# apple/ml-gmpi

Hardware: AMD Instinct MI355X
Metric: Mpix*planes/s (higher is better)
Workload: dtype f32; 1 GPU; FFHQ1024-shaped: 1024x1024, 96 planes, batch 4 views, bf16 storage; views_per_gpu=4, views_total=4, H=1024, W=1024, planes=96, variant=auto, strict_order=False, outputs=rgb+depth, parallelism=views sharded x1, poses=truncated-gaussian draw (seed 3) on every rank

## Files before the change

### include/gmpi_render.h

```cpp
#ifndef GMPI_RENDER_H
#define GMPI_RENDER_H

#include <stdint.h>

#ifdef __cplusplus
extern "C" {
#endif

#define GMPI_ABI_VERSION 2

enum { GMPI_DTYPE_F32 = 0, GMPI_DTYPE_BF16 = 1, GMPI_DTYPE_F16 = 2, GMPI_DTYPE_U8 = 3 };

enum {
    GMPI_FLAG_ALIGN_CORNERS = 1 << 0,
    GMPI_FLAG_OUT_PM1 = 1 << 1,
    GMPI_FLAG_CHECK_LAST_PLANE = 1 << 2,
    GMPI_FLAG_CHECK_RANGE = 1 << 3,
    GMPI_FLAG_STRICT_ORDER = 1 << 4,
    GMPI_FLAG_HINT_FRONTAL = 1 << 5,
    GMPI_FLAG_HINT_TILTED = 1 << 6,
    GMPI_FLAG_GRAD_OVERWRITE = 1 << 7,
    GMPI_FLAG_HINT_OBLIQUE = 1 << 8,
    GMPI_FLAG_ALL = (1 << 9) - 1
};
// ... 9 lines not shown
enum {
    GMPI_VARIANT_AUTO = 0,
    GMPI_VARIANT_GATHER = 1,
    GMPI_VARIANT_LDS = 2,
    GMPI_VARIANT_WAVE = 3,
    GMPI_VARIANT_DMA = 4,
    GMPI_VARIANT_BAND = 5
};

enum {
    GMPI_OK = 0,
    GMPI_E_NULL = -1,
    GMPI_E_SHAPE = -2,
    GMPI_E_DTYPE = -3,
    GMPI_E_STRIDE = -4,
    GMPI_E_ABI = -5,
    GMPI_E_VARIANT = -6,
    GMPI_E_FLAGS = -7,
    GMPI_E_WORKSPACE = -8,
    GMPI_E_LAUNCH = -100
};

typedef struct GmpiRenderParams {
    uint32_t struct_size;
    uint32_t flags;
    int32_t variant;
    int32_t rgba_dtype;

    int32_t N, M, D;
    int32_t Ht, Wt;
    int32_t H, W;
    int32_t views_per_mpi;

    const void *rgba;
    int64_t rgba_stride[5];
    const int32_t *view_to_mpi;
    const float *dhw;
    const float *ray_dir;
    const float *eye_pos;
    const float *z_dir;

    float *rgb_out;
    float *depth_out;
    float *transmittance_out;
    uint32_t *status;

    void *workspace;
    uint64_t workspace_bytes;
} GmpiRenderParams;

uint64_t gmpi_render_workspace_bytes(const GmpiRenderParams *params);

int gmpi_mpi_render_launch(const GmpiRenderParams *params, void *stream);

int gmpi_mpi_render_layers_launch(const GmpiRenderParams *params, void *stream);

int gmpi_render_layers_supports(const GmpiRenderParams *params);

int gmpi_mpi_render_layers_backward_launch(const GmpiRenderParams *params, const float *grad_rgb, const float *grad_depth,
                                           const float *grad_transmittance , float *grad_layers,
                                           const int64_t *grad_layers_stride , void *stream);

int gmpi_render_layers_backward_supports(const GmpiRenderParams *params, const int64_t *grad_layers_stride);

int gmpi_mpi_render_backward_launch(const GmpiRenderParams *params, const float *grad_rgb, const float *grad_depth,
                                    float *grad_rgba, const int64_t *grad_rgba_stride, void *stream);
int gmpi_mpi_render_backward_ex_launch(const GmpiRenderParams *params, const float *grad_rgb, const float *grad_depth,
                                       const float *grad_transmittance, float *grad_rgba, const int64_t *grad_rgba_stride,
                                       void *stream);
uint64_t gmpi_render_backward_workspace_bytes(const GmpiRenderParams *params);

typedef struct GmpiCarry {
    uint32_t struct_size;
    uint32_t reserved;
    const float *state_in;
    float *state_out;
} GmpiCarry;
int gmpi_mpi_render_chunk_launch(const GmpiRenderParams *params, const GmpiCarry *carry, void *stream);

int gmpi_mpi_render_chunk_backward_launch(const GmpiRenderParams *params, const float *grad_rgb, const float *grad_depth,
                                          const float *grad_transmittance, const float *T_in, const float *S_in, float *S_out,
                                          float *grad_rgba, const int64_t *grad_rgba_stride, void *stream);

int gmpi_mpi_render_geometry_backward_launch(const GmpiRenderParams *params, const float *grad_rgb, const float *grad_depth,
                                             float *grad_ray_dir, float *grad_eye_pos, float *grad_z_dir, float *grad_dhw,
                                             void *stream);
int gmpi_mpi_render_geometry_backward_ex_launch(const GmpiRenderParams *params, const float *grad_rgb, const float *grad_depth,
                                                const float *grad_transmittance, float *grad_ray_dir, float *grad_eye_pos,
                                                float *grad_z_dir, float *grad_dhw, void *stream);
uint64_t gmpi_render_geometry_backward_workspace_bytes(const GmpiRenderParams *params, int want_dhw);

typedef struct GmpiSharedColor {
    uint32_t struct_size;
    const void *rgb;
    int64_t rgb_stride[3];
    const void *background;
    int64_t background_stride[3];
} GmpiSharedColor;

int gmpi_mpi_render_shared_launch(const GmpiRenderParams *params, const GmpiSharedColor *shared, void *stream);

int gmpi_render_shared_supports(const GmpiRenderParams *params, const GmpiSharedColor *shared);

int gmpi_mpi_render_shared_backward_launch(const GmpiRenderParams *params, const GmpiSharedColor *shared, const float *grad_rgb_out,
                                           const float *grad_depth, const float *grad_transmittance, float *grad_shared_rgb,
                                           const int64_t *grad_shared_rgb_stride, float *grad_alpha, const int64_t *grad_alpha_stride,
// ... 141 lines not shown
```

### ml-gmpi_amd/_lib.py

```python
import ctypes
import os
import subprocess

_PKG = os.path.dirname(os.path.abspath(__file__))
_SO = os.path.join(_PKG, "libgmpi_render.so")
_LIB = None

ABI_VERSION = 2
DTYPE_F32, DTYPE_BF16, DTYPE_F16 = 0, 1, 2
DTYPE_U8 = 3
FLAG_ALIGN_CORNERS, FLAG_OUT_PM1, FLAG_CHECK_LAST_PLANE, FLAG_CHECK_RANGE, FLAG_STRICT_ORDER, FLAG_HINT_FRONTAL, FLAG_HINT_TILTED = 1, 2, 4, 8, 16, 32, 64
FLAG_HINT_OBLIQUE = 256
FLAG_GRAD_OVERWRITE = 128
STATUS_OUT_OF_LAST_PLANE, STATUS_RGBA_RANGE, STATUS_CAMERA_BEHIND_PLANE, STATUS_BAD_VIEW_INDEX = 1, 2, 4, 8
STATUS_WORDS = 4
VARIANT_AUTO, VARIANT_GATHER, VARIANT_LDS, VARIANT_WAVE, VARIANT_DMA, VARIANT_BAND = 0, 1, 2, 3, 4, 5
VARIANTS = {"auto": VARIANT_AUTO, "gather": VARIANT_GATHER, "lds": VARIANT_LDS, "wave": VARIANT_WAVE, "band": VARIANT_BAND}

EXPORTS = (
    "gmpi_mpi_render_launch",
    "gmpi_render_workspace_bytes",
    "gmpi_render_backward_workspace_bytes",
    "gmpi_mpi_render_backward_launch",
    "gmpi_render_geometry_backward_workspace_bytes",
    "gmpi_mpi_render_geometry_backward_launch",
    "gmpi_mpi_render_backward_ex_launch",
    "gmpi_mpi_render_geometry_backward_ex_launch",
    "gmpi_mpi_render_chunk_launch",
    "gmpi_mpi_render_chunk_backward_launch",
    "gmpi_mpi_render_layers_launch",
    "gmpi_render_layers_supports",
    "gmpi_mpi_render_layers_backward_launch",
    "gmpi_render_layers_backward_supports",
    "gmpi_mpi_render_shared_launch",
    "gmpi_mpi_render_shared_backward_launch",
    "gmpi_render_shared_supports",
    "gmpi_mpi_render_shaded_launch",
    "gmpi_render_shaded_supports",
    "gmpi_mpi_render_shaded_backward_launch",
    "gmpi_mpi_render_depth_launch",
    "gmpi_mpi_render_depth_window_launch",
    "gmpi_render_depth_window_supports",
    "gmpi_mpi_render_depth_backward_launch",
    "gmpi_mpi_render_depth_backward_tile_launch",
    "gmpi_render_layout_backward_gather_workspace_bytes",
    "gmpi_render_layout_backward_gather_runs",
    "gmpi_render_layout_backward_gather_set_runs",
    "gmpi_mpi_render_shared_backward_gather_launch",
    "gmpi_mpi_render_depth_backward_gather_launch",
    "gmpi_mpi_render_shared_geometry_backward_launch",
    "gmpi_mpi_render_depth_geometry_backward_launch",
    "gmpi_mpi_render_depth_geometry_backward_pz_launch",
    "gmpi_render_depth_geometry_backward_workspace_bytes",
    "gmpi_last_plane_uv_minmax_launch",
    "gmpi_rgba_range_check_launch",
    "gmpi_frames_to_uint8_launch",
    "gmpi_generate_rays_launch",
    "gmpi_alpha_depth_launch",
    "gmpi_light_blur_launch",
    "gmpi_light_shading_launch",
    "gmpi_light_apply_launch",
    "gmpi_light_apply_backward_launch",
    "gmpi_light_shading_backward_launch",
    "gmpi_light_blur_backward_launch",
    "gmpi_light_shade_images_launch",
    "gmpi_light_shade_images_backward_launch",
    "gmpi_alpha_depth_backward_launch",
    "gmpi_alpha_depth_backward_ex_launch",
    "gmpi_ramp_depth_launch",
    "gmpi_ramp_depth_backward_launch",
    "gmpi_selftest_division_launch",
    "gmpi_stream_probe_launch",
    "gmpi_query",
    "gmpi_version_string",
)

_ERRORS = {
    -1: "GMPI_E_NULL (required pointer is NULL)",
    -2: "GMPI_E_SHAPE (non-positive or inconsistent extent, or more than 65535 views for the gather kernel / the backward)",
    -3: "GMPI_E_DTYPE (unknown rgba dtype, or uint8 storage handed to an entry other than the forward render)",
    -4: "GMPI_E_STRIDE (innermost rgba stride must be 1 -- or 4 with channel stride 1 for interleaved uint8 texels in the forward render, or for float layers at gmpi_mpi_render_layers_launch --, strides non-negative)",
    -5: "GMPI_E_ABI (GmpiRenderParams size mismatch between binding and library)",
    -6: "GMPI_E_VARIANT (requested kernel variant cannot run this shape)",
    -7: "GMPI_E_FLAGS (undefined bit in GmpiRenderParams.flags)",
    -8: "GMPI_E_WORKSPACE (workspace missing, too small or not 256-byte aligned)",
}


class GmpiError(RuntimeError):
    pass


class GmpiRenderParams(ctypes.Structure):
    _fields_ = [
        ("struct_size", ctypes.c_uint32), ("flags", ctypes.c_uint32),
        ("variant", ctypes.c_int32), ("rgba_dtype", ctypes.c_int32),
        ("N", ctypes.c_int32), ("M", ctypes.c_int32), ("D", ctypes.c_int32),
        ("Ht", ctypes.c_int32), ("Wt", ctypes.c_int32), ("H", ctypes.c_int32), ("W", ctypes.c_int32),
        ("views_per_mpi", ctypes.c_int32),
        ("rgba", ctypes.c_void_p), ("rgba_stride", ctypes.c_int64 * 5),
        ("view_to_mpi", ctypes.c_void_p), ("dhw", ctypes.c_void_p), ("ray_dir", ctypes.c_void_p),
        ("eye_pos", ctypes.c_void_p), ("z_dir", ctypes.c_void_p),
        ("rgb_out", ctypes.c_void_p), ("depth_out", ctypes.c_void_p), ("transmittance_out", ctypes.c_void_p),
        ("status", ctypes.c_void_p),
        ("workspace", ctypes.c_void_p), ("workspace_bytes", ctypes.c_uint64),
    ]


class GmpiCarry(ctypes.Structure):
    _fields_ = [
        ("struct_size", ctypes.c_uint32), ("reserved", ctypes.c_uint32),
        ("state_in", ctypes.c_void_p), ("state_out", ctypes.c_void_p),
    ]


class GmpiSharedColor(ctypes.Structure):
    _fields_ = [
        ("struct_size", ctypes.c_uint32),
        ("rgb", ctypes.c_void_p), ("rgb_stride", ctypes.c_int64 * 3),
        ("background", ctypes.c_void_p), ("background_stride", ctypes.c_int64 * 3),
    ]


class GmpiShading(ctypes.Structure):
    _fields_ = [
        ("struct_size", ctypes.c_uint32),
        ("shading", ctypes.c_void_p), ("shading_stride", ctypes.c_int64 * 2),
    ]


class GmpiDepthAlpha(ctypes.Structure):
    _fields_ = [
        ("struct_size", ctypes.c_uint32),
        ("plane_z", ctypes.c_void_p), ("plane_z_stride", ctypes.c_int64),
        ("z_lo", ctypes.c_float), ("z_hi", ctypes.c_float), ("z_den", ctypes.c_float),
    ]


def source_hash() -> str:
    import glob
    import hashlib
    h = hashlib.sha256()
    files = sorted(glob.glob(os.path.join(_PKG, "csrc", "*.hip")) + glob.glob(os.path.join(_PKG, "csrc", "*.hpp")))
    files.append(os.path.join(os.path.dirname(_PKG), "include", "gmpi_render.h"))
    for f in files:
        with open(f, "rb") as fh:
            h.update(os.path.basename(f).encode() + b"\0" + fh.read())
    return h.hexdigest()[:12]


def library_path() -> str:
    return _SO


_STAMP = os.path.join(_PKG, "csrc", ".built_from")


def build_extension(force: bool = False, verbose: bool = False) -> str:
    want = source_hash() + " " + _makefile_hash()
    have = open(_STAMP).read().strip() if os.path.isfile(_STAMP) else None
    force = force or os.environ.get("GMPI_BUILD_FORCE", "") not in ("", "0") or have != want or not os.path.isfile(_SO)
    cmd = ["make", "-C", os.path.join(_PKG, "csrc"), "-j4"] + (["-B"] if force else [])
    res = subprocess.run(cmd, capture_output=True, text=True)
    if verbose or res.returncode != 0:
        print(res.stdout)
        print(res.stderr)
    if res.returncode != 0 or not os.path.isfile(_SO):
        raise GmpiError("building libgmpi_render.so failed:\n" + res.stderr[-4000:])
    with open(_STAMP, "w") as f:
        f.write(want + "\n")
    return _SO


def _makefile_hash() -> str:
    import hashlib
    with open(os.path.join(_PKG, "csrc", "Makefile"), "rb") as f:
        return hashlib.sha256(f.read()).hexdigest()[:8]


def build_report() -> str:
    import glob
    import time
    rows = [f"sources {source_hash()} (csrc/*.hip, *.hpp, include/gmpi_render.h); stamp {open(_STAMP).read().strip() if os.path.isfile(_STAMP) else None}"]
    for f in sorted(glob.glob(os.path.join(_PKG, "csrc", "*.o"))) + [_SO]:
        if os.path.isfile(f):
            rows.append(f"  {os.path.relpath(f, os.path.dirname(_PKG)):44s} {os.path.getsize(f):9d} B  {time.strftime('%Y-%m-%d %H:%M:%S', time.localtime(os.path.getmtime(f)))}")
    return "\n".join(rows)


def load_library():
    global _LIB
    if _LIB is not None:
        return _LIB
    if not os.path.isfile(_SO):
        raise GmpiError(
            f"HIP extension not built: {_SO} is missing. This package has no CPU/PyTorch fallback. "
            "Build it with `python -c \"import __graft_entry__ as g; g.build()\"` or `make -C ml-gmpi_amd/csrc`.")
    import torch
    try:
        lib = ctypes.CDLL(_SO)
    except OSError as e:
        raise GmpiError(f"could not load {_SO}: {e}") from e
    missing = [s for s in EXPORTS if not hasattr(lib, s)]
    if missing:
        raise GmpiError(f"{_SO} does not export {missing}; rebuild it")
    vp = ctypes.c_void_p
    lib.gmpi_mpi_render_launch.restype = ctypes.c_int
    lib.gmpi_mpi_render_launch.argtypes = [ctypes.POINTER(GmpiRenderParams), vp]
    lib.gmpi_render_workspace_bytes.restype = ctypes.c_uint64
    lib.gmpi_render_workspace_bytes.argtypes = [ctypes.POINTER(GmpiRenderParams)]
    lib.gmpi_render_backward_workspace_bytes.restype = ctypes.c_uint64
    lib.gmpi_render_backward_workspace_bytes.argtypes = [ctypes.POINTER(GmpiRenderParams)]
    lib.gmpi_mpi_render_backward_launch.restype = ctypes.c_int
    lib.gmpi_mpi_render_backward_launch.argtypes = [ctypes.POINTER(GmpiRenderParams), vp, vp, vp,
                                                    ctypes.POINTER(ctypes.c_int64), vp]
    lib.gmpi_render_geometry_backward_workspace_bytes.restype = ctypes.c_uint64
    lib.gmpi_render_geometry_backward_workspace_bytes.argtypes = [ctypes.POINTER(GmpiRenderParams), ctypes.c_int]
    lib.gmpi_mpi_render_geometry_backward_launch.restype = ctypes.c_int
    lib.gmpi_mpi_render_geometry_backward_launch.argtypes = [ctypes.POINTER(GmpiRenderParams), vp, vp, vp, vp, vp, vp, vp]
    lib.gmpi_mpi_render_backward_ex_launch.restype = ctypes.c_int
    lib.gmpi_mpi_render_backward_ex_launch.argtypes = [ctypes.POINTER(GmpiRenderParams), vp, vp, vp, vp,
                                                       ctypes.POINTER(ctypes.c_int64), vp]
    lib.gmpi_mpi_render_geometry_backward_ex_launch.restype = ctypes.c_int
    lib.gmpi_mpi_render_geometry_backward_ex_launch.argtypes = [ctypes.POINTER(GmpiRenderParams), vp, vp, vp, vp, vp, vp, vp, vp]
    lib.gmpi_mpi_render_chunk_launch.restype = ctypes.c_int
    lib.gmpi_mpi_render_chunk_launch.argtypes = [ctypes.POINTER(GmpiRenderParams), ctypes.POINTER(GmpiCarry), vp]
    lib.gmpi_mpi_render_chunk_backward_launch.restype = ctypes.c_int
    lib.gmpi_mpi_render_chunk_backward_launch.argtypes = [ctypes.POINTER(GmpiRenderParams), vp, vp, vp, vp, vp, vp, vp,
                                                          ctypes.POINTER(ctypes.c_int64), vp]
    lib.gmpi_mpi_render_layers_launch.restype = ctypes.c_int
    lib.gmpi_mpi_render_layers_launch.argtypes = [ctypes.POINTER(GmpiRenderParams), vp]
    lib.gmpi_render_layers_supports.restype = ctypes.c_int
    lib.gmpi_render_layers_supports.argtypes = [ctypes.POINTER(GmpiRenderParams)]
    lib.gmpi_mpi_render_layers_backward_launch.restype = ctypes.c_int
    lib.gmpi_mpi_render_layers_backward_launch.argtypes = [ctypes.POINTER(GmpiRenderParams), vp, vp, vp, vp, ctypes.POINTER(ctypes.c_int64), vp]
    lib.gmpi_render_layers_backward_supports.restype = ctypes.c_int
    lib.gmpi_render_layers_backward_supports.argtypes = [ctypes.POINTER(GmpiRenderParams), ctypes.POINTER(ctypes.c_int64)]
    lib.gmpi_mpi_render_shared_launch.restype = ctypes.c_int
    lib.gmpi_mpi_render_shared_launch.argtypes = [ctypes.POINTER(GmpiRenderParams), ctypes.POINTER(GmpiSharedColor), vp]
    i64p = ctypes.POINTER(ctypes.c_int64)
    lib.gmpi_render_shared_supports.restype = ctypes.c_int
    lib.gmpi_render_shared_supports.argtypes = [ctypes.POINTER(GmpiRenderParams), ctypes.POINTER(GmpiSharedColor)]
    lib.gmpi_mpi_render_shared_backward_launch.restype = ctypes.c_int
    lib.gmpi_mpi_render_shared_backward_launch.argtypes = [ctypes.POINTER(GmpiRenderParams), ctypes.POINTER(GmpiSharedColor), vp, vp, vp,
                                                           vp, i64p, vp, i64p, vp, i64p, vp]
    lib.gmpi_mpi_render_shaded_launch.restype = ctypes.c_int
    lib.gmpi_mpi_render_shaded_launch.argtypes = [ctypes.POINTER(GmpiRenderParams), ctypes.POINTER(GmpiShading), vp]
    lib.gmpi_render_shaded_supports.restype = ctypes.c_int
    lib.gmpi_render_shaded_supports.argtypes = [ctypes.POINTER(GmpiRenderParams), ctypes.POINTER(GmpiShading)]
    lib.gmpi_mpi_render_shaded_backward_launch.restype = ctypes.c_int
    lib.gmpi_mpi_render_shaded_backward_launch.argtypes = [ctypes.POINTER(GmpiRenderParams), ctypes.POINTER(GmpiShading), vp, vp, vp, vp, i64p, vp, i64p, vp]
    lib.gmpi_mpi_render_depth_launch.restype = ctypes.c_int
    lib.gmpi_mpi_render_depth_launch.argtypes = [ctypes.POINTER(GmpiRenderParams), ctypes.POINTER(GmpiSharedColor), ctypes.POINTER(GmpiDepthAlpha), vp]
    lib.gmpi_mpi_render_depth_window_launch.restype = ctypes.c_int
    lib.gmpi_mpi_render_depth_window_launch.argtypes = list(lib.gmpi_mpi_render_depth_launch.argtypes)
    lib.gmpi_render_depth_window_supports.restype = ctypes.c_int
    lib.gmpi_render_depth_window_supports.argtypes = [ctypes.POINTER(GmpiRenderParams), ctypes.POINTER(GmpiSharedColor), ctypes.POINTER(GmpiDepthAlpha)]
    lib.gmpi_mpi_render_depth_backward_launch.restype = ctypes.c_int
    lib.gmpi_mpi_render_depth_backward_launch.argtypes = [ctypes.POINTER(GmpiRenderParams), ctypes.POINTER(GmpiSharedColor), ctypes.POINTER(GmpiDepthAlpha),
                                                          vp, vp, vp, vp, i64p, vp, i64p, vp, i64p, vp]
    lib.gmpi_mpi_render_depth_backward_tile_launch.restype = ctypes.c_int
# ... 91 lines not shown
```

### ml-gmpi_amd/csrc/gmpi_abi.hip

```cpp
#include "gmpi_device.hpp"
#include "gmpi_shared.hpp"

#include "../../include/gmpi_render.h"

#include <atomic>
#include <cstdlib>

namespace gmpi {

hipError_t launch_gather(const KParams& p, int dtype, hipStream_t stream);
hipError_t launch_lds(const KParams& p, int dtype, int tune, hipStream_t stream);
hipError_t launch_gather_chunk(const KParams& p, const CarryK& carry, int dtype, hipStream_t stream);
hipError_t launch_lds_chunk(const KParams& p, const CarryK& carry, int dtype, hipStream_t stream);
hipError_t launch_u8_chunk(const KParams& p, const CarryK& carry, hipStream_t stream);
hipError_t launch_backward_chunk(const KParams& p, int dtype, const float* g_rgb, const float* g_depth, const float* g_T, const float* T_in, const float* S_in,
                                 float* S_out, float* g_rgba, const int64_t* gstride, bool tiles, hipStream_t stream);
hipError_t launch_backward(const KParams& p, int dtype, const float* g_rgb, const float* g_depth, const float* g_T, float* g_rgba,
                           const int64_t* gstride, bool tiles, hipStream_t stream);
bool lds_variant_supports(const KParams& p, int dtype);
int lds_variant_query(int what);
hipError_t launch_wave(const KParams& p, int dtype, int tune, hipStream_t stream);
bool wave_variant_supports(const KParams& p, int dtype);
hipError_t launch_band(const KParams& p, int dtype, int tune, hipStream_t stream);
bool band_variant_supports(const KParams& p, int dtype);
// ... 178 lines not shown
                                                          float* __restrict__ depth, float* __restrict__ tout) {
    const int b = blockIdx.z;
    const int x = blockIdx.x * blockDim.x + threadIdx.x, y = blockIdx.y;
    if (x >= W) return;
    const T* a = alpha + b * sb + y * sr + x;
    float Tr = 1.0f, Z = 0.0f;
    alpha_depth_composite(D, ds, [&](int k) { return to_f32(a[k * sd]); }, Tr, Z);
    const int64_t o = (static_cast<int64_t>(b) * H + y) * W + x;
    depth[o] = Z;
    if (tout) tout[o] = Tr;
}

__device__ __forceinline__ uint32_t mix32(uint32_t x) {
    x ^= x >> 16, x *= 0x7feb352du, x ^= x >> 15, x *= 0x846ca68bu, x ^= x >> 16;
    return x;
}
__device__ __forceinline__ float unit_float(uint32_t h) { return __uint_as_float(0x3f800000u | (h >> 9)) - 1.0f; }
__global__ __launch_bounds__(256) void selftest_division_kernel(uint64_t pairs, uint32_t seed, unsigned long long* mism) {
    const uint64_t stride = static_cast<uint64_t>(gridDim.x) * blockDim.x;
    unsigned int bad[4] = {0, 0, 0, 0};
    for (uint64_t i = static_cast<uint64_t>(blockIdx.x) * blockDim.x + threadIdx.x; i < pairs; i += stride) {
        const uint32_t lo = static_cast<uint32_t>(i), hi = static_cast<uint32_t>(i >> 32);
        const uint32_t a = mix32(lo ^ seed), b = mix32(a + mix32(seed + 0x5bd1e995u) * 0x9e3779b9u + hi * 0x85ebca6bu + 0x85ebca6bu), c = mix32(b ^ 0xc2b2ae35u);
        const int cls = static_cast<int>(c & 3u);
        float n, d;
        if (cls == 0) {
            n = (unit_float(a) - 0.5f) * 4.0f;
            d = 0.35f + 0.65f * unit_float(b);
            if (c & 4u) d = -d;
        } else if (cls == 1) {
            n = (unit_float(a) - 0.5f) * 2.0f;
            d = 0.02f + 2.0f * unit_float(b);
        } else if (cls == 2) {
            n = __uint_as_float((a & 0x807fffffu) | ((107u + (a >> 23) % 41u) << 23));
            d = __uint_as_float((b & 0x807fffffu) | ((107u + (b >> 23) % 41u) << 23));
        } else {
            n = __uint_as_float((a & 0x807fffffu) | ((107u + (a >> 23) % 41u) << 23));
            d = __uint_as_float(0x007fffffu | ((107u + (b >> 23) % 41u) << 23) | (b & 0x80000000u));
        }
        const float r = 1.0f / d;
        const float q = div_by_recip(n, d, r);
        const float q_ref = n / d;
        if (__float_as_uint(q) != __float_as_uint(q_ref) && !(q == 0.0f && q_ref == 0.0f)) bad[cls]++;
    }
#pragma unroll
    for (int k = 0; k < 4; ++k) {
        unsigned int v = bad[k];
#pragma unroll
        for (int o = 32; o > 0; o >>= 1) v += __shfl_xor(v, o);
        if ((threadIdx.x & 63) == 0 && v) atomicAdd(mism + k, static_cast<unsigned long long>(v));
    }
}

static int to_kparams(const GmpiRenderParams* q, KParams& p, bool need_outputs, bool need_volume = false, bool takes_u8 = false) {
    if (q == nullptr) return GMPI_E_NULL;
    if (q->struct_size != sizeof(GmpiRenderParams)) return GMPI_E_ABI;
    bool interleaved = false;
    if (q->flags & ~static_cast<uint32_t>(GMPI_FLAG_ALL)) return GMPI_E_FLAGS;
    if (q->N < 0 || q->M <= 0 || q->D <= 0 || q->Ht <= 0 || q->Wt <= 0 || q->H <= 0 || q->W <= 0) return GMPI_E_SHAPE;
    if (q->view_to_mpi == nullptr) {
        if (q->views_per_mpi < 1) return GMPI_E_SHAPE;
        if (q->N > static_cast<int64_t>(q->M) * q->views_per_mpi) return GMPI_E_SHAPE;
    }
    if (q->dhw == nullptr || q->ray_dir == nullptr || q->eye_pos == nullptr) return GMPI_E_NULL;
    if (need_outputs && (q->rgb_out == nullptr || q->depth_out == nullptr)) return GMPI_E_NULL;
    if (need_outputs || need_volume) {
        if (q->rgba == nullptr || q->z_dir == nullptr) return GMPI_E_NULL;
        if (q->rgba_dtype < GMPI_DTYPE_F32 || q->rgba_dtype > (takes_u8 ? GMPI_DTYPE_U8 : GMPI_DTYPE_F16)) return GMPI_E_DTYPE;
        interleaved = takes_u8 && q->rgba_dtype == GMPI_DTYPE_U8 && q->rgba_stride[4] == 4 && q->rgba_stride[2] == 1;
        if (q->rgba_stride[4] != 1 && !interleaved) return GMPI_E_STRIDE;
        for (int i = 0; i < 4; ++i)
            if (q->rgba_stride[i] < 0) return GMPI_E_STRIDE;
        if (q->rgba_stride[3] < (interleaved ? 4 : 1) * static_cast<int64_t>(q->Wt) || q->rgba_stride[2] == 0 || q->rgba_stride[1] == 0) return GMPI_E_STRIDE;
    }
    p.rgba = q->rgba;
    p.view_to_mpi = q->view_to_mpi;
    p.dhw = q->dhw;
    p.ray_dir = q->ray_dir;
    p.eye_pos = q->eye_pos;
    p.z_dir = q->z_dir;
    p.rgb_out = q->rgb_out;
    p.depth_out = q->depth_out;
    p.T_out = q->transmittance_out;
    p.status = q->status;
    p.s_mpi = q->rgba_stride[0];
    p.s_plane = q->rgba_stride[1];
    p.s_chan = interleaved ? 0 : q->rgba_stride[2];
    p.s_row = q->rgba_stride[3];
    p.N = q->N, p.M = q->M, p.D = q->D, p.Ht = q->Ht, p.Wt = q->Wt, p.H = q->H, p.W = q->W;
    p.views_per_mpi = q->view_to_mpi ? 1 : q->views_per_mpi;
    p.flags = q->flags;
    p.ws = q->workspace;
    p.ws_bytes = q->workspace != nullptr ? q->workspace_bytes : 0;
    p.gate = nullptr, p.gate_gen = 0, p.gate_sense = 0;
    p.band_cols = 1, p.band_rot = 0, p.band_split = 1, p.band_tail = 0;
    return GMPI_OK;
}

constexpr int64_t kAutoBandMin = 256;
constexpr int64_t kAutoBandMinF32 = 1024;
constexpr int64_t kAutoBandMinUnmeasured = 512;
constexpr int64_t kAutoBandMinShared = 1024, kAutoBandMinSharedF32 = 2048;

static int64_t band_count(const KParams& p, int dtype) {
    const int bw = band_pixels_wide(dtype);
    return static_cast<int64_t>(p.N) * ((p.W + bw - 1) / bw) * ((p.H + 7) / 8);
}
static bool auto_takes_band(const KParams& p, int dtype) {
    if (dtype != GMPI_DTYPE_BF16 && dtype != GMPI_DTYPE_F32 && dtype != GMPI_DTYPE_F16) return false;
    if (p.view_to_mpi == nullptr && p.views_per_mpi > 1) {
        if ((p.flags & (GMPI_FLAG_HINT_OBLIQUE | GMPI_FLAG_HINT_TILTED)) != 0) return false;
#ifdef GMPI_TUNE
        static const int env_shared = [] { const char* e = getenv("GMPI_TUNE_SHARED"); return e ? atoi(e) : 1; }();
        if (env_shared == 0) return false;
#endif
    }
    const int bw = band_pixels_wide(dtype);
    const int64_t cols = (p.W + bw - 1) / bw, rows = (p.H + 7) / 8;
    if (static_cast<int64_t>(p.W) * 4 < cols * bw * 3 || static_cast<int64_t>(p.H) * 4 < rows * 8 * 3) return false;
    int64_t need = dtype == GMPI_DTYPE_F32 ? kAutoBandMinF32 : kAutoBandMin;
    if (p.view_to_mpi == nullptr && p.views_per_mpi > 1) need = dtype == GMPI_DTYPE_F32 ? kAutoBandMinSharedF32 : kAutoBandMinShared;
    if (dtype != GMPI_DTYPE_F32 && (p.flags & (GMPI_FLAG_STRICT_ORDER | GMPI_FLAG_HINT_TILTED | GMPI_FLAG_HINT_OBLIQUE)) != 0) need = kAutoBandMinUnmeasured;
    return band_count(p, dtype) >= need;
}

static int hip_rc(hipError_t e) { return e == hipSuccess ? GMPI_OK : GMPI_E_LAUNCH - static_cast<int>(e); }

static int layers_strides_ok(const GmpiRenderParams* q) {
    if (q->rgba_stride[2] != 1 || q->rgba_stride[4] != 4) return GMPI_E_STRIDE;
    if (q->rgba_stride[0] < 0 || q->rgba_stride[1] < 0 || q->rgba_stride[3] < 4 * static_cast<int64_t>(q->Wt)) return GMPI_E_STRIDE;
    return GMPI_OK;
}
static int to_kparams_layers(const GmpiRenderParams* q, KParams& p, bool backward = false) {
    GmpiRenderParams planar = *q;
    planar.rgba_stride[0] = planar.rgba_stride[1] = planar.rgba_stride[2] = 1, planar.rgba_stride[3] = q->Wt, planar.rgba_stride[4] = 1;
    const int rc = to_kparams(&planar, p, !backward, backward);
    if (rc != GMPI_OK) return rc;
    const int64_t esize = q->rgba_dtype == GMPI_DTYPE_F32 ? 4 : 2;
    p.s_mpi = q->rgba_stride[0] * esize, p.s_plane = q->rgba_stride[1] * esize, p.s_row = q->rgba_stride[3] * esize, p.s_chan = 0;
    return GMPI_OK;
}
static int layers_backward_args(const GmpiRenderParams* q, const int64_t* gst, KParams& p) {
    if (q == nullptr) return GMPI_E_NULL;
    if (q->struct_size != sizeof(GmpiRenderParams)) return GMPI_E_ABI;
    const int rs = layers_strides_ok(q);
    if (rs != GMPI_OK) return rs;
    if (q->rgba_dtype == GMPI_DTYPE_U8) return GMPI_E_DTYPE;
    const int rc = to_kparams_layers(q, p, true);
    if (rc != GMPI_OK) return rc;
    if (gst == nullptr) return GMPI_E_NULL;
    if (gst[2] != 1 || gst[4] != 4 || gst[3] < 4 * static_cast<int64_t>(q->Wt)) return GMPI_E_STRIDE;
    if (gst[1] <= 0 || (gst[0] <= 0 && !(gst[0] == 0 && q->M == 1))) return GMPI_E_STRIDE;
    return GMPI_OK;
}

}

using namespace gmpi;

extern "C" {

int gmpi_mpi_render_launch(const GmpiRenderParams* params, void* stream) {
    if (params != nullptr && params->struct_size == sizeof(GmpiRenderParams) && params->N == 0) return GMPI_OK;
    KParams p;
    const int rc = to_kparams(params, p, true, false, true);
    if (rc != GMPI_OK) return rc;
    if (p.N == 0) return GMPI_OK;
    hipStream_t st = static_cast<hipStream_t>(stream);
    int variant = params->variant;
    if (params->rgba_dtype == GMPI_DTYPE_U8) {
        const bool staged = u8_variant_supports(p);
        if (variant == GMPI_VARIANT_AUTO) variant = staged ? GMPI_VARIANT_LDS : GMPI_VARIANT_GATHER;
        if (variant == GMPI_VARIANT_GATHER) {
            if (p.N > 65535) return GMPI_E_SHAPE;
            return hip_rc(launch_gather(p, GMPI_DTYPE_U8, st));
        }
        if (variant == GMPI_VARIANT_LDS && staged) return hip_rc(launch_u8(p, st));
        return GMPI_E_VARIANT;
    }
    if (variant == GMPI_VARIANT_AUTO) {
        const int64_t pixels = static_cast<int64_t>(p.N) * p.H * p.W;
        const int64_t strips = static_cast<int64_t>(p.N) * ((p.W + 31) / 32) * ((p.H + 7) / 8);
        const bool strict = (p.flags & GMPI_FLAG_STRICT_ORDER) != 0;
        const bool lds_ok = lds_variant_supports(p, params->rgba_dtype), wave_ok = wave_variant_supports(p, params->rgba_dtype);
        const bool frontal = (p.flags & GMPI_FLAG_HINT_FRONTAL) != 0;
        const bool tilted = (p.flags & GMPI_FLAG_HINT_TILTED) != 0;
        const bool shared = p.view_to_mpi == nullptr && p.views_per_mpi > 1;
        const bool small = strict ? (pixels <= (int64_t(1) << 19) && pixels > (int64_t(1) << 18))
                         : params->rgba_dtype == GMPI_DTYPE_F32 ? (strips <= 512 || (strips > 1536 && strips <= 2048 && !tilted))
                                                                : (strips <= 512 || (strips <= 2048 && frontal && !shared));
        variant = (wave_ok && (small || !lds_ok)) ? GMPI_VARIANT_WAVE : lds_ok ? GMPI_VARIANT_LDS : GMPI_VARIANT_GATHER;
        const bool band_path = lds_ok && auto_takes_band(p, params->rgba_dtype) && band_variant_supports(p, params->rgba_dtype);
        if (band_path) variant = GMPI_VARIANT_LDS;
        if (band_path) {
            static std::atomic<uint32_t> gate_counter{0x6d2b79f5u};
            uint32_t gen = gate_counter.fetch_add(1u, std::memory_order_relaxed);
            KParams pb = p;
            pb.gate = band_gate_words(p, params->rgba_dtype), pb.gate_gen = gen, pb.gate_sense = 0u;
            const hipError_t e = launch_band(pb, params->rgba_dtype, 0, st);
            if (e != hipSuccess) return hip_rc(e);
            pb.gate_sense = 1u;
            return hip_rc(launch_lds(pb, params->rgba_dtype, 0, st));
        }
    }
    if (variant == GMPI_VARIANT_GATHER) {
        if (p.N > 65535) return GMPI_E_SHAPE;
        return hip_rc(launch_gather(p, params->rgba_dtype, st));
    }
    int tune = 0;
#ifdef GMPI_TUNE
    static const int env_tune = [] { const char* e = getenv("GMPI_TUNE_WAVE"); return e ? atoi(e) : 0; }();
    tune = env_tune;
#endif
    if (variant == GMPI_VARIANT_WAVE) {
        if (!wave_variant_supports(p, params->rgba_dtype)) return GMPI_E_VARIANT;
        return hip_rc(launch_wave(p, params->rgba_dtype, tune, st));
    }
    if (variant == GMPI_VARIANT_LDS) {
        if (!lds_variant_supports(p, params->rgba_dtype)) return GMPI_E_VARIANT;
        return hip_rc(launch_lds(p, params->rgba_dtype, tune, st));
    }
    if (variant == GMPI_VARIANT_BAND) {
        if (!band_variant_supports(p, params->rgba_dtype)) return GMPI_E_VARIANT;
        return hip_rc(launch_band(p, params->rgba_dtype, tune, st));
    }
    return GMPI_E_VARIANT;
}

int gmpi_render_layers_supports(const GmpiRenderParams* params) {
    if (params == nullptr) return GMPI_E_NULL;
    if (params->struct_size != sizeof(GmpiRenderParams)) return GMPI_E_ABI;
    const int rs = layers_strides_ok(params);
    if (rs != GMPI_OK) return rs;
    KParams p;
    if (params->rgba_dtype == GMPI_DTYPE_U8) {
        const int rc = to_kparams(params, p, true, false, true);
        return rc != GMPI_OK ? rc : (u8_variant_supports(p) ? 1 : 0);
    }
    const int rc = to_kparams_layers(params, p);
    return rc != GMPI_OK ? rc : (layers_variant_supports(p, params->rgba_dtype) ? 1 : 0);
}

int gmpi_mpi_render_layers_launch(const GmpiRenderParams* params, void* stream) {
    if (params == nullptr) return GMPI_E_NULL;
    if (params->struct_size != sizeof(GmpiRenderParams)) return GMPI_E_ABI;
    if (params->N == 0) return GMPI_OK;
    const int rs = layers_strides_ok(params);
    if (rs != GMPI_OK) return rs;
    if (params->rgba_dtype == GMPI_DTYPE_U8) return gmpi_mpi_render_launch(params, stream);
    KParams p;
    const int rc = to_kparams_layers(params, p);
    if (rc != GMPI_OK) return rc;
    int variant = params->variant;
    if (variant != GMPI_VARIANT_AUTO && variant != GMPI_VARIANT_GATHER && variant != GMPI_VARIANT_LDS) return GMPI_E_VARIANT;
    const bool staged = layers_variant_supports(p, params->rgba_dtype);
    if (variant == GMPI_VARIANT_AUTO) variant = staged ? GMPI_VARIANT_LDS : GMPI_VARIANT_GATHER;
    hipStream_t st = static_cast<hipStream_t>(stream);
    if (variant == GMPI_VARIANT_GATHER) {
        if (p.N > 65535) return GMPI_E_SHAPE;
        return hip_rc(launch_gather_layers(p, params->rgba_dtype, st));
    }
    if (!staged) return GMPI_E_VARIANT;
    return hip_rc(launch_layers(p, params->rgba_dtype, st));
}

int gmpi_render_layers_backward_supports(const GmpiRenderParams* params, const int64_t* grad_layers_stride) {
    KParams p;
    const int rc = layers_backward_args(params, grad_layers_stride, p);
    return rc != GMPI_OK ? rc : (backward_layers_tile_supports(p, params->rgba_dtype, grad_layers_stride) ? 1 : 0);
}

int gmpi_mpi_render_layers_backward_launch(const GmpiRenderParams* params, const float* grad_rgb, const float* grad_depth, const float* grad_transmittance,
                                           float* grad_layers, const int64_t* grad_layers_stride, void* stream) {
    if (params != nullptr && params->struct_size == sizeof(GmpiRenderParams) && params->N == 0) return GMPI_OK;
    KParams p;
    const int rc = layers_backward_args(params, grad_layers_stride, p);
    if (rc != GMPI_OK) return rc;
    if (grad_rgb == nullptr || grad_layers == nullptr) return GMPI_E_NULL;
    return hip_rc(launch_backward_layers(p, params->rgba_dtype, grad_rgb, grad_depth, grad_transmittance, grad_layers, grad_layers_stride,
                                         params->variant != GMPI_VARIANT_GATHER, static_cast<hipStream_t>(stream)));
}

uint64_t gmpi_render_workspace_bytes(const GmpiRenderParams* params) {
    KParams p;
    if (to_kparams(params, p, true, false, true) != GMPI_OK || p.N == 0) return 0;
    if (params->rgba_dtype == GMPI_DTYPE_U8) return 0;
    if (params->variant == GMPI_VARIANT_BAND) return band_workspace_bytes(p, params->rgba_dtype);
    if (params->variant == GMPI_VARIANT_AUTO && auto_takes_band(p, params->rgba_dtype)) return band_workspace_bytes(p, params->rgba_dtype);
    return 0;
}

uint64_t gmpi_render_backward_workspace_bytes(const GmpiRenderParams* params) {
    KParams p;
    if (to_kparams(params, p, false, true) != GMPI_OK || p.N == 0) return 0;
    if (params->variant == GMPI_VARIANT_GATHER) return 0;
    return backward_gather_workspace_bytes(p, params->rgba_dtype);
}

int gmpi_mpi_render_backward_launch(const GmpiRenderParams* params, const float* grad_rgb, const float* grad_depth,
                                    float* grad_rgba, const int64_t* grad_rgba_stride, void* stream) {
    return gmpi_mpi_render_backward_ex_launch(params, grad_rgb, grad_depth, nullptr, grad_rgba, grad_rgba_stride, stream);
}

int gmpi_mpi_render_backward_ex_launch(const GmpiRenderParams* params, const float* grad_rgb, const float* grad_depth,
                                       const float* grad_transmittance, float* grad_rgba, const int64_t* grad_rgba_stride, void* stream) {
    if (params != nullptr && params->struct_size == sizeof(GmpiRenderParams) && params->N == 0) return GMPI_OK;
    KParams p;
    const int rc = to_kparams(params, p, false, true);
    if (rc != GMPI_OK) return rc;
    if (grad_rgb == nullptr || grad_rgba == nullptr || grad_rgba_stride == nullptr) return GMPI_E_NULL;
    if (p.N > 65535) return GMPI_E_SHAPE;
    if (grad_rgba_stride[4] != 1) return GMPI_E_STRIDE;
    for (int i = 0; i < 4; ++i)
        if (grad_rgba_stride[i] <= 0 && !(i == 0 && params->M == 1)) return GMPI_E_STRIDE;
    return hip_rc(launch_backward(p, params->rgba_dtype, grad_rgb, grad_depth, grad_transmittance, grad_rgba, grad_rgba_stride,
                                  params->variant != GMPI_VARIANT_GATHER, static_cast<hipStream_t>(stream)));
}

int gmpi_mpi_render_chunk_launch(const GmpiRenderParams* params, const GmpiCarry* carry, void* stream) {
    if (params != nullptr && params->struct_size == sizeof(GmpiRenderParams) && params->N == 0) return GMPI_OK;
    KParams p;
    const int rc = to_kparams(params, p, false, true, true);
    if (rc != GMPI_OK) return rc;
    if (carry == nullptr) return GMPI_E_NULL;
    if (carry->struct_size != sizeof(GmpiCarry)) return GMPI_E_ABI;
    int variant = params->variant;
    if (variant == GMPI_VARIANT_WAVE || variant == GMPI_VARIANT_BAND) return GMPI_E_VARIANT;
    if (variant != GMPI_VARIANT_AUTO && variant != GMPI_VARIANT_GATHER && variant != GMPI_VARIANT_LDS) return GMPI_E_VARIANT;
    if (carry->state_out == nullptr && p.rgb_out == nullptr && p.depth_out == nullptr && p.T_out == nullptr) return GMPI_E_NULL;
    const CarryK ck{carry->state_in, carry->state_out};
    p.ws = nullptr, p.ws_bytes = 0;
    hipStream_t st = static_cast<hipStream_t>(stream);
    const bool u8 = params->rgba_dtype == GMPI_DTYPE_U8;
    const bool staged = u8 ? u8_variant_supports(p) : lds_variant_supports(p, params->rgba_dtype);
    if (variant == GMPI_VARIANT_AUTO) variant = staged ? GMPI_VARIANT_LDS : GMPI_VARIANT_GATHER;
    if (variant == GMPI_VARIANT_GATHER) {
        if (p.N > 65535) return GMPI_E_SHAPE;
        return hip_rc(launch_gather_chunk(p, ck, params->rgba_dtype, st));
// ... 493 lines not shown
    hipStream_t st = static_cast<hipStream_t>(stream);
    dispatch_dtype(alpha_dtype, [&](auto t) {
        using T = typename decltype(t)::type;
        hipLaunchKernelGGL(alpha_depth_kernel<T>, grid, block, 0, st, static_cast<const T*>(alpha), stride_b, stride_d, stride_row, plane_ds, D, H, W, depth_out,
                           transmittance_out);
    });
    return hip_rc(hipGetLastError());
}

int gmpi_selftest_division_launch(uint64_t pairs, uint32_t seed, uint64_t* mismatches, void* stream) {
    if (mismatches == nullptr) return GMPI_E_NULL;
    if (pairs == 0) return GMPI_OK;
    const uint64_t want = (pairs + 255) / 256;
    const unsigned blocks = static_cast<unsigned>(want < 256u * 64u ? want : 256u * 64u);
    hipLaunchKernelGGL(selftest_division_kernel, dim3(blocks), dim3(256), 0, static_cast<hipStream_t>(stream), pairs, seed,
                       reinterpret_cast<unsigned long long*>(mismatches));
    return hip_rc(hipGetLastError());
}

int gmpi_stream_probe_launch(const void* buf, uint64_t bytes, uint32_t* sink, void* stream) {
    if (buf == nullptr) return GMPI_E_NULL;
    if (reinterpret_cast<uintptr_t>(buf) % 4 != 0) return GMPI_E_STRIDE;
    if (bytes < 4) return GMPI_OK;
    hipLaunchKernelGGL(stream_probe_kernel, dim3(256 * 2), dim3(256), 0, static_cast<hipStream_t>(stream), static_cast<const uint32_t*>(buf),
                       static_cast<int64_t>(bytes / 4), sink);
    return hip_rc(hipGetLastError());
}

int gmpi_query(int32_t what) {
    switch (what) {
        case 0: return GMPI_ABI_VERSION;
        case 1: return static_cast<int>(sizeof(GmpiRenderParams));
        case 2: return 950;
        case 3: case 4: case 5: return lds_variant_query(what);
        case 6: return 1;
        case 7: return 0;
        case 8: return 1;
        case 9: return static_cast<int>(kAutoBandMin);
        case 10: return static_cast<int>(kAutoBandMinF32);
        case 11: return 1;
        case 12: case 13: case 14: return shared_forward_query(what);
        case 16: case 17: case 18: case 20: return u8_variant_query(what);
        case 22: return 1;
        case 23: return depth_tile_planes();
        case 25: return 1;
        case 26: case 27: case 28: return depth_window_query(what);
        case 30: return 1;
        case 32: return 1;
        case 34: return 1;
        case 38: return 1;
        case 40: return 1;
        case 42: return 1;
        case 44: return 1;
        case 46: return 1;
        case 36: return 1;
        default: return -1;
    }
}

const char* gmpi_version_string(void) { return "ml-gmpi_amd 0.3 (gfx950, ABI 2)"; }

}
```

### ml-gmpi_amd/csrc/gmpi_device.hpp

```cpp
#pragma once
#include <hip/hip_runtime.h>
#include <stdint.h>

#include <type_traits>

#include "../../include/gmpi_render.h"

#pragma clang fp contract(off)

namespace gmpi {

constexpr float kNarrowScale = 0.95f;

struct KParams {
    const void* rgba;
    const int32_t* view_to_mpi;
    const float* dhw;
    const float* ray_dir;
    const float* eye_pos;
    const float* z_dir;
    float* rgb_out;
    float* depth_out;
    float* T_out;
    uint32_t* status;
    int64_t s_mpi, s_plane, s_chan, s_row;
    int32_t N, M, D, Ht, Wt, H, W, views_per_mpi;
    uint32_t flags;
    void* ws;
    uint64_t ws_bytes;
    uint32_t* gate;
    uint32_t gate_gen, gate_sense;
    int32_t band_cols;
    int32_t band_rot, band_split;
    int32_t band_tail;
};
struct CarryK {
    const float* state_in;
    float* state_out;
};
struct NoCarry {};

__device__ __forceinline__ int xcd_item_per_group(int block, int group_items, int n_items, int rot = 0, int split = 1) {
    const int per_xcd = (group_items + 7) / 8, n_groups = (n_items + group_items - 1) / group_items;
    const int jb = block / 8, grp = jb / per_xcd, rr = jb - grp * per_xcd;
    const int piece = split > 1 ? rr * split / per_xcd : 0;
    const int in_group = ((block + grp * rot + piece * (8 / max(split, 1))) % 8) * per_xcd + rr;
    const int item = grp * group_items + in_group;
    return (grp >= n_groups || in_group >= group_items || item >= n_items) ? n_items : item;
}
inline __host__ unsigned xcd_grid_per_group(int group_items, int n_items) {
    return static_cast<unsigned>(((group_items + 7) / 8) * 8 * ((n_items + group_items - 1) / group_items));
}

__device__ __forceinline__ bool view_gated_out(const KParams& p, int n) {
    return p.gate != nullptr && ((p.gate[n] == p.gate_gen) != (p.gate_sense != 0u));
}

__device__ __forceinline__ int view_mpi(const KParams& p, int n, uint32_t& bad) {
    int m = p.view_to_mpi ? p.view_to_mpi[n] : n / p.views_per_mpi;
    if (m < 0 || m >= p.M) {
        bad |= GMPI_STATUS_BAD_VIEW_INDEX;
        m = min(max(m, 0), p.M - 1);
    }
    return m;
}

__device__ __forceinline__ void item_to_view(const KParams& p, int item, int per_view, int& n, int& rem) {
    if (p.view_to_mpi == nullptr && p.views_per_mpi > 1) {
        const int group = item / (per_view * p.views_per_mpi);
        const int first = group * p.views_per_mpi, size = min(p.views_per_mpi, p.N - first);
        const int r = item - first * per_view;
        rem = r / size;
        n = first + (r - rem * size);
    } else {
        n = item / per_view;
        rem = item - n * per_view;
    }
}

struct bf16_t { uint16_t bits; };
struct f16_t { _Float16 v; };

__device__ __forceinline__ float to_f32(float v) { return v; }
__device__ __forceinline__ float to_f32(bf16_t v) { return __uint_as_float(static_cast<uint32_t>(v.bits) << 16); }
__device__ __forceinline__ float to_f32(f16_t v) { return static_cast<float>(v.v); }
struct u8_t { uint8_t code; };
constexpr float kInv255 = 1.0f / 255.0f;
__device__ __forceinline__ float unorm8_to_f32(float c) {
// ... 244 lines not shown
            const float t_se = to_f32(ch[ob + xb]);
            if (check_range && !(in_unit(t_nw) && in_unit(t_ne) && in_unit(t_sw) && in_unit(t_se))) bad |= GMPI_STATUS_RGBA_RANGE;
            smp[c] = bilerp<STRICT>(t_nw, t_ne, t_sw, t_se, f);
        }
    }
}

struct NoShade {};
struct ShadeK {
    const float* s;
    int64_t s_mpi, s_row;
};
__device__ __forceinline__ float shade_texel(float t, float s) { return fminf(fmaxf(t * s, 0.0f), 1.0f); }

template <typename TexT, bool STRICT>
__device__ __forceinline__ void shaded_gather_sample(const TexT* __restrict__ pl, int64_t s_chan, int64_t s_row, const float* __restrict__ sh, int64_t sh_row,
                                                     int Ht, int Wt, float ix, float iy, bool check_range, uint32_t& bad, float (&smp)[4]) {
    Footprint f = footprint(ix, iy, Ht, Wt);
    const bool x0in = f.x0 >= 0 && f.x0 <= Wt - 1, x1in = f.x0 >= -1 && f.x0 <= Wt - 2;
    const bool y0in = f.y0 >= 0 && f.y0 <= Ht - 1, y1in = f.y0 >= -1 && f.y0 <= Ht - 2;
    if (!(x0in && y0in)) f.nw = 0.0f;
    if (!(x1in && y0in)) f.ne = 0.0f;
    if (!(x0in && y1in)) f.sw = 0.0f;
    if (!(x1in && y1in)) f.se = 0.0f;
    const int xa = min(max(f.x0, 0), Wt - 1), xb = min(max(f.x0 + 1, 0), Wt - 1);
    const int ya = min(max(f.y0, 0), Ht - 1), yb = min(max(f.y0 + 1, 0), Ht - 1);
    const int64_t oa = static_cast<int64_t>(ya) * s_row, ob = static_cast<int64_t>(yb) * s_row;
    const int64_t ha = static_cast<int64_t>(ya) * sh_row, hb = static_cast<int64_t>(yb) * sh_row;
    const float s_nw = sh[ha + xa], s_ne = sh[ha + xb], s_sw = sh[hb + xa], s_se = sh[hb + xb];
#pragma unroll
    for (int c = 0; c < 4; ++c) {
        const TexT* __restrict__ ch = pl + c * s_chan;
        float t_nw = to_f32(ch[oa + xa]);
        float t_ne = to_f32(ch[oa + xb]);
        float t_sw = to_f32(ch[ob + xa]);
        float t_se = to_f32(ch[ob + xb]);
        if (c < 3) {
            t_nw = shade_texel(t_nw, s_nw), t_ne = shade_texel(t_ne, s_ne), t_sw = shade_texel(t_sw, s_sw), t_se = shade_texel(t_se, s_se);
        } else if (check_range && !(in_unit(t_nw) && in_unit(t_ne) && in_unit(t_sw) && in_unit(t_se))) {
            bad |= GMPI_STATUS_RGBA_RANGE;
        }
        smp[c] = bilerp<STRICT>(t_nw, t_ne, t_sw, t_se, f);
    }
}

struct View {
    int m;
    const float* __restrict__ dhw;
    float ex, ey, ez;
    float zx, zy, zz;
    float cx, cy;
    int64_t HW;
    const float* __restrict__ rays;
};
template <bool AC>
__device__ __forceinline__ View view_setup(const KParams& p, int n, uint32_t& bad) {
    View vw;
    vw.m = view_mpi(p, n, bad);
    vw.dhw = p.dhw + static_cast<int64_t>(vw.m) * p.D * 3;
    vw.ex = p.eye_pos[3 * n + 0], vw.ey = p.eye_pos[3 * n + 1], vw.ez = p.eye_pos[3 * n + 2];
    vw.zx = p.z_dir[3 * n + 0], vw.zy = p.z_dir[3 * n + 1], vw.zz = p.z_dir[3 * n + 2];
    vw.cx = AC ? static_cast<float>(p.Wt - 1) * 0.5f : static_cast<float>(p.Wt);
    vw.cy = AC ? static_cast<float>(p.Ht - 1) * 0.5f : static_cast<float>(p.Ht);
    vw.HW = static_cast<int64_t>(p.H) * p.W;
    vw.rays = p.ray_dir + static_cast<int64_t>(n) * 3 * vw.HW;
    return vw;
}

__device__ __forceinline__ void check_camera_behind(const KParams& p, const View& vw, bool once) {
    if (p.status != nullptr && once) {
        const float ez0 = p.eye_pos[2];
        bool behind = false;
        for (int k = 0; k < p.D; ++k) behind |= !(vw.dhw[3 * k] >= ez0);
        if (behind) atomicOr(p.status, GMPI_STATUS_CAMERA_BEHIND_PLANE);
    }
}

__device__ __forceinline__ float ray_dot(const View& vw, float rx, float ry, float rz) {
    float dot = rx * vw.zx;
    dot = dot + ry * vw.zy;
    dot = dot + rz * vw.zz;
    return dot;
}

__device__ __forceinline__ bool outside_pm1(float u, float v) { return !(u >= -1.0f && u <= 1.0f && v >= -1.0f && v <= 1.0f); }

struct LastPlane {
    bool check;
    float d, ph, pw;
};
__device__ __forceinline__ LastPlane last_plane(const KParams& p, const View& vw) {
    LastPlane lp{(p.flags & GMPI_FLAG_CHECK_LAST_PLANE) != 0, 0.0f, 1.0f, 1.0f};
    if (lp.check) lp.d = vw.dhw[3 * (p.D - 1) + 0], lp.ph = vw.dhw[3 * (p.D - 1) + 1], lp.pw = vw.dhw[3 * (p.D - 1) + 2];
    return lp;
}
template <bool AC>
__device__ __forceinline__ bool leaves_last_plane(const View& vw, const LastPlane& lp, float rx, float ry, float rz) {
    if (!lp.check) return false;
    float ix, iy, s, u, v;
    plane_coord<AC>(lp.d - vw.ez, lp.ph, lp.pw, vw.ex, vw.ey, rx, ry, rz, vw.cx, vw.cy, ix, iy, s, u, v);
    return outside_pm1(u, v);
}

template <typename TexT, bool AC, bool STRICT, typename CheckT>
__device__ __forceinline__ void gather_plane(const KParams& p, const View& vw, const TexT* vol, int k, float zdiff, float ph, float pw,
                                             float rx, float ry, float rz, float dot, CheckT check_range, uint32_t& bad, Accum& A) {
    float ix, iy, s, u, v, smp[4];
    plane_coord<AC>(zdiff, ph, pw, vw.ex, vw.ey, rx, ry, rz, vw.cx, vw.cy, ix, iy, s, u, v);
    gather_sample<TexT, STRICT>(tex_offset(vol, static_cast<int64_t>(k) * p.s_plane), p.s_chan, p.s_row, p.Ht, p.Wt, ix, iy, check_range, bad, smp);
    blend<STRICT>(A, smp[0], smp[1], smp[2], smp[3], s, dot);
}

__device__ __forceinline__ Accum load_carry(NoCarry, int, int64_t, int64_t) { return Accum{}; }
__device__ __forceinline__ void store_carry(NoCarry, int, int64_t, int64_t, const Accum&, bool) {}
__device__ __forceinline__ Accum load_carry(const CarryK& c, int n, int64_t HW, int64_t pix) {
    Accum A;
    if (c.state_in != nullptr) {
        const float* s = c.state_in + static_cast<int64_t>(n) * 5 * HW + pix;
        A.r = s[0], A.g = s[HW], A.b = s[2 * HW], A.z = s[3 * HW], A.T = s[4 * HW];
    }
    return A;
}
__device__ __forceinline__ void store_carry(const CarryK& c, int n, int64_t HW, int64_t pix, const Accum& A, bool active) {
    if (c.state_out != nullptr && active) {
// ... 24 lines not shown
    if (active) {
        float* __restrict__ out = p.rgb_out + static_cast<int64_t>(n) * 3 * HW + pix;
        out[0] = r;
        out[HW] = g;
        out[2 * HW] = b;
        p.depth_out[static_cast<int64_t>(n) * HW + pix] = finish_depth<STRICT>(A, dot);
        if (p.T_out) p.T_out[static_cast<int64_t>(n) * HW + pix] = A.T;
    }
}

inline __host__ __device__ int view_group_items(const KParams& p, int per_view) { return per_view * (p.view_to_mpi == nullptr ? p.views_per_mpi : 1); }

__device__ __forceinline__ int fwd_tile_id(const KParams& p, int block, int tiles_x, int tiles_y, int n_tiles, int rot = 0, int split = 1) {
    return xcd_item_per_group(block, view_group_items(p, tiles_x * tiles_y), n_tiles, rot, split);
}
struct FwdTile { int n, rem, txi, tyi; };
__device__ __forceinline__ bool fwd_tile(const KParams& p, int tile_id, int tiles_x, int tiles_y, int n_tiles, FwdTile& t) {
    if (tile_id >= n_tiles) return false;
    item_to_view(p, tile_id, tiles_x * tiles_y, t.n, t.rem);
    t.tyi = t.rem / tiles_x, t.txi = t.rem - t.tyi * tiles_x;
    return true;
}
struct FwdTileGrid { int tiles_x, tiles_y, n_tiles; dim3 grid; };
template <int TW, int TH>
inline FwdTileGrid fwd_tile_grid(const KParams& p) {
    const int tiles_x = (p.W + TW - 1) / TW, tiles_y = (p.H + TH - 1) / TH, n_tiles = tiles_x * tiles_y * p.N;
    return FwdTileGrid{tiles_x, tiles_y, n_tiles, dim3(xcd_grid_per_group(view_group_items(p, tiles_x * tiles_y), n_tiles))};
}

struct TileLane { int px, py; bool active; int64_t pix; };
template <int TW, int TH>
__device__ __forceinline__ TileLane tile_lane(int txi, int tyi, int lane, int W, int H) {
    TileLane l;
    l.px = txi * TW + (lane % TW), l.py = tyi * TH + (lane / TW);
    l.active = l.px < W && l.py < H;
    l.pix = static_cast<int64_t>(min(l.py, H - 1)) * W + min(l.px, W - 1);
    return l;
}
struct TileCorners { int cx0, cx1, cy0, cy1; };
template <int TW, int TH>
__device__ __forceinline__ TileCorners tile_corners(int txi, int tyi, int W, int H) {
    const int cx0 = txi * TW, cy0 = tyi * TH;
    return TileCorners{cx0, min(cx0 + TW - 1, W - 1), cy0, min(cy0 + TH - 1, H - 1)};
}

struct CornerExtent { float mnx, mxx, mny, mxy; bool finite; };
template <bool AC>
__device__ __forceinline__ CornerExtent corner_extent(const View& vw, const float* __restrict__ rdv, int W, float zdiff, float ph, float pw, int cx0, int cx1,
                                                      int cy0, int cy1, float (&cix)[4], float (&ciy)[4]) {
    CornerExtent e{__builtin_inff(), -__builtin_inff(), __builtin_inff(), -__builtin_inff(), true};
#pragma unroll
    for (int c = 0; c < 4; ++c) {
        const int64_t q = static_cast<int64_t>((c & 2) ? cy1 : cy0) * W + ((c & 1) ? cx1 : cx0);
        float s, u, v;
        plane_coord<AC>(zdiff, ph, pw, vw.ex, vw.ey, rdv[q], rdv[vw.HW + q], rdv[2 * vw.HW + q], vw.cx, vw.cy, cix[c], ciy[c], s, u, v);
        e.finite = e.finite && (fabsf(cix[c]) < 1e6f) && (fabsf(ciy[c]) < 1e6f);
        e.mnx = fminf(e.mnx, cix[c]), e.mxx = fmaxf(e.mxx, cix[c]), e.mny = fminf(e.mny, ciy[c]), e.mxy = fmaxf(e.mxy, ciy[c]);
    }
    return e;
}
template <bool AC>
__device__ __forceinline__ CornerExtent corner_extent(const View& vw, const float* __restrict__ rdv, int W, float zdiff, float ph, float pw, int cx0, int cx1,
                                                      int cy0, int cy1) {
    float cix[4], ciy[4];
    return corner_extent<AC>(vw, rdv, W, zdiff, ph, pw, cx0, cx1, cy0, cy1, cix, ciy);
}
constexpr float kBoxSlack = 1.0f / 64;
template <int TPI>
__device__ __forceinline__ int4 item_box(const CornerExtent& e, int max_cols, int max_rows, bool& fits) {
    int4 bb = make_int4(0, 0, 0, 0);
    fits = false;
    if (e.finite) {
        const int bx0 = static_cast<int>(floorf(e.mnx - kBoxSlack)), bx1 = static_cast<int>(floorf(e.mxx + kBoxSlack)) + 1;
        const int by0 = static_cast<int>(floorf(e.mny - kBoxSlack)), by1 = static_cast<int>(floorf(e.mxy + kBoxSlack)) + 1;
        bb.x = bx0 & ~(TPI - 1), bb.y = by0;
        bb.z = (bx1 - bb.x) / TPI + 1, bb.w = by1 - by0 + 1;
        fits = bb.z <= max_cols && bb.w <= max_rows;
    }
    return bb;
}
template <bool AC>
__device__ __forceinline__ int4 tile_box(const KParams& p, const View& vw, const float* __restrict__ rdv, float zdiff, float ph, float pw, int cx0, int cx1,
                                         int cy0, int cy1, int pitch, int rows, float (&cix)[4], float (&ciy)[4]) {
    bool fits;
    int4 bb = item_box<1>(corner_extent<AC>(vw, rdv, p.W, zdiff, ph, pw, cx0, cx1, cy0, cy1, cix, ciy), pitch, rows, fits);
    if (!fits) bb.z = 0;
    return bb;
}
template <bool AC>
__device__ __forceinline__ int4 tile_box(const KParams& p, const View& vw, const float* __restrict__ rdv, float zdiff, float ph, float pw, int cx0, int cx1,
                                         int cy0, int cy1, int pitch, int rows) {
    float cix[4], ciy[4];
    return tile_box<AC>(p, vw, rdv, zdiff, ph, pw, cx0, cx1, cy0, cy1, pitch, rows, cix, ciy);
}

__device__ __forceinline__ int2 origin_words(uint64_t a) { return make_int2(static_cast<int>(a & 0xffffffffu), static_cast<int>((a >> 32) & 0xffffu)); }
__device__ __forceinline__ __amdgpu_buffer_rsrc_t origin_rsrc(int lo, int hi) {
    const uint32_t b_lo = static_cast<uint32_t>(__builtin_amdgcn_readfirstlane(lo)), b_hi = static_cast<uint32_t>(__builtin_amdgcn_readfirstlane(hi));
    return __builtin_amdgcn_make_buffer_rsrc(reinterpret_cast<void*>((static_cast<uint64_t>(b_hi) << 32) | b_lo), 0, static_cast<int>(0x80000000u), 0x00020000);
}

__device__ __forceinline__ int floor_to_int(float x) {
    int r;
    asm("v_cvt_flr_i32_f32 %0, %1" : "=v"(r) : "v"(x));
    return r;
}

__device__ __forceinline__ void report_status(uint32_t* status, uint32_t bad) {
// ... 10 lines not shown
```

### ml-gmpi_amd/csrc/render_band.hip

```cpp
#include "gmpi_device.hpp"
#include "gmpi_band_masks.hpp"

#include <algorithm>
#include <cstdlib>
#include <type_traits>


namespace gmpi {
namespace band {

constexpr int kNT = 1024;
constexpr int SBW = 64, SBH = 8;
constexpr float kBoxEps = 1.0f / 64;
constexpr int kWindowCols16 = 2, kWindowCols32 = 2, kWindowCols32Deep = 2, kDeepPlanes = 128;
constexpr int kViewRotation = 1;
constexpr int kRunPieces = 2;
constexpr int kTicketTail = 16;
constexpr float kCoordLimit = 16384.0f;

typedef uint32_t u32x4 __attribute__((ext_vector_type(4)));
template <int V> using ic = std::integral_constant<int, V>;

template <int D0, int STEP>
__device__ __forceinline__ void dma16x2(uint32_t voff, uint32_t soff1, const u32x4& rsrc, uint32_t lds_dst, uint64_t m0, uint64_t m1);
// ... 82 lines not shown
                 "s_mov_b64 exec, %7\n\ts_add_i32 m0, %3, %16\n\ts_nop 0\n\tbuffer_load_dwordx4 %1, %2, %11 offen lds\n\t"
                 "s_mov_b64 exec, %8\n\ts_add_i32 m0, %3, %17\n\ts_nop 0\n\tbuffer_load_dwordx4 %1, %2, %12 offen lds\n\t"
                 "s_mov_b64 exec, %0"
                 : "=&s"(save) : "v"(voff), "s"(rsrc), "s"(lds_dst), "s"(m0), "s"(m1), "s"(m2), "s"(m3), "s"(m4), "s"(s1), "s"(s2), "s"(s3), "s"(s4),
                   "i"(D0), "i"(D0 + STEP), "i"(D0 + 2 * STEP), "i"(D0 + 3 * STEP), "i"(D0 + 4 * STEP)
                 : "memory", "scc");
}
__device__ __forceinline__ void wg_barrier() { asm volatile("s_waitcnt vmcnt(0) lgkmcnt(0)\n\ts_barrier" ::: "memory"); }
template <int O> __device__ __forceinline__ void tap16(uint32_t& t, uint32_t a) {
    asm volatile("ds_read_u16_d16_hi %0, %1 offset:%2" : "=v"(t) : "v"(a), "i"(O));
}
template <int O> __device__ __forceinline__ void tap32x2(uint32_t& t0, uint32_t& t1, uint32_t a) {
    typedef uint32_t u32x2 __attribute__((ext_vector_type(2)));
    u32x2 v;
    asm volatile("ds_read2_b32 %0, %1 offset0:%2 offset1:%3" : "=v"(v) : "v"(a), "i"(O), "i"(O + 1));
    t0 = v.x, t1 = v.y;
}

__device__ __forceinline__ void band_pos(int brem, int bands_x, int bands_y, int wc, int& bxi, int& byi) {
    const int per_window = wc * bands_y;
    const int g = brem / per_window, r = brem - g * per_window;
    const int cols = min(wc, bands_x - g * wc);
    byi = r / cols;
    bxi = g * wc + (r - byi * cols);
}

constexpr int kPlU4 = 2;
__device__ __forceinline__ uint32_t shape_pack(int nq, int rows, int clo, int ncol, int rlo, int nrow, bool inside) {
    return inside ? static_cast<uint32_t>(nq | rows << 5)
                  : static_cast<uint32_t>(nq | rows << 5 | clo << 9 | ncol << 14 | rlo << 19 | nrow << 23) | 0x80000000u;
}
struct Shape { int nq, rows; uint32_t clo, ncol, rlo, nrow; };
__device__ __forceinline__ Shape shape_unpack(uint32_t w) {
    Shape h;
    h.nq = w & 31, h.rows = (w >> 5) & 15;
    const bool padded = (w >> 31) != 0;
    h.clo = padded ? (w >> 9) & 31 : 0u, h.ncol = padded ? (w >> 14) & 31 : static_cast<uint32_t>(h.nq);
    h.rlo = padded ? (w >> 19) & 15 : 0u, h.nrow = padded ? (w >> 23) & 15 : static_cast<uint32_t>(h.rows);
    return h;
}
template <typename TexT, bool AC>
__global__ __launch_bounds__(1024) void band_table_kernel(const KParams p, const int bands_x, const int bands_y, const int n_bands, const float cx, const float cy,
                                                         uint4* __restrict__ recs, uint4* __restrict__ pl, uint32_t* __restrict__ hdr, uint32_t* __restrict__ tickets) {
    using G = Geo<TexT>;
    constexpr int kES = G::kES, kTPI = G::kTPI, kCols = G::kCols, kMaxRows = G::kMaxRows, kRowBytes = G::kRowBytes, kSubBytes = G::kSubBytes;
    constexpr int NSB = G::NSB;
    static_assert(kCols < 32 && kMaxRows < 16, "shape_pack");
    const int band_id = blockIdx.x;
    int n, brem;
    item_to_view(p, band_id, bands_x * bands_y, n, brem);
    int bxi, byi;
    band_pos(brem, bands_x, bands_y, p.band_cols, bxi, byi);
    uint32_t ignore = 0;
    const int m = view_mpi(p, n, ignore);
    const int Ht = p.Ht, Wt = p.Wt, H = p.H, W = p.W;
    const float ex = p.eye_pos[3 * n + 0], ey = p.eye_pos[3 * n + 1], ez = p.eye_pos[3 * n + 2];
    const int64_t HW = static_cast<int64_t>(H) * W;
    const float* __restrict__ rdv = p.ray_dir + static_cast<int64_t>(n) * 3 * HW;
    const TexT* __restrict__ vol = static_cast<const TexT*>(p.rgba) + static_cast<int64_t>(m) * p.s_mpi;
    const int sx0 = min(bxi * (NSB * SBW), W - 1), sy0 = byi * SBH;
    const int by0p = min(sy0, H - 1), by1p = min(sy0 + SBH - 1, H - 1);
    bool unfit = false;
    for (int i = threadIdx.x; i < p.D * NSB; i += blockDim.x) {
        const int b = i % NSB, k = i / NSB;
        const float* __restrict__ dhw = p.dhw + (static_cast<int64_t>(m) * p.D + k) * 3;
        const float d = dhw[0], ph = dhw[1], pw = dhw[2];
        const float zdiff = d - ez;
        const float hw = pw * 0.5f, hh = ph * 0.5f;
        const int bx0p = min(sx0 + b * SBW, W - 1), bx1p = min(sx0 + b * SBW + SBW - 1, W - 1);
        float mnx = __builtin_inff(), mxx = -__builtin_inff(), mny = mnx, mxy = mxx;
        bool finite = true;
        const float rw_a = __builtin_amdgcn_rcpf(hw), rh_a = __builtin_amdgcn_rcpf(hh);
#pragma unroll
        for (int c = 0; c < 4; ++c) {
            const int64_t q = static_cast<int64_t>((c & 2) ? by1p : by0p) * W + ((c & 1) ? bx1p : bx0p);
            float ix, iy, sc;
            const float crz = rdv[2 * HW + q];
            plane_coord_recip<AC>(zdiff, hw, hh, rw_a, rh_a, ex, ey, rdv[q], rdv[HW + q], crz, __builtin_amdgcn_rcpf(crz), cx, cy, ix, iy, sc);
            finite = finite && (fabsf(ix) < kCoordLimit) && (fabsf(iy) < kCoordLimit);
            mnx = fminf(mnx, ix), mxx = fmaxf(mxx, ix), mny = fminf(mny, iy), mxy = fmaxf(mxy, iy);
        }
        int qx0 = 0, by0 = 0, nq = -1, nrows = 0;
        if (finite) {
            const int bx0 = static_cast<int>(floorf(mnx - kBoxEps)), bx1 = static_cast<int>(floorf(mxx + kBoxEps)) + 1;
            by0 = static_cast<int>(floorf(mny - kBoxEps));
            const int by1 = static_cast<int>(floorf(mxy + kBoxEps)) + 1;
            qx0 = bx0 & ~(kTPI - 1);
            nq = (bx1 - qx0) / kTPI + 1;
            nrows = by1 - by0 + 1;
            if (nq > kCols || nrows > kMaxRows) nq = -1;
        }
        uint32_t shape = 0;
        if (nq > 0) {
            const int clo = min(max(-qx0 / kTPI, 0), nq), chi = min(max((Wt - qx0) / kTPI, 0), nq);
            const int rlo = min(max(-by0, 0), nrows), rhi = min(max(Ht - by0, 0), nrows);
            const bool inside = clo == 0 && chi == nq && rlo == 0 && rhi == nrows;
            shape = shape_pack(nq, nrows, clo, chi - clo, rlo, rhi - rlo, inside);
        } else {
            qx0 = 0, by0 = 0;
            unfit = true;
        }
        const uint64_t origin = reinterpret_cast<uint64_t>(vol + (static_cast<int64_t>(k) * p.s_plane + static_cast<int64_t>(by0) * p.s_row + qx0));
        const int gpart = b * kSubBytes - (by0 * kRowBytes + qx0 * kES);
        recs[(static_cast<int64_t>(band_id) * p.D + k) * NSB + b] =
            make_uint4(static_cast<uint32_t>(origin & 0xffffffffu), static_cast<uint32_t>((origin >> 32) & 0xffffu), shape, static_cast<uint32_t>(gpart));
        if (brem == 0 && b == 0) {
            uint4* r = pl + (static_cast<int64_t>(n) * p.D + k) * kPlU4;
            r[0] = make_uint4(__float_as_uint(zdiff), __float_as_uint(hw), __float_as_uint(hh), __float_as_uint(1.0f / hw));
            r[1] = make_uint4(__float_as_uint(1.0f / hh), 0u, 0u, 0u);
        }
    }
    if (blockIdx.x == 0 && threadIdx.x < 8) tickets[threadIdx.x] = 0u;
    const int any_unfit = __syncthreads_or(unfit ? 1 : 0);
    if (threadIdx.x == 0) {
        hdr[band_id] = static_cast<uint32_t>(any_unfit);
        if (any_unfit && p.gate != nullptr) {
            if (p.view_to_mpi == nullptr && p.views_per_mpi > 1) {
                const int first = n / p.views_per_mpi * p.views_per_mpi, size = min(p.views_per_mpi, p.N - first);
                for (int v = 0; v < size; ++v) p.gate[first + v] = p.gate_gen;
            } else {
                p.gate[n] = p.gate_gen;
            }
        }
    }
}

template <typename TexT, bool AC, bool STRICT, bool CHECK>
__global__ __launch_bounds__(Geo<TexT>::kThreads, Geo<TexT>::kWavesPerSimd) void render_band_kernel(const KParams p, const int bands_x, const int bands_y, const int n_bands, const float cx, const float cy,
                                                         const uint4* __restrict__ recs, const uint4* __restrict__ pl, const uint32_t* __restrict__ hdr, uint32_t* __restrict__ tickets) {
    using G = Geo<TexT>;
    constexpr int kES = G::kES, kTPI = G::kTPI, kCols = G::kCols, kNP = G::kNP;
// ... 7 lines not shown
    __shared__ __attribute__((aligned(16))) unsigned char smem[G::kLdsBytes];
    typedef __attribute__((address_space(3))) unsigned char lds_byte;
    const uint32_t tile_base = static_cast<uint32_t>(reinterpret_cast<uintptr_t>((lds_byte*)smem));

    const int group_items = bands_x * bands_y * (p.view_to_mpi == nullptr ? p.views_per_mpi : 1);
    int band_id;
    {
        const int per_xcd = (group_items + 7) / 8, n_groups = (n_bands + group_items - 1) / group_items, static_blocks = per_xcd * 8 * n_groups;
        const int T = min(p.band_tail, per_xcd);
        const int jb = static_cast<int>(blockIdx.x) / 8, x = static_cast<int>(blockIdx.x) % 8;
        const bool ticketed = T > 0 && (static_cast<int>(blockIdx.x) >= static_blocks || (jb / per_xcd == n_groups - 1 && jb % per_xcd >= per_xcd - T));
        if (!ticketed) {
            band_id = blockIdx.x < static_cast<unsigned>(static_blocks) ? xcd_item_per_group(blockIdx.x, group_items, n_bands, p.band_rot, p.band_split) : n_bands;
        } else {
            int* word = reinterpret_cast<int*>(smem + 2 * kBufBytes);
            if (threadIdx.x == 0) {
                int got = n_bands;
                for (int i = 0; i < 8; ++i) {
                    const int q = (x + i) % 8;
                    const int t = static_cast<int>(atomicAdd(tickets + q, 1u));
                    if (t < T) {
                        got = xcd_item_per_group(q + 8 * ((n_groups - 1) * per_xcd + per_xcd - T + t), group_items, n_bands, p.band_rot, p.band_split);
                        break;
                    }
                }
                *word = got;
            }
            __syncthreads();
            band_id = __builtin_amdgcn_readfirstlane(*word);
            __syncthreads();
        }
    }
#ifdef GMPI_TUNE
    if (p.flags & (1u << 19)) band_id = static_cast<int>(blockIdx.x % 8) * ((n_bands + 7) / 8) + static_cast<int>(blockIdx.x / 8);
#endif
    if (band_id >= n_bands) return;
    int n, brem;
    item_to_view(p, band_id, bands_x * bands_y, n, brem);
    if (view_gated_out(p, n)) return;
    int bxi, byi;
    band_pos(brem, bands_x, bands_y, p.band_cols, bxi, byi);
#ifdef GMPI_TUNE
    const bool stamp = (p.flags & (1u << 22)) != 0 && p.status != nullptr;
    uint64_t stamp_start = 0;
    if (stamp) asm volatile("s_memrealtime %0\n\ts_waitcnt lgkmcnt(0)" : "=s"(stamp_start));
#endif

    const int tid = threadIdx.x;
    auto fresh_tid = [&]() { int t = tid; asm volatile("" : "+v"(t)); return t; };
    const int wave = __builtin_amdgcn_readfirstlane(tid >> 6);
    const int sb = wave / WPS, wj = wave % WPS;
    const int lane = tid & 63;
    uint32_t bad_w = 0;
    View vw = view_setup<AC>(p, n, bad_w);
    vw.cx = cx, vw.cy = cy;
    const int D = p.D, H = p.H, W = p.W;
    const float* __restrict__ dhw = vw.dhw;
    const float ex = vw.ex, ey = vw.ey, ez = vw.ez;
    constexpr bool check_range = CHECK;
    const int64_t HW = vw.HW;
    const float* __restrict__ rdv = vw.rays;
    const TexT* __restrict__ vol = static_cast<const TexT*>(p.rgba) + static_cast<int64_t>(vw.m) * p.s_mpi;
    const int64_t s_chan = p.s_chan, s_row = p.s_row;

    check_camera_behind(p, vw, brem == 0 && tid == 0);

    const int px = bxi * (NSB * SBW) + sb * SBW + lane;
    const int py0 = byi * SBH + wj;
    const int pxc = min(px, W - 1);
    float rx[PPT], ry[PPT], rz[PPT], rcp_rz[PPT];
    Accum A[PPT];
#pragma unroll
    for (int q = 0; q < PPT; ++q) {
        const int64_t pix = static_cast<int64_t>(min(py0 + WPS * q, H - 1)) * W + pxc;
        rx[q] = rdv[pix], ry[q] = rdv[HW + pix], rz[q] = rdv[2 * HW + pix];
        rcp_rz[q] = 1.0f / rz[q];
    }
    auto ray_dot = [&](int q) { return gmpi::ray_dot(vw, rx[q], ry[q], rz[q]); };

    auto loader_pos = [&](int& l_col, int& l_line, int& l_row, bool& l_on) {
        const int t = fresh_tid() & (kSubLanes - 1);
        l_line = t / kCols, l_col = t - l_line * kCols, l_row = l_line >> 2, l_on = t < kPassItems;
    };
    {
        int l_col, l_line, l_row;
        bool l_on;
        loader_pos(l_col, l_line, l_row, l_on);
        reinterpret_cast<uint32_t*>(smem + 2 * kBufBytes)[tid] = static_cast<uint32_t>(l_row * s_row + (l_line & 3) * s_chan + kTPI * l_col) * static_cast<uint32_t>(kES);
    }
    const uint32_t pass_off = static_cast<uint32_t>(kRPP * s_row) * static_cast<uint32_t>(kES), pass_off2 = 2 * pass_off;
    const uint32_t pass_off3 = 3 * pass_off, pass_off4 = 4 * pass_off;
    const uint32_t sub_base = tile_base + static_cast<uint32_t>(sb * kSubBytes);
    const uint32_t wave_dst = sub_base + static_cast<uint32_t>(wj) * 1024u;

#ifdef GMPI_TUNE
    const bool abl_noload = (p.flags & (1u << 16)) != 0, abl_nocomp = (p.flags & (1u << 17)) != 0, abl_noissue = (p.flags & (1u << 18)) != 0;
    const bool abl_nobar = (p.flags & (1u << 20)) != 0, abl_norec = (p.flags & (1u << 21)) != 0;
#else
    constexpr bool abl_noload = false, abl_nocomp = false, abl_noissue = false, abl_nobar = false, abl_norec = false;
#endif

#ifdef GMPI_PROF
    uint32_t prof_acc[8] = {0, 0, 0, 0, 0, 0, 0, 0};
    uint64_t prof_last, prof_start;
    asm volatile("s_memtime %0\n\ts_waitcnt lgkmcnt(0)" : "=s"(prof_start));
    prof_last = prof_start;
#define GMPI_STAMP(i) do { uint64_t now_; asm volatile("s_memtime %0\n\ts_waitcnt lgkmcnt(0)" : "=s"(now_)); prof_acc[i] += static_cast<uint32_t>(now_ - prof_last); prof_last = now_; } while (0)
#else
#define GMPI_STAMP(i) do { } while (0)
#endif

    const uint4* __restrict__ myrec = recs + (static_cast<int64_t>(band_id) * D * NSB + sb);
    const uint4* __restrict__ mypl = pl + static_cast<int64_t>(n) * D * kPlU4;
    constexpr int kRecStep = NSB;

    if (hdr[band_id] != 0) {
#pragma unroll
        for (int q = 0; q < PPT; ++q) {
            const float dot = ray_dot(q);
            for (int t = 0; t < D; ++t) {
                uint32_t gbad = 0;
                gather_plane<TexT, AC, STRICT>(p, vw, vol, t, dhw[3 * t] - ez, dhw[3 * t + 1], dhw[3 * t + 2], rx[q], ry[q], rz[q], dot, std::bool_constant<CHECK>{}, gbad, A[q]);
                if (check_range && __any(gbad != 0)) bad_w |= GMPI_STATUS_RGBA_RANGE;
            }
        }
    } else {
        float dots[PPT];
#pragma unroll
// ... 465 lines not shown
```

### ml-gmpi_amd/csrc/render_gather.hip

```cpp
#include "gmpi_device.hpp"

namespace gmpi {

constexpr int kGatherTileW = 64;
constexpr int kGatherTileH = 4;

template <typename TexT, bool AC, bool STRICT, typename Carry>
__device__ __forceinline__ void render_gather_pixel(const KParams& p, const Carry& carry) {
    const int n = blockIdx.z;
    const int px = blockIdx.x * kGatherTileW + threadIdx.x;
    const int py = blockIdx.y * kGatherTileH + threadIdx.y;
    uint32_t bad = 0;
    const View vw = view_setup<AC>(p, n, bad);
    check_camera_behind(p, vw, blockIdx.x == 0 && blockIdx.y == 0 && threadIdx.x == 0 && threadIdx.y == 0);
    const bool active = px < p.W && py < p.H;
    const int64_t HW = vw.HW;
    const int64_t pix = static_cast<int64_t>(min(py, p.H - 1)) * p.W + min(px, p.W - 1);
    const float rx = vw.rays[pix], ry = vw.rays[HW + pix], rz = vw.rays[2 * HW + pix];
    const float dot = ray_dot(vw, rx, ry, rz);
    const bool check_range = (p.flags & GMPI_FLAG_CHECK_RANGE) != 0;
    const TexT* __restrict__ vol = tex_offset(static_cast<const TexT*>(p.rgba), static_cast<int64_t>(vw.m) * p.s_mpi);

    Accum A = load_carry(carry, n, HW, pix);
#pragma unroll 2
    for (int k = 0; k < p.D; ++k) {
        const float d = vw.dhw[3 * k + 0], ph = vw.dhw[3 * k + 1], pw = vw.dhw[3 * k + 2];
        float ix, iy, s, u, v;
        plane_coord<AC>(d - vw.ez, ph, pw, vw.ex, vw.ey, rx, ry, rz, vw.cx, vw.cy, ix, iy, s, u, v);
        float smp[4];
        gather_sample<TexT, STRICT>(tex_offset(vol, static_cast<int64_t>(k) * p.s_plane), p.s_chan, p.s_row, p.Ht, p.Wt, ix, iy, check_range, bad, smp);
        blend<STRICT>(A, smp[0], smp[1], smp[2], smp[3], s, dot);
    }
    const LastPlane lp = last_plane(p, vw);
    if (leaves_last_plane<AC>(vw, lp, rx, ry, rz)) bad |= GMPI_STATUS_OUT_OF_LAST_PLANE;
    store_pixel<STRICT>(p, n, HW, pix, A, dot, active, carry);
    report_status(p.status, bad);
}

template <typename TexT, bool AC, bool STRICT>
__global__ __launch_bounds__(kGatherTileW* kGatherTileH) void render_gather_kernel(const KParams p) {
    render_gather_pixel<TexT, AC, STRICT>(p, NoCarry{});
}
template <typename TexT, bool AC, bool STRICT>
__global__ __launch_bounds__(kGatherTileW* kGatherTileH) void render_gather_chunk_kernel(const KParams p, const CarryK carry) {
    render_gather_pixel<TexT, AC, STRICT>(p, carry);
}

template <typename TexT>
static hipError_t launch_gather_t(const KParams& p, const CarryK* carry, hipStream_t stream) {
    const dim3 block(kGatherTileW, kGatherTileH);
    const dim3 grid((p.W + kGatherTileW - 1) / kGatherTileW, (p.H + kGatherTileH - 1) / kGatherTileH, p.N);
    dispatch_ac_strict(p.flags, [&](auto AC, auto STRICT) {
        if (carry != nullptr) hipLaunchKernelGGL((render_gather_chunk_kernel<TexT, decltype(AC)::value, decltype(STRICT)::value>), grid, block, 0, stream, p, *carry);
        else hipLaunchKernelGGL((render_gather_kernel<TexT, decltype(AC)::value, decltype(STRICT)::value>), grid, block, 0, stream, p);
    });
    return hipGetLastError();
}

static hipError_t launch_gather_any(const KParams& p, const CarryK* carry, int dtype, hipStream_t stream) {
    if (dtype == GMPI_DTYPE_U8 && u8_interleaved(p)) return launch_gather_t<rgba8_t>(p, carry, stream);
    if (dtype == GMPI_DTYPE_U8) return launch_gather_t<u8_t>(p, carry, stream);
    return dispatch_dtype(dtype, [&](auto t) { return launch_gather_t<typename decltype(t)::type>(p, carry, stream); });
}
hipError_t launch_gather(const KParams& p, int dtype, hipStream_t stream) { return launch_gather_any(p, nullptr, dtype, stream); }
hipError_t launch_gather_chunk(const KParams& p, const CarryK& carry, int dtype, hipStream_t stream) { return launch_gather_any(p, &carry, dtype, stream); }

template <typename TexT>
static hipError_t launch_gather_layers_t(const KParams& p, hipStream_t stream) {
    const dim3 block(kGatherTileW, kGatherTileH);
    const dim3 grid((p.W + kGatherTileW - 1) / kGatherTileW, (p.H + kGatherTileH - 1) / kGatherTileH, p.N);
    dispatch_ac_strict(p.flags, [&](auto AC, auto STRICT) {
// ... 15 lines not shown
```

### ml-gmpi_amd/csrc/render_lds.hip

```cpp
#include "gmpi_device.hpp"

#include <cstdlib>

#include <algorithm>

#include <type_traits>

namespace gmpi {

constexpr int kNT = 512;
constexpr int kChunk = 96;
constexpr int kRecBytes = 48;
constexpr int kMaxStagedItems = 4;

template <int TW> struct TileCfg;
template <> struct TileCfg<32> { static constexpr int kPitch = 56, kMaxLines = 108; };
template <> struct TileCfg<64> { static constexpr int kPitch = 96, kMaxLines = 56; };
template <int TW> constexpr int lds_bytes() { return kChunk * kRecBytes + 2 * TileCfg<TW>::kMaxLines * TileCfg<TW>::kPitch * 4; }
static_assert(lds_bytes<32>() <= 53 * 1024, "3 workgroups per CU");

template <int TPI, int TW, int LPR> struct LoaderCfg {
    static constexpr int kCols = TileCfg<TW>::kPitch / TPI;
    static constexpr int kLinesPerPass = kNT / kCols;
    static constexpr int kNL = (TileCfg<TW>::kMaxLines / 4 * LPR + kLinesPerPass - 1) / kLinesPerPass;
// ... 38 lines not shown
        const h2 a = __builtin_bit_cast(h2, vx), b = __builtin_bit_cast(h2, vy), c = __builtin_bit_cast(h2, vz), d = __builtin_bit_cast(h2, vw);
        o[0] = make_float4(static_cast<float>(a.x), static_cast<float>(a.y), static_cast<float>(b.x), static_cast<float>(b.y));
        o[1] = make_float4(static_cast<float>(c.x), static_cast<float>(c.y), static_cast<float>(d.x), static_cast<float>(d.y));
    }
};

__device__ __forceinline__ bool quad_out_of_unit(const float4& q) {
    const uint32_t a = __float_as_uint(q.x), b = __float_as_uint(q.y), c = __float_as_uint(q.z), d = __float_as_uint(q.w);
    const uint32_t m = max(max(a, b), max(c, d));
    if (__builtin_expect(m <= 0x3f800000u, 1)) return false;
    auto ok = [](uint32_t e) { return e <= 0x3f800000u || e == 0x80000000u; };
    return !(ok(a) && ok(b) && ok(c) && ok(d));
}

template <typename TexT, bool AC, bool STRICT, int TW, int MINW, int PF, int LAYOUT, typename Carry = NoCarry>
__device__ __forceinline__ void render_lds_tile(const KParams& p, const int tiles_x, const int tiles_y, const int n_tiles, const unsigned vblock,
                                                const uint32_t* view_bits = nullptr, const Carry& carry = Carry{}) {
    using Q = Quad<TexT>;
    constexpr int LPR = LAYOUT == 1 ? 1 : 4;
    constexpr int kTexelBytes = 4 * static_cast<int>(sizeof(TexT));
    using LC = LoaderCfg<(LAYOUT == 1 ? 16 / kTexelBytes : Q::kTexels), TW, LPR>;
    constexpr int kPitch = TileCfg<TW>::kPitch, kMaxLines = TileCfg<TW>::kMaxLines, kMaxRows = kMaxLines / 4;
    constexpr int kCapFloats = (LAYOUT == 1 && sizeof(TexT) == 2) ? kMaxLines * kPitch / 2 : kMaxLines * kPitch;
    constexpr int kLdsBytes = kChunk * kRecBytes + 2 * kCapFloats * 4;
    constexpr int TPI = LAYOUT == 1 ? 16 / kTexelBytes : Q::kTexels, kCols = LC::kCols, kRowcPerPass = LC::kLinesPerPass, kNL = LC::kNL;
    constexpr int TH = kNT / TW;

    __shared__ __attribute__((aligned(16))) unsigned char smem[kLdsBytes];
    __shared__ int box_max[2];
    int4* tabL = reinterpret_cast<int4*>(smem);
    float4* tabF = reinterpret_cast<float4*>(smem + kChunk * 16);
    int4* tabG = reinterpret_cast<int4*>(smem + kChunk * 32);
    float* tile0 = reinterpret_cast<float*>(smem + kChunk * kRecBytes);

    const int per_xcd = (n_tiles + 7) / 8;
    int tile_id = (vblock % 8) * per_xcd + vblock / 8;
    if (vblock >= static_cast<unsigned>(per_xcd * 8)) tile_id = n_tiles;
    if (p.gate != nullptr || sizeof(TexT) == 4)
        tile_id = fwd_tile_id(p, vblock, tiles_x, tiles_y, n_tiles, p.band_rot, p.band_split);
#ifdef GMPI_TUNE
    if (p.flags & (1u << 19)) {
        tile_id = (p.gate != nullptr || sizeof(TexT) == 4) ? (vblock % 8) * per_xcd + vblock / 8
                                                           : fwd_tile_id(p, vblock, tiles_x, tiles_y, n_tiles);
        if (vblock >= static_cast<unsigned>(per_xcd * 8) && (p.gate != nullptr || sizeof(TexT) == 4)) tile_id = n_tiles;
    }
#endif
    FwdTile ft;
    if (!fwd_tile(p, tile_id, tiles_x, tiles_y, n_tiles, ft)) return;
    const int n = ft.n;
    if (view_bits != nullptr ? ((view_bits[n >> 5] >> (n & 31)) & 1u) == 0u : view_gated_out(p, n)) return;

    const int tid = threadIdx.x;
    uint32_t bad = 0;
    const View vw = view_setup<AC>(p, n, bad);
    const int D = p.D, Ht = p.Ht, Wt = p.Wt, H = p.H, W = p.W;
    const float* __restrict__ dhw = vw.dhw;
    const float ex = vw.ex, ey = vw.ey, ez = vw.ez, cx = vw.cx, cy = vw.cy;
    const bool check_range = (p.flags & GMPI_FLAG_CHECK_RANGE) != 0;
    const int64_t HW = vw.HW;
    const float* __restrict__ rdv = vw.rays;
    const TexT* __restrict__ vol = static_cast<const TexT*>(p.rgba) + static_cast<int64_t>(vw.m) * p.s_mpi;
    const int64_t s_chan = p.s_chan, s_row = p.s_row, s_plane = p.s_plane;

    check_camera_behind(p, vw, ft.rem == 0 && tid == 0);

    const TileLane tl = tile_lane<TW, TH>(ft.txi, ft.tyi, tid, W, H);
    const int64_t pix = tl.pix;
    const float rx = rdv[pix], ry = rdv[HW + pix], rz = rdv[2 * HW + pix];
    const float dot = ray_dot(vw, rx, ry, rz);
    const float rcp_rz = 1.0f / rz;
    Accum A = load_carry(carry, n, HW, pix);

    const TileCorners tc = tile_corners<TW, TH>(ft.txi, ft.tyi, W, H);
    const int cy0 = tc.cy0, cy1 = tc.cy1;

    int lcol = 0, lrowc = 0, perpass = kRowcPerPass, npass = kNL, dst_base = 0;
    uint32_t g_off[kNL];
    auto set_loader_map = [&](int cols, int max_rows) {
        perpass = __builtin_amdgcn_readfirstlane(kNT / cols);
        npass = __builtin_amdgcn_readfirstlane((LPR * max_rows + perpass - 1) / perpass);
        lrowc = tid / cols;
        lcol = tid - lrowc * cols;
        dst_base = LAYOUT == 1 ? lrowc * (kPitch / TPI) + lcol : lrowc * (kPitch / 4) + lcol * (TPI / 4);
        if (lrowc >= perpass) lcol = 0x3fffffff;
#pragma unroll
        for (int r = 0; r < kNL; ++r) {
            const int rowc = lrowc + r * perpass;
            g_off[r] = static_cast<uint32_t>(LAYOUT == 1 ? rowc * s_row + TPI * lcol : (rowc & 3) * s_chan + (rowc >> 2) * s_row + TPI * lcol) *
                       static_cast<uint32_t>(sizeof(TexT));
        }
    };

    for (int kc = 0; kc < D; kc += kChunk) {
        const int kn = min(kChunk, D - kc);
        int max_nq = kCols, max_rows = kMaxRows;
        auto build_table = [&](int y_lo, int y_hi) -> bool {
            __syncthreads();
            if (tid < 2) box_max[tid] = 0;
            __syncthreads();
            int nq_max = 0, row_max = 0;
            for (int t = tid; t < kn; t += kNT) {
                const int k = kc + t;
                const float d = dhw[3 * k + 0], ph = dhw[3 * k + 1], pw = dhw[3 * k + 2];
                const float zdiff = d - ez;
                bool fits;
                int4 ri = item_box<TPI>(corner_extent<AC>(vw, rdv, W, zdiff, ph, pw, tc.cx0, tc.cx1, y_lo, y_hi), kCols, kMaxRows, fits);
                int cols = 0, lines = 0;
                if (!fits) {
                    ri.z = -1;
                } else {
                    const int clo = min(max(-ri.x / TPI, 0), ri.z), chi = min(max((Wt - ri.x) / TPI, 0), ri.z);
                    const int rlo = min(max(-ri.y, 0), ri.w), rhi = min(max(Ht - ri.y, 0), ri.w);
                    cols = ri.z | clo << 8 | (chi - clo) << 16;
                    lines = LPR * ri.w | LPR * rlo << 8 | LPR * (rhi - rlo) << 16;
                }
                nq_max = max(nq_max, ri.z < 0 ? 1 << 20 : ri.z);
                row_max = max(row_max, ri.w);
                const float hw = pw * 0.5f, hh = ph * 0.5f;
                const int2 origin = origin_words(reinterpret_cast<uint64_t>(vol + (static_cast<int64_t>(k) * s_plane + static_cast<int64_t>(ri.y) * s_row + ri.x)));
                tabL[t] = make_int4(origin.x, origin.y, cols, lines);
                tabF[t] = make_float4(zdiff, hw, hh, 1.0f / hw);
// ... 365 lines not shown
```

### ml-gmpi_amd/csrc/render_u8.hip

```cpp
#include "gmpi_device.hpp"

namespace gmpi {

constexpr int kUW = 32, kUH = 16, kUThreads = kUW * kUH;
constexpr int kUPitch = 64, kURows = 32;
constexpr int kUTPI = 4, kUCols = kUPitch / kUTPI;
constexpr int kUBufWords = kURows * kUPitch;
constexpr int kUChunk = 64;
static_assert(kURows * kUCols == kUThreads, "one loader item per thread");
static_assert(kUPitch % 32 == 0, "row pitch: a multiple of the 32 banks of ds_read2_b32");
static_assert(2 * kUBufWords * 4 + kUChunk * 48 <= 40 * 1024, "4 workgroups per CU");

template <typename TexT, bool AC, bool STRICT, typename Carry = NoCarry>
__device__ __forceinline__ void render_u8_tile(const KParams& p, const int tiles_x, const int tiles_y, const int n_tiles, const Carry& carry = Carry{}) {
    __shared__ int4 box[kUChunk];
    __shared__ int4 org[kUChunk];
    __shared__ float4 geo[kUChunk];
    __shared__ __attribute__((aligned(16))) uint32_t stage[2][kUBufWords];

    const int tid = threadIdx.x;
    FwdTile ft;
    if (!fwd_tile(p, fwd_tile_id(p, blockIdx.x, tiles_x, tiles_y, n_tiles), tiles_x, tiles_y, n_tiles, ft)) return;
    const int n = ft.n;

    uint32_t bad = 0;
    const View vw = view_setup<AC>(p, n, bad);
    check_camera_behind(p, vw, ft.rem == 0 && tid == 0);
    const int D = p.D, Ht = p.Ht, Wt = p.Wt, H = p.H, W = p.W;
    const int64_t HW = vw.HW;
    const float* __restrict__ rdv = vw.rays;
    constexpr bool kPacked = std::is_same_v<TexT, rgba8_t>;
    constexpr int kTexelBytes = kPacked ? 4 : 1;
    const TexT* __restrict__ vol = tex_offset(static_cast<const TexT*>(p.rgba), static_cast<int64_t>(vw.m) * p.s_mpi);

    const TileLane tl = tile_lane<kUW, kUH>(ft.txi, ft.tyi, tid, W, H);
    const int64_t pix = tl.pix;
    const float rx = rdv[pix], ry = rdv[HW + pix], rz = rdv[2 * HW + pix];
    const float dot = ray_dot(vw, rx, ry, rz);
    const float rcp_rz = 1.0f / rz;
    Accum A = load_carry(carry, n, HW, pix);
    const TileCorners tc = tile_corners<kUW, kUH>(ft.txi, ft.tyi, W, H);

    const int lrow = tid / kUCols, lcol = tid - lrow * kUCols;
    const uint32_t l_off = static_cast<uint32_t>(lrow) * static_cast<uint32_t>(p.s_row) + kTexelBytes * kUTPI * lcol;
    const int chan_bytes = __builtin_amdgcn_readfirstlane(static_cast<int>(p.s_chan));

    for (int kc = 0; kc < D; kc += kUChunk) {
        const int kn = min(kUChunk, D - kc);
        __syncthreads();
        for (int t = tid; t < kn; t += kUThreads) {
            const int k = kc + t;
            const float zdiff = vw.dhw[3 * k] - vw.ez, ph = vw.dhw[3 * k + 1], pw = vw.dhw[3 * k + 2];
            bool fits;
            int4 bb = item_box<kUTPI>(corner_extent<AC>(vw, rdv, W, zdiff, ph, pw, tc.cx0, tc.cx1, tc.cy0, tc.cy1), kUCols, kURows, fits);
            if (!fits) bb = make_int4(0, 0, 0, 0);
            box[t] = bb;
            const float hw = pw * 0.5f, hh = ph * 0.5f;
            const int2 o = origin_words(reinterpret_cast<uint64_t>(vol) + static_cast<uint64_t>(static_cast<int64_t>(k) * p.s_plane + bb.y * p.s_row + kTexelBytes * bb.x));
            org[t] = make_int4(o.x, o.y, __float_as_int(1.0f / hh), 0);
            geo[t] = make_float4(zdiff, hw, hh, 1.0f / hw);
        }
        __syncthreads();

        auto issue_loads = [&](int t, uint32_t (&L)[4]) {
            const int4 bb = box[min(t, kn - 1)];
            const int4 oo = org[min(t, kn - 1)];
            const int qx0 = __builtin_amdgcn_readfirstlane(bb.x), by0 = __builtin_amdgcn_readfirstlane(bb.y);
            const int nq = t < kn ? __builtin_amdgcn_readfirstlane(bb.z) : 0, nrows = __builtin_amdgcn_readfirstlane(bb.w);
            const __amdgpu_buffer_rsrc_t rsrc = origin_rsrc(oo.x, oo.y);
            const int gx = qx0 + kUTPI * lcol, gy = by0 + lrow;
            const bool ok = (lcol < nq) & (lrow < nrows) & (gx >= 0) & (gx < Wt) & (gy >= 0) & (gy < Ht);
            const uint32_t off = ok ? l_off : 0x80000000u;
            if constexpr (kPacked) {
                typedef uint32_t u32x4 __attribute__((ext_vector_type(4)));
                const u32x4 q = __builtin_bit_cast(u32x4, __builtin_amdgcn_raw_buffer_load_b128(rsrc, off, 0, 0));
                L[0] = q.x, L[1] = q.y, L[2] = q.z, L[3] = q.w;
            } else {
                L[0] = __builtin_amdgcn_raw_buffer_load_b32(rsrc, off, 0, 0);
                L[1] = __builtin_amdgcn_raw_buffer_load_b32(rsrc, off, chan_bytes, 0);
                L[2] = __builtin_amdgcn_raw_buffer_load_b32(rsrc, off, 2 * chan_bytes, 0);
                L[3] = __builtin_amdgcn_raw_buffer_load_b32(rsrc, off, 3 * chan_bytes, 0);
            }
        };
        auto store_box = [&](int t, uint32_t* buf, const uint32_t (&L)[4]) {
            const int4 bb = box[t];
            const int nq = __builtin_amdgcn_readfirstlane(bb.z), nrows = __builtin_amdgcn_readfirstlane(bb.w);
            typedef uint32_t u32x4 __attribute__((ext_vector_type(4)));
            u32x4 o;
            if constexpr (kPacked) {
                o.x = L[0], o.y = L[1], o.z = L[2], o.w = L[3];
// ... 134 lines not shown
```

### ml-gmpi_amd/csrc/render_wave.hip

```cpp
#include "gmpi_device.hpp"

#include <type_traits>

namespace gmpi {

constexpr int kSW = 32, kSH = 8;
constexpr int kPX = 4;
constexpr int kRing = 32;
constexpr int kGroup = 16;
constexpr int kEntry = 32;
constexpr int wave_lds(int waves_per_simd) { return waves_per_simd >= 4 ? 10240 : waves_per_simd == 3 ? 13312 : 20480; }
constexpr int box_slots(int waves_per_simd, int slot_bytes) { return (wave_lds(waves_per_simd) - kRing * kEntry - 16) / slot_bytes; }
constexpr int kMaxNP = 3;

typedef uint32_t u32x4_t __attribute__((ext_vector_type(4)));
typedef uint32_t u32x2_t __attribute__((ext_vector_type(2)));
typedef float f32x4_t __attribute__((ext_vector_type(4)));
typedef __attribute__((address_space(3))) f32x4_t lds_f32x4;
typedef __attribute__((address_space(3))) u32x4_t lds_u32x4;
typedef __attribute__((address_space(3))) u32x2_t lds_u32x2;
typedef _Float16 f16x2_t __attribute__((ext_vector_type(2)));

template <typename TexT> struct ItemIO;
template <> struct ItemIO<float> {
// ... 53 lines not shown
    }
    static __device__ __forceinline__ bool unsafe_half(const u32x4_t&) { return false; }
    static __device__ __forceinline__ void unpack(const u32x4_t& v, float (&o)[8]) {
        typedef _Float16 h2 __attribute__((ext_vector_type(2)));
        const uint32_t d[4] = {v.x, v.y, v.z, v.w};
#pragma unroll
        for (int i = 0; i < 4; ++i) {
            const h2 h = __builtin_bit_cast(h2, d[i]);
            o[2 * i] = static_cast<float>(h.x), o[2 * i + 1] = static_cast<float>(h.y);
        }
    }
};

__device__ __forceinline__ int wave_max(int v) {
#pragma unroll
    for (int o = 32; o > 0; o >>= 1) v = max(v, __shfl_xor(v, o));
    return __builtin_amdgcn_readfirstlane(v);
}

template <typename TexT, bool AC, bool STRICT, int WPB, int WPS, int SPLIT, bool HALF, int GRPSEL>
__global__ __launch_bounds__(WPB * SPLIT * 64, WPS) void render_wave_kernel(const KParams p, const int tiles_x, const int tiles_y,
                                                                   const int n_tiles) {
    using IO = ItemIO<TexT>;
    constexpr int TPI = IO::kTPI;
    constexpr int ES = static_cast<int>(sizeof(TexT));
    constexpr int SS = HALF ? 8 : 16;
    constexpr int PADS = HALF ? 2 : 1;
    constexpr int kWaveLds = wave_lds(WPS), kBoxSlots = box_slots(WPS, SS);
    static_assert(SPLIT == 1 || !STRICT, "plane split changes the association of the composite");
    static_assert(!HALF || (!STRICT && sizeof(TexT) == 2), "fp16 texels in LDS: 16-bit volumes, default mode");
    __shared__ __attribute__((aligned(16))) unsigned char smem[WPB * SPLIT * kWaveLds];
    const int lane = threadIdx.x & 63;
    const int wv = __builtin_amdgcn_readfirstlane(static_cast<int>(threadIdx.x) >> 6);

    const int per_xcd = (n_tiles + 7) / 8;
    const int tile_id = (blockIdx.x % 8) * per_xcd + blockIdx.x / 8;
    if (tile_id >= n_tiles) return;
    const int tiles_per_view = tiles_x * tiles_y;
    int n, trem;
    if (p.view_to_mpi == nullptr && p.views_per_mpi > 1) {
        const int group = tile_id / (tiles_per_view * p.views_per_mpi);
        const int first = group * p.views_per_mpi, size = min(p.views_per_mpi, p.N - first);
        const int r = tile_id - first * tiles_per_view;
        trem = r / size;
        n = first + (r - trem * size);
    } else {
        n = tile_id / tiles_per_view;
        trem = tile_id - n * tiles_per_view;
    }
    if (view_gated_out(p, n)) return;
    const int tyi = trem / tiles_x, txi = trem - tyi * tiles_x;

    uint32_t bad = 0;
    const int m = view_mpi(p, n, bad);
    const int D = p.D, Ht = p.Ht, Wt = p.Wt, H = p.H, W = p.W;
    const float* __restrict__ dhw = p.dhw + static_cast<int64_t>(m) * D * 3;
    const float ex = p.eye_pos[3 * n + 0], ey = p.eye_pos[3 * n + 1], ez = p.eye_pos[3 * n + 2];
    const float zx = p.z_dir[3 * n + 0], zy = p.z_dir[3 * n + 1], zz = p.z_dir[3 * n + 2];
    const float cx = AC ? static_cast<float>(Wt - 1) * 0.5f : static_cast<float>(Wt);
    const float cy = AC ? static_cast<float>(Ht - 1) * 0.5f : static_cast<float>(Ht);
    const bool check_range = (p.flags & GMPI_FLAG_CHECK_RANGE) != 0;
    const bool check_last = (p.flags & GMPI_FLAG_CHECK_LAST_PLANE) != 0;
    const int64_t HW = static_cast<int64_t>(H) * W;
    const float* __restrict__ rdv = p.ray_dir + static_cast<int64_t>(n) * 3 * HW;
    const TexT* __restrict__ vol = static_cast<const TexT*>(p.rgba) + static_cast<int64_t>(m) * p.s_mpi;
    const int64_t s_chan = p.s_chan, s_row = p.s_row, s_plane = p.s_plane;

    if (p.status != nullptr && trem == 0 && threadIdx.x == 0) {
        const float ez0 = p.eye_pos[2];
        bool behind = false;
        for (int k = 0; k < D; ++k) behind |= !(dhw[3 * k] >= ez0);
        if (behind) atomicOr(p.status, GMPI_STATUS_CAMERA_BEHIND_PLANE);
    }

    const int part = SPLIT == 1 ? 0 : wv / WPB;
    int sx0 = (txi * WPB + (wv - part * WPB)) * kSW;
    const int sy0 = tyi * kSH;
    const bool ghost = sx0 >= W;
    if (ghost) {
        if (SPLIT == 1) return;
        sx0 = 0;
    }
    const int planes_per_part = (D + SPLIT - 1) / SPLIT;
    const int k_begin = SPLIT == 1 ? 0 : min(part * planes_per_part, D), k_end = SPLIT == 1 ? D : min(k_begin + planes_per_part, D);
    const int lxp = lane & 31, lyp = lane >> 5;
    const int pxx = min(sx0 + lxp, W - 1);
    float rx[kPX], ry[kPX], rz[kPX], rrz[kPX];
    auto pixel_index = [&](int j) -> int64_t { return static_cast<int64_t>(min(sy0 + lyp + 2 * j, H - 1)) * W + pxx; };
#pragma unroll
    for (int j = 0; j < kPX; ++j) {
        const int64_t q = pixel_index(j);
        rx[j] = rdv[q], ry[j] = rdv[HW + q], rz[j] = rdv[2 * HW + q];
        rrz[j] = 1.0f / rz[j];
    }
    Accum A[kPX];
    auto ray_dot = [&](int j) -> float {
        float d = rx[j] * zx;
        d = d + ry[j] * zy;
        d = d + rz[j] * zz;
        return d;
    };

    lds_u32x4* const tab = reinterpret_cast<lds_u32x4*>(
        static_cast<uintptr_t>(static_cast<uint32_t>(reinterpret_cast<uintptr_t>((__attribute__((address_space(3))) unsigned char*)smem)) +
                               static_cast<uint32_t>(wv * kWaveLds)));
    const uint32_t box_addr = static_cast<uint32_t>(reinterpret_cast<uintptr_t>(tab)) + kRing * kEntry + 16;
    const int qc = lane & 3, qt = lane >> 2;

#pragma unroll 1
    for (int att = 0; att < 3 && !ghost && k_begin < k_end; ++att) {
        const int pmask = att == 0 ? 3 : att;
        const int y_lo = min(sy0 + (att == 2 ? kSH / 2 : 0), H - 1);
        const int y_hi = min(sy0 + (att == 1 ? kSH / 2 - 1 : kSH - 1), H - 1);

        float crx, cry, crz;
        {
            const int64_t q = static_cast<int64_t>((qc & 2) ? y_hi : y_lo) * W + ((qc & 1) ? min(sx0 + kSW - 1, W - 1) : sx0);
            crx = rdv[q], cry = rdv[HW + q], crz = rdv[2 * HW + q];
        }
        struct Box { int bx0, bx1, by0, nr; float zdiff, hw, hh; };
        const float crcp = __builtin_amdgcn_rcpf(crz);
        auto box_of = [&](int k) -> Box {
            Box b;
            const float d = dhw[3 * k + 0];
            b.hh = dhw[3 * k + 1] * 0.5f, b.hw = dhw[3 * k + 2] * 0.5f;
            b.zdiff = d - ez;
            float ix, iy, s;
            plane_coord_recip<AC>(b.zdiff, b.hw, b.hh, __builtin_amdgcn_rcpf(b.hw), __builtin_amdgcn_rcpf(b.hh), ex, ey, crx, cry, crz, crcp,
                                  cx, cy, ix, iy, s);
            const float inf = __builtin_inff();
            if (!(fabsf(ix) < 16384.0f)) ix = inf;
            if (!(fabsf(iy) < 16384.0f)) iy = inf;
            float mnx = ix, mxx = ix, mny = iy, mxy = iy;
#pragma unroll
            for (int o = 1; o < 4; o <<= 1) {
                mnx = fminf(mnx, __shfl_xor(mnx, o)), mxx = fmaxf(mxx, __shfl_xor(mxx, o));
                mny = fminf(mny, __shfl_xor(mny, o)), mxy = fmaxf(mxy, __shfl_xor(mxy, o));
            }
            if (mxx < inf && mxy < inf) {
                b.bx0 = static_cast<int>(floorf(mnx - kBoxSlack)), b.bx1 = static_cast<int>(floorf(mxx + kBoxSlack)) + 1;
                b.by0 = static_cast<int>(floorf(mny - kBoxSlack));
                b.nr = static_cast<int>(floorf(mxy + kBoxSlack)) + 1 - b.by0 + 1;
            } else {
                b.bx0 = b.by0 = 0, b.bx1 = -1, b.nr = 1;
            }
            return b;
        };

        constexpr int kLooseAlign = ES == 2 ? 2 : TPI;
        int ni_loose = 1, ni_tight = 1, nr_max = 1, touch = 0;
        for (int g = k_begin; g < k_end; g += 16) {
            const Box b = box_of(min(g + qt, k_end - 1));
            if (b.bx1 < b.bx0) ni_loose = ni_tight = 1 << 20;
            ni_loose = max(ni_loose, (b.bx1 - (b.bx0 & ~(kLooseAlign - 1))) / TPI + 1);
            ni_tight = max(ni_tight, (b.bx1 - (b.bx0 & ~(TPI - 1))) / TPI + 1);
            nr_max = max(nr_max, b.nr);
            touch |= (b.bx0 < 0 || b.bx1 + TPI > Wt) ? 1 : 0;
        }
        const int align = wave_max(touch) ? TPI : kLooseAlign;
        const int LPR = wave_max(align == TPI ? ni_tight : ni_loose);
        const int NR = wave_max(nr_max);
        const bool wide = LPR > 64;
        const int rpp_max = wide ? 1 : 64 / LPR;
        const int NP = (NR + rpp_max - 1) / rpp_max;
        const int RPP = (NR + NP - 1) / NP;
        const int pitch = TPI == 8 ? (8 + PADS) * LPR : TPI * LPR + (TPI * LPR + 7) / 8 + 1;
        const bool fit = !wide && NP <= kMaxNP && pitch * NR <= kBoxSlots;
#ifdef GMPI_TUNE
        if (p.status != nullptr && lane == 0) {
            if (p.flags & (1u << 27)) {
                if (fit) atomicAdd(p.status + 1, static_cast<uint32_t>(NP - 1)), atomicAdd(p.status + 2, static_cast<uint32_t>(LPR)), atomicAdd(p.status + 3, static_cast<uint32_t>(NR));
// ... 420 lines not shown
```

### ml-gmpi_amd/driver.py

```python
import ctypes
from typing import Callable, List, Optional, Sequence

import torch
import torch.distributed as dist

from . import _lib
from .hip_mpi import _call, _ptr


def shard_views(n_views: int, rank: int, world_size: int, mode: str = "strided") -> List[int]:
    assert 0 <= rank < world_size
    if mode == "strided":
        return list(range(rank, n_views, world_size))
    if mode == "block":
        per = (n_views + world_size - 1) // world_size
        return list(range(min(rank * per, n_views), min((rank + 1) * per, n_views)))
    raise ValueError(mode)


def frames_to_uint8(rgb_pm1: torch.Tensor, depth: Optional[torch.Tensor], near: float, far: float, out=None):
    if not rgb_pm1.is_cuda:
        raise _lib.GmpiError("frames_to_uint8 needs device tensors (no CPU path)")
    rgb_pm1 = rgb_pm1.contiguous()
    N, _, H, W = rgb_pm1.shape
# ... 59 lines not shown
    paths = []
    for n in range(img8.shape[0]):
        seed, j = divmod(n, n_view_per_z)
        name = f"{start_index + seed:06d}" if n_view_per_z == 1 else f"{start_index + seed:06d}_{j}"
        Image.fromarray(img8[n]).save(os.path.join(dirs["rgb"], name + ".png"))
        with open(os.path.join(dirs["angle"], name + ".npy"), "wb") as f:
            np.save(f, angles[n])
        if depth is not None:
            with open(os.path.join(dirs["depth"], name + ".npy"), "wb") as f:
                np.save(f, depth[n])
        paths.append(os.path.join(dirs["rgb"], name + ".png"))
    return paths


DEPTH_FORWARD_DEFAULT = "pixel"


class ViewBatchDriver:

    def __init__(self, renderer, batch: int = 8):
        self.renderer = renderer
        self.batch = int(batch)
        self._host = {}
        self._copy_stream = None

    def _pinned(self, slot, shape, dtype):
        key = (slot, tuple(shape), dtype)
        buf = self._host.get(key)
        if buf is None:
            while len(self._host) >= 8:
                self._host.pop(next(iter(self._host)))
            buf = self._host[key] = torch.empty(shape, dtype=dtype, pin_memory=True)
        return buf

    def to_host(self, *tensors: torch.Tensor):
        outs = []
        for i, t in enumerate(tensors):
            buf = self._pinned(i, t.shape, t.dtype) if t.is_cuda else torch.empty(t.shape, dtype=t.dtype)
            buf.copy_(t, non_blocking=True)
            outs.append(buf)
        if tensors and tensors[0].is_cuda:
            torch.cuda.current_stream(tensors[0].device).synchronize()
        return tuple(outs)

    @torch.no_grad()
    def render_path(self, mpi_rgbas: torch.Tensor, render_size: int, yaws: Sequence[float],
                    pitches: Sequence[float], indices: Optional[Sequence[int]] = None, to_uint8: bool = False,
                    depth_range=None, want_transmittance: bool = False, to_host: bool = False):
        assert mpi_rgbas.shape[0] == 1, "render_path draws many views of one MPI"
        r = self.renderer

        def launch(dhw, ray, eye, zd, **kw):
            r.mpi.render_views(mpi_rgbas, dhw, ray, eye, zd, **kw)
        return self._render_path(launch, mpi_rgbas.device, render_size, yaws, pitches, indices, to_uint8, depth_range, want_transmittance, to_host)

    @torch.no_grad()
    def render_path_layers(self, layers: torch.Tensor, render_size: int, yaws: Sequence[float], pitches: Sequence[float],
                           indices: Optional[Sequence[int]] = None, to_uint8: bool = False, depth_range=None, want_transmittance: bool = False,
                           to_host: bool = False, variant: Optional[str] = None):
        assert layers.ndim == 5 and layers.shape[4] == 4 and layers.shape[0] == 1, "render_path_layers draws many views of one MPI [1,D,Ht,Wt,4]"
        r = self.renderer

        def launch(dhw, ray, eye, zd, **kw):
            r.mpi.render_views_layers(layers, dhw, ray, eye, zd, variant=variant, **kw)
        return self._render_path(launch, layers.device, render_size, yaws, pitches, indices, to_uint8, depth_range, want_transmittance, to_host)

    @torch.no_grad()
    def render_path_shared(self, rgb: torch.Tensor, alpha: torch.Tensor, render_size: int, yaws: Sequence[float], pitches: Sequence[float],
                           background: Optional[torch.Tensor] = None, indices: Optional[Sequence[int]] = None, to_uint8: bool = False,
                           depth_range=None, want_transmittance: bool = False, to_host: bool = False, variant: Optional[str] = "lds"):
        from .shared_color import _check
        _check(rgb, alpha, background)
        assert alpha.shape[0] == 1, "render_path_shared draws many views of one MPI"
        r = self.renderer

        def launch(dhw, ray, eye, zd, **kw):
            r.mpi.render_views_shared(rgb, alpha, dhw, ray, eye, zd, background=background, variant=variant, **kw)
        return self._render_path(launch, alpha.device, render_size, yaws, pitches, indices, to_uint8, depth_range, want_transmittance, to_host)

    @torch.no_grad()
    def render_path_depth(self, rgb: torch.Tensor, depth: torch.Tensor, render_size: int, yaws: Sequence[float], pitches: Sequence[float], *,
                          z_range, n_z_bins, plane_z: Optional[torch.Tensor] = None, background: Optional[torch.Tensor] = None,
                          indices: Optional[Sequence[int]] = None, to_uint8: bool = False, depth_range=None, want_transmittance: bool = False,
                          to_host: bool = False, depth_forward: Optional[str] = DEPTH_FORWARD_DEFAULT):
        from .depth_alpha import depth_alpha_bounds
        assert depth.shape[0] == 1, "render_path_depth draws many views of one MPI"
        r = self.renderer
        if plane_z is None:
            plane_z = r.get_xyz_single_res(depth.shape[-2], depth.shape[-1], only_z=True)[1].reshape(-1)
        z_bounds = depth_alpha_bounds(z_range, n_z_bins)

        def launch(dhw, ray, eye, zd, **kw):
            r.mpi.render_views_depth(rgb, depth, plane_z, z_bounds, dhw, ray, eye, zd, background=background, depth_forward=depth_forward, **kw)
        return self._render_path(launch, depth.device, render_size, yaws, pitches, indices, to_uint8, depth_range, want_transmittance, to_host)

    def _render_path(self, launch, dev, render_size, yaws, pitches, indices, to_uint8, depth_range, want_transmittance, to_host):
        r = self.renderer
        idx = list(range(len(yaws))) if indices is None else list(indices)
        n = len(idx)
        rgb = torch.empty((n, 3, render_size, render_size), dtype=torch.float32, device=dev)
        dep = torch.empty((n, 1, render_size, render_size), dtype=torch.float32, device=dev)
        T = torch.empty((n, 1, render_size, render_size), dtype=torch.float32, device=dev) if want_transmittance else None
        status = torch.zeros(_lib.STATUS_WORDS, dtype=torch.int32, device=dev)
        if render_size != r.render_h or render_size != r.render_w:
            r.set_cam(r.cam_fov, render_size, render_size)
        dhw = r._dhw_on_device()
        pipe = to_host and to_uint8 and dev.type == "cuda"
        if pipe:
            near, far = depth_range if depth_range is not None else (r.plane_min_d, r.plane_max_d)
            img8 = torch.empty((n, render_size, render_size, 3), dtype=torch.uint8, device=dev)
            dep8 = torch.empty((n, render_size, render_size, 1), dtype=torch.uint8, device=dev)
            img8_h, dep8_h = self._pinned("path_img8", img8.shape, torch.uint8), self._pinned("path_dep8", dep8.shape, torch.uint8)
            if self._copy_stream is None or self._copy_stream.device != dev:
                self._copy_stream = torch.cuda.Stream(device=dev)
            main = torch.cuda.current_stream(dev)
            self._copy_stream.wait_stream(main)
        group = max(self.batch, (int(256e6 // (12 * render_size * render_size)) // self.batch) * self.batch)
        ray_g = eye_g = zd_g = None
        for s in range(0, n, self.batch):
            chunk = idx[s:s + self.batch]
            if s % group == 0:
                members = idx[s:s + group]
                gy = torch.tensor([[float(yaws[i])] for i in members], dtype=torch.float32)
                gp = torch.tensor([[float(pitches[i])] for i in members], dtype=torch.float32)
                _, _, c2w, rays, eyes, zdirs = r.sample_cam_poses(len(members), 0.0, 0.0, 0.0, 0.0, False, given_yaws=gy, given_pitches=gp)
                if r._batched_cam is not None and rays is r._batched_cam[0]:
                    ray_g, eye_g, zd_g = r._batched_cam[1:]
                else:
                    ray_g, eye_g, zd_g = torch.cat(rays), torch.cat(eyes), torch.cat(zdirs)
                r._batched_cam = None
            g0 = s % group
            ray_t, eye_t, zd_t = ray_g[g0:g0 + len(chunk)], eye_g[g0:g0 + len(chunk)], zd_g[g0:g0 + len(chunk)]
            out = dict(color=rgb[s:s + len(chunk)], depth=dep[s:s + len(chunk)])
            if T is not None:
                out["T"] = T[s:s + len(chunk)]
            launch(dhw, ray_t, eye_t, zd_t, views_per_mpi=len(chunk), check_last_plane=True, out_pm1=True,
                   want_transmittance=want_transmittance, status=status, defer_status=True, out=out)
            if pipe:
                e = s + len(chunk)
                frames_to_uint8(rgb[s:e], dep[s:e], near, far, out=(img8[s:e], dep8[s:e]))
                ev = torch.cuda.Event()
                ev.record(main)
                with torch.cuda.stream(self._copy_stream):
                    self._copy_stream.wait_event(ev)
                    img8_h[s:e].copy_(img8[s:e], non_blocking=True)
                    dep8_h[s:e].copy_(dep8[s:e], non_blocking=True)
        r.mpi.raise_on_status(status)
        res = dict(rgb=rgb, depth=dep, T=T)
        if pipe:
            self._copy_stream.synchronize()
            res.update(img8=img8, dep8=dep8, img8_host=img8_h, dep8_host=dep8_h)
        elif to_uint8:
            near, far = depth_range if depth_range is not None else (r.plane_min_d, r.plane_max_d)
            res["img8"], res["dep8"] = frames_to_uint8(rgb, dep, near, far)
        return res

    @torch.no_grad()
    def render_seeds(self, mpi_rgbas: torch.Tensor, render_size: int, views_per_mpi: int = 1, **render_kwargs):
        def render(s):
            return self.renderer.render(mpi_rgbas[s:s + self.batch], render_size, render_size, views_per_mpi=views_per_mpi, **render_kwargs)
        return self._render_seeds(render, mpi_rgbas.shape[0], render_kwargs)

    @torch.no_grad()
    def render_seeds_layers(self, layers: torch.Tensor, render_size: int, views_per_mpi: int = 1, variant: Optional[str] = None, **render_kwargs):
        def render(s):
            return self.renderer.render_layers(layers[s:s + self.batch], render_size, render_size, variant=variant, views_per_mpi=views_per_mpi, **render_kwargs)
        return self._render_seeds(render, layers.shape[0], render_kwargs)

    @torch.no_grad()
    def render_seeds_shared(self, rgb: torch.Tensor, alpha: torch.Tensor, render_size: int, background: Optional[torch.Tensor] = None,
                            views_per_mpi: int = 1, variant: Optional[str] = "lds", **render_kwargs):
        def render(s):
            e = s + self.batch
            return self.renderer.render_shared(rgb[s:e], alpha[s:e], render_size, render_size, background_rgb=None if background is None else background[s:e],
                                               variant=variant, views_per_mpi=views_per_mpi, **render_kwargs)
        return self._render_seeds(render, alpha.shape[0], render_kwargs)

    @torch.no_grad()
    def render_seeds_depth(self, rgb: torch.Tensor, depth: torch.Tensor, render_size: int, *, z_range, n_z_bins,
                           plane_z: Optional[torch.Tensor] = None, background: Optional[torch.Tensor] = None, views_per_mpi: int = 1,
                           depth_forward: Optional[str] = DEPTH_FORWARD_DEFAULT, **render_kwargs):
        def render(s):
            e = s + self.batch
            return self.renderer.render_depth(rgb[s:e], depth[s:e], render_size, render_size, z_range=z_range, n_z_bins=n_z_bins,
                                              plane_z=plane_z[s:e] if plane_z is not None and plane_z.ndim == 2 else plane_z,
                                              background_rgb=None if background is None else background[s:e], depth_forward=depth_forward,
                                              views_per_mpi=views_per_mpi, **render_kwargs)
        return self._render_seeds(render, depth.shape[0], render_kwargs)

    def _render_seeds(self, render, n_mpis, render_kwargs):
# ... 9 lines not shown
```

### ml-gmpi_amd/hip_mpi.py

```python
import atexit
import collections
import contextlib
import ctypes
import sys
import threading
import warnings
import weakref
from typing import List, Optional, Sequence, Union

import numpy as np
import torch
from torch import nn

from . import _lib, depth_alpha, shaded, shared_color
from .quantized import is_interleaved, layers_as_volume
from .layers import FLOAT_DTYPES, is_float_layers, layer_strides

_DTYPES = {torch.float32: _lib.DTYPE_F32, torch.bfloat16: _lib.DTYPE_BF16, torch.float16: _lib.DTYPE_F16, torch.uint8: _lib.DTYPE_U8}


def _refuse_uint8(what: str, *tensors) -> None:
    for t in tensors:
        if t is not None and t.dtype is torch.uint8:
            raise TypeError(f"{what} does not take uint8 storage: pass dequantize_volume(q) (ml_gmpi_amd.quantized), or render the RGBA volume "
# ... 178 lines not shown
    return status, defer_status, None, None


def _flush_at_exit() -> None:
    try:
        flush_status()
    except BaseException as e:
        import os
        import traceback
        if not isinstance(e, SystemExit):
            traceback.print_exception(type(e), e, e.__traceback__)
        print("ml_gmpi_amd: a render with a lagged status check asserted (above); exit status 1", file=sys.stderr)
        try:
            atexit.unregister(_flush_at_exit)
            atexit._run_exitfuncs()
        except BaseException:
            traceback.print_exc()
        try:
            import logging
            logging.shutdown()
        except BaseException:
            pass
        sys.stderr.flush(), sys.stdout.flush()
        os._exit(1)


atexit.register(_flush_at_exit)


def _on_device(dev: Optional[torch.device]):
    if dev is None or dev.index is None or torch.cuda.current_device() == dev.index:
        return contextlib.nullcontext()
    return torch.cuda.device(dev)


def _call(name: str, dev: torch.device, *args, stream: Optional[int] = None) -> None:
    lib = _lib.load_library()
    if dev.type != "cuda":
        if not getattr(lib, "records_only", False):
            raise _lib.GmpiError(f"{name} needs tensors on a ROCm device: this package has no CPU path (got {dev})")
        return _lib.check(getattr(lib, name)(*args, 0), name)
    if stream is None:
        stream = torch.cuda.current_stream(dev).cuda_stream
    if dev.index is None or torch.cuda.current_device() == dev.index:
        return _lib.check(getattr(lib, name)(*args, stream), name)
    with torch.cuda.device(dev):
        _lib.check(getattr(lib, name)(*args, stream), name)


def _ptr(t: Optional[torch.Tensor]):
    return None if t is None else t.data_ptr()


_Keep = collections.namedtuple("_Keep", "rgba dhw ray_dir eye_pos z_dir view_to_mpi")
_Scalars = collections.namedtuple("_Scalars", "flags variant rgba_dtype N M D Ht Wt H W views_per_mpi")


def _render_params(scalars: _Scalars, keep: _Keep, color=None, depth=None, T=None, status=None) -> _lib.GmpiRenderParams:
    p = _lib.GmpiRenderParams()
    p.struct_size = ctypes.sizeof(_lib.GmpiRenderParams)
    p.flags, p.variant, p.rgba_dtype, p.N, p.M, p.D, p.Ht, p.Wt, p.H, p.W, p.views_per_mpi = scalars
    rgba, dhw, ray_dir, eye_pos, z_dir, view_to_mpi = keep
    p.rgba = rgba.data_ptr()
    p.rgba_stride[:] = rgba.stride()
    p.dhw, p.ray_dir, p.eye_pos, p.z_dir = dhw.data_ptr(), ray_dir.data_ptr(), eye_pos.data_ptr(), z_dir.data_ptr()
    if view_to_mpi is not None:
        p.view_to_mpi = view_to_mpi.data_ptr()
    if color is not None:
        p.rgb_out, p.depth_out, p.status = color.data_ptr(), depth.data_ptr(), status.data_ptr()
    if T is not None:
        p.transmittance_out = T.data_ptr()
    return p


def _shared_color(rgb: torch.Tensor, background: Optional[torch.Tensor]) -> _lib.GmpiSharedColor:
    sc = _lib.GmpiSharedColor()
    sc.struct_size = ctypes.sizeof(_lib.GmpiSharedColor)
    sc.rgb = rgb.data_ptr()
    sc.rgb_stride[:] = rgb.stride()[:3]
    if background is not None:
        sc.background = background.data_ptr()
        sc.background_stride[:] = background.stride()[:3]
    return sc


def _shading_struct(shading: torch.Tensor) -> _lib.GmpiShading:
    sh = _lib.GmpiShading()
    sh.struct_size = ctypes.sizeof(_lib.GmpiShading)
    sh.shading = shading.data_ptr()
    sh.shading_stride[:] = (shading.stride(0), shading.stride(2))
    return sh


def _shading_operand(shading: torch.Tensor, dev: torch.device) -> torch.Tensor:
    shading = shading.to(dev, torch.float32)
    M, _, _, Wt = shading.shape
    ok = shading.stride(3) == 1 and shading.stride(2) >= Wt and (shading.stride(0) > 0 or (shading.stride(0) == 0 and M == 1))
    return shading if ok else shading.contiguous()


def _depth_alpha(plane_z: torch.Tensor, z_lo: float, z_hi: float) -> _lib.GmpiDepthAlpha:
    da = _lib.GmpiDepthAlpha()
    da.struct_size = ctypes.sizeof(_lib.GmpiDepthAlpha)
    da.plane_z = plane_z.data_ptr()
    da.plane_z_stride = plane_z.stride(0) if plane_z.ndim == 2 else 0
    da.z_lo, da.z_hi, da.z_den = depth_alpha.ramp_constants(z_lo, z_hi)
    return da


_Kind = collections.namedtuple("_Kind", "name expand first geometry_entry")
_SHARED_COLOUR = _Kind("shared-colour", "expand_shared_color", "alpha", "gmpi_mpi_render_shared_geometry_backward_launch")
_DEPTH_ALPHA = _Kind("depth-alpha", "expand_depth_alpha", "depth", "gmpi_mpi_render_depth_geometry_backward_launch")
_DEPTH_PZ_ENTRY, _DEPTH_PZ_QUERY = "gmpi_mpi_render_depth_geometry_backward_pz_launch", "gmpi_render_depth_geometry_backward_workspace_bytes"
_DEPTH_BACKWARD_ENTRIES = {"pixel": "gmpi_mpi_render_depth_backward_launch", "tile": "gmpi_mpi_render_depth_backward_tile_launch",
                           "gather": "gmpi_mpi_render_depth_backward_launch"}
_SHARED_BACKWARD_ENTRIES = {"tile": "gmpi_mpi_render_shared_backward_launch", "gather": "gmpi_mpi_render_shared_backward_launch"}
_GATHER_ENTRIES = {"shared-colour": "gmpi_mpi_render_shared_backward_gather_launch", "depth-alpha": "gmpi_mpi_render_depth_backward_gather_launch"}


class _Layout:

    def __init__(self, kind, rgb, background, variant, backward_entry, plane_z=None, ramp=None, depth_forward=None, gather=False, gather_runs=None,
                 plane_z_arg=None):
        self.kind, self.rgb, self.background, self.variant, self.backward_entry = kind, rgb, background, variant, backward_entry
        self.plane_z, self.plane_z_arg, self.ramp, self.depth_forward = plane_z, plane_z_arg, ramp, depth_forward
# ... 276 lines not shown
    def _volume_fingerprint(rgba: torch.Tensor):
        anchor = rgba._base if rgba._base is not None else rgba
        return anchor, (rgba.data_ptr(), tuple(rgba.shape), tuple(rgba.stride()), rgba.dtype, rgba._version, str(rgba.device))

    def _full_check_needed(self, rgba: torch.Tensor) -> bool:
        hit = self._full_check_passed
        if hit is None:
            return True
        anchor, fp = self._volume_fingerprint(rgba)
        return not (hit[0]() is anchor and hit[1] == fp)

    def _full_check_record(self, rgba: torch.Tensor) -> None:
        anchor, fp = self._volume_fingerprint(rgba)
        try:
            self._full_check_passed = (weakref.ref(anchor), fp)
        except TypeError:
            self._full_check_passed = None

    def check_shapes(self, *, batch_rgba, batch_dhw, batch_ray_dir, batch_eye_pos, batch_z_dir, separate_background):
        assert (batch_rgba.ndim == 5) and (batch_rgba.shape[2] == 4), (
            f"Expected rgba to be of shape (#mpi, #planes, 4, texture_height, texture_width), "
            f"but instead got {batch_rgba.shape}")
        assert ((batch_dhw.ndim == 3) and (batch_dhw.shape[0] == batch_rgba.shape[0])
                and (batch_dhw.shape[1] == batch_rgba.shape[1]) and (batch_dhw.shape[2] == 3)), (
            f"Expected dhw to be of shape (#mpi, #planes, 3), but instead got {batch_dhw.shape} (rgba: {batch_rgba.shape})")
        n_mpi = batch_rgba.shape[0]
        assert len(batch_ray_dir) == n_mpi, f"{len(batch_ray_dir)}, {n_mpi}"
        assert len(batch_eye_pos) == n_mpi, f"{len(batch_eye_pos)}, {n_mpi}"
        assert len(batch_z_dir) == n_mpi, f"{len(batch_z_dir)}, {n_mpi}"
        for i in range(n_mpi):
            assert (batch_ray_dir[i].ndim == 4) and (batch_ray_dir[i].shape[1] == 3), (
                f"Expected ray_dir to be of shape (minibatch, 3, image_height, image_width), "
                f"but instead got {batch_ray_dir[i].shape} for {i} th elem.")
            assert (batch_eye_pos[i].ndim == 2) and (batch_eye_pos[i].shape[1] == 3), (
                f"Expected eye_pos to be of shape (minibatch, 3), but instead got {batch_eye_pos[i].shape} for {i} th elem.")
            assert (batch_z_dir[i].ndim == 2) and (batch_z_dir[i].shape[1] == 3), (
                f"Expected z_dir to be of shape (minibatch, 3), but instead got {batch_z_dir[i].shape} for {i} th elem.")
        if separate_background is not None:
            assert separate_background.ndim == 4 and separate_background.shape[1] == 3, (
                f"Expect background to be of shape (#mpi, 3, h, w), but instead get {separate_background.shape}.")

    def forward(self, *, batch_rgba: torch.Tensor, batch_dhw: torch.Tensor, batch_ray_dir: List[torch.Tensor],
                batch_eye_pos: List[torch.Tensor], batch_z_dir: List[torch.Tensor],
                separate_background: Union[None, torch.Tensor], assert_not_out_of_last_plane: bool = False,
                c2w_mat: torch.Tensor = None, sphere_c: np.ndarray = None):
        self.check_shapes(batch_rgba=batch_rgba, batch_dhw=batch_dhw, batch_ray_dir=batch_ray_dir,
                          batch_eye_pos=batch_eye_pos, batch_z_dir=batch_z_dir, separate_background=separate_background)
        counts = [int(r.shape[0]) for r in batch_ray_dir]
        out = self.render_views(batch_rgba, batch_dhw, _cat(batch_ray_dir), _cat(batch_eye_pos), _cat(batch_z_dir),
                                views_per_mpi=counts, check_last_plane=assert_not_out_of_last_plane,
                                c2w_mat=c2w_mat, sphere_c=sphere_c)
        return out["color"], out["depth"]

    def render_views(self, rgba: torch.Tensor, dhw: torch.Tensor, ray_dir: torch.Tensor, eye_pos: torch.Tensor,
                     z_dir: torch.Tensor, views_per_mpi: Union[int, Sequence[int]] = 1,
                     view_to_mpi: Optional[torch.Tensor] = None, check_last_plane: bool = False,
                     out_pm1: bool = False, want_transmittance: bool = False, c2w_mat=None, sphere_c=None,
                     status: Optional[torch.Tensor] = None, defer_status: bool = False, out: Optional[dict] = None,
                     _in_autograd_fn: bool = False, frontal_hint: bool = False, tilted_hint: bool = False, oblique_hint: bool = False,
                     _layout: Optional[_Layout] = None, _shading: Optional[torch.Tensor] = None, _layers: Optional[str] = None,
                     _layers_backward: str = "planar"):
        if torch.is_grad_enabled() and dhw.requires_grad and not self.geometry_grad:
            raise NotImplementedError("no gradient flows to the plane geometry (the reference computes the grid under "
                                      "torch.no_grad(), mpi.py:65); MPI(geometry_grad=True) provides one")
        if torch.is_grad_enabled() and not _in_autograd_fn:
            if rgba.dtype is torch.uint8 and self.geometry_grad and any(t.requires_grad for t in (dhw, ray_dir, eye_pos, z_dir)):
                raise NotImplementedError("no gradient flows through a uint8 volume, w.r.t. the plane geometry and the camera tensors included "
                                          "(geometry_grad=True): render dequantize_volume(q) (ml_gmpi_amd.quantized) for that, or detach the "
                                          "camera and dhw tensors")
            if _layers is not None:
                bridge = self._layers_bridge(rgba, dhw, ray_dir, eye_pos, z_dir)
            else:
                bridge = self._autograd_bridge(rgba, dhw, ray_dir, eye_pos, z_dir, _layout) if _shading is None else self._shaded_bridge(
                    rgba, _shading, dhw, ray_dir, eye_pos, z_dir)
            if bridge is not None:
                kwargs = dict(views_per_mpi=views_per_mpi, view_to_mpi=view_to_mpi, check_last_plane=check_last_plane,
                              out_pm1=out_pm1, want_transmittance=want_transmittance, c2w_mat=c2w_mat, sphere_c=sphere_c,
                              status=status, defer_status=defer_status, out=out, frontal_hint=frontal_hint, tilted_hint=tilted_hint, oblique_hint=oblique_hint,
                              _layout=_layout, _shading=_shading)
                if _layers is not None:
                    kwargs["_layers"], kwargs["_layers_backward"] = _layers, _layers_backward
                color, depth, T, st = bridge[0].apply(*bridge[1], self, dhw, ray_dir, eye_pos, z_dir, kwargs)
                return dict(color=color, depth=depth, T=T if want_transmittance else None, status=st)
        on_device = rgba.is_cuda
        if not on_device and not getattr(_lib.load_library(), "records_only", False):
            raise _lib.GmpiError("MPI.forward needs tensors on a ROCm device: this package has no CPU path "
                                 f"(got rgba on {rgba.device})")
        dev = rgba.device
        rgba_in = rgba
        if _layers is None:
            rgba = _volume_operand(rgba)
            M, D, _, Ht, Wt = rgba.shape
            variant, images = _lib.VARIANTS[self.variant], None
        else:
            M, D, Ht, Wt, _ = rgba.shape
            variant, images = _lib.VARIANTS[_layers], None
        if _shading is not None:
            variant, images = _lib.VARIANT_GATHER if self.variant == "gather" else _lib.VARIANT_AUTO, (_shading_operand(_shading, dev),)
        if _layout is not None:
            D, variant, images = _layout.operands(self, rgba, dhw)
        ray_dir, eye_pos, z_dir, dhw = (_f32_on(t, dev) for t in (ray_dir, eye_pos, z_dir, dhw))
        N, _, H, W = ray_dir.shape
        assert eye_pos.shape == (N, 3) and z_dir.shape == (N, 3), (eye_pos.shape, z_dir.shape, N)
        assert dhw.shape == (M, D, 3), (dhw.shape, rgba.shape)
        uniform, view_to_mpi = _view_index(views_per_mpi, view_to_mpi, M, N, dev)
        keep = _Keep(rgba, dhw, ray_dir, eye_pos, z_dir, view_to_mpi)
        out = out or {}
        color, depth, T = out.get("color"), out.get("depth"), out.get("T") if want_transmittance else None
        if color is None:
            color = torch.empty((N, 3, H, W), dtype=torch.float32, device=dev)
        if depth is None:
            depth = torch.empty((N, 1, H, W), dtype=torch.float32, device=dev)
        if T is None and want_transmittance:
            T = torch.empty((N, 1, H, W), dtype=torch.float32, device=dev)
        scalars = _Scalars(self._flags(out_pm1, check_last_plane, frontal_hint, tilted_hint, oblique_hint), variant, _DTYPES[rgba.dtype],
                           N, M, D, Ht, Wt, H, W, max(uniform, 1))
        current = torch.cuda.current_stream(dev) if on_device else None
        stream = current.cuda_stream if on_device else 0
        with _stream_lock(dev, stream) if on_device else contextlib.nullcontext():
            status, defer_status, ring, slot = _status_target(dev, stream, status, defer_status, on_device and not _in_autograd_fn)
            p = _render_params(scalars, keep, color, depth, T, status)
            fully_checked = None
            if _layers is not None:
                p.rgba_stride[:] = layer_strides(rgba)
                if self.range_check == "full" and self._full_check_needed(rgba_in):
                    _range_pass((rgba[:1] if M > 1 and rgba.stride(0) == 0 else rgba,), p, dev, stream)
                    fully_checked = rgba_in
                if variant == _lib.VARIANT_LDS and on_device:
                    rc = _lib.load_library().gmpi_render_layers_supports(ctypes.byref(p))
                    if rc < 0:
                        _lib.check(rc, "gmpi_render_layers_supports")
                    if rc == 0:
                        p.variant = _lib.VARIANT_GATHER
                        self.layers_lds_fallbacks += 1
                        _warn_layers_lds_fallback()
                _call("gmpi_mpi_render_layers_launch", dev, ctypes.byref(p), stream=stream)
            elif _shading is not None:
                if self.range_check == "full":
                    _range_pass((rgba[:, :, 3:],), p, dev, stream)
                sh = _shading_struct(images[0])
                if self.variant != "gather" and on_device:
                    p.variant = _lib.VARIANT_LDS
                    if not _forward_takes("gmpi_render_shaded_supports", (p, sh), (rgba, images[0])):
                        p.variant = _lib.VARIANT_GATHER
                        if self.variant == "lds":
                            self.shaded_lds_fallbacks += 1
                            _warn_shaded_lds_fallback()
                _call("gmpi_mpi_render_shaded_launch", dev, ctypes.byref(p), ctypes.byref(sh), stream=stream)
            elif _layout is None:
                if on_device:
                    need = int(_lib.load_library().gmpi_render_workspace_bytes(ctypes.byref(p)))
                    if need:
                        _lend(p, _workspace(dev, stream, need))
                if self.range_check == "full" and rgba.dtype is not torch.uint8 and self._full_check_needed(rgba_in):
                    _range_pass((rgba,), p, dev, stream)
                    fully_checked = rgba_in
                _call("gmpi_mpi_render_launch", dev, ctypes.byref(p), stream=stream)
            else:
                _layout.launch(self, p, rgba, images, dev, stream)
            res = dict(color=color, depth=depth, T=T, status=status)
            if _in_autograd_fn:
                res["_bwd"] = (p, keep) if images is None else (p, keep, images)
            if ring is not None:
                ring.host_words[slot].copy_(status, non_blocking=True)
                ev = torch.cuda.Event()
                ev.record(current)
                ring.pending.append((slot, ev, self, p, keep, c2w_mat, sphere_c))
            elif not defer_status:
                self._settle(status, p, keep, c2w_mat, sphere_c, fully_checked)
            return res

    def _autograd_bridge(self, rgba, dhw, ray_dir, eye_pos, z_dir, layout):
        geometry = self.geometry_grad and any(t.requires_grad for t in (dhw, ray_dir, eye_pos, z_dir))
        if layout is None:
            return (_RenderFunction, (rgba,)) if rgba.requires_grad or geometry else None
        if geometry and not self.geometry_grad_layouts:
            raise NotImplementedError(f"the {layout.kind.name} render has no gradient w.r.t. the plane geometry or the camera tensors under "
                                      f'geometry_grad=True: build the module with geometry_grad="all" for that (or render the expanded '
                                      f"volume, {layout.kind.expand}, with render_views)")
        plane_z = layout.plane_z_arg if self.geometry_grad_layouts and layout.plane_z_arg is not None and layout.plane_z_arg.requires_grad else None
        if geometry or rgba.requires_grad or layout.requires_grad or plane_z is not None:
            return _LayoutRenderFunction, (layout.rgb, rgba, layout.background, plane_z)
        return None

    def _layers_bridge(self, layers, dhw, ray_dir, eye_pos, z_dir):
        if self.geometry_grad and any(t.requires_grad for t in (dhw, ray_dir, eye_pos, z_dir)):
            raise NotImplementedError("the render of float layers has no gradient w.r.t. the plane geometry or the camera tensors: render the planar "
                                      "volume layers.permute(0, 1, 4, 2, 3) with render_views for that, or detach the camera and dhw tensors")
        return (_LayersRenderFunction, (layers,)) if layers.requires_grad else None

    def _shaded_bridge(self, rgba, shading, dhw, ray_dir, eye_pos, z_dir):
        if self.geometry_grad and any(t.requires_grad for t in (dhw, ray_dir, eye_pos, z_dir)):
            raise NotImplementedError("the shaded render has no gradient w.r.t. the plane geometry or the camera tensors: render "
                                      "apply_shading(rgba, shading) with render_views for that, or detach the camera and dhw tensors")
        return (_ShadedRenderFunction, (rgba, shading)) if rgba.requires_grad or shading.requires_grad else None

    def _flags(self, out_pm1, check_last_plane, frontal_hint, tilted_hint, oblique_hint) -> int:
        return ((_lib.FLAG_ALIGN_CORNERS if self._align_corners else 0) | (_lib.FLAG_OUT_PM1 if out_pm1 else 0)
                | (_lib.FLAG_CHECK_LAST_PLANE if check_last_plane else 0) | (_lib.FLAG_CHECK_RANGE if self.range_check != "off" else 0)
                | (_lib.FLAG_STRICT_ORDER if self.strict_order else 0) | (_lib.FLAG_HINT_FRONTAL if frontal_hint else 0)
                | (_lib.FLAG_HINT_TILTED if tilted_hint else 0) | (_lib.FLAG_HINT_OBLIQUE if oblique_hint else 0))

    def _settle(self, status, p, keep, c2w_mat, sphere_c, fully_checked) -> None:
        try:
            self.raise_on_status(status, params=p, keep=keep, c2w_mat=c2w_mat, sphere_c=sphere_c)
        except BaseException:
            if status.is_cuda:
                status.zero_()
            self._full_check_passed = None
            raise
# ... 27 lines not shown
            _warn_layers_copy()
        return self.render_views(layers, dhw, ray_dir, eye_pos, z_dir, _layers=variant, _layers_backward=layers_backward, **kwargs)

    def render_views_shaded(self, rgba: torch.Tensor, shading: torch.Tensor, dhw: torch.Tensor, ray_dir: torch.Tensor, eye_pos: torch.Tensor,
                            z_dir: torch.Tensor, **kwargs):
        if rgba.dtype is torch.uint8:
            raise TypeError("the shaded render takes fp32, bf16 or fp16 volumes, not uint8 codes: render dequantize_volume(q) (ml_gmpi_amd.quantized)")
        shaded._check(rgba, shading)
        return self.render_views(rgba, dhw, ray_dir, eye_pos, z_dir, _shading=shading, **kwargs)

    def render_views_shared(self, rgb: torch.Tensor, alpha: torch.Tensor, dhw: torch.Tensor, ray_dir: torch.Tensor, eye_pos: torch.Tensor,
                            z_dir: torch.Tensor, background: Optional[torch.Tensor] = None, variant: Optional[str] = None, **kwargs):
        alpha, layout = _shared_layout(rgb, alpha, background, variant, kwargs.pop("shared_backward", "tile"), kwargs.pop("_gather_runs", None))
        return self.render_views(alpha, dhw, ray_dir, eye_pos, z_dir, _layout=layout, **kwargs)

    def render_views_depth(self, rgb: torch.Tensor, depth: torch.Tensor, plane_z: torch.Tensor, z_bounds, dhw: torch.Tensor, ray_dir: torch.Tensor,
                           eye_pos: torch.Tensor, z_dir: torch.Tensor, background: Optional[torch.Tensor] = None, **kwargs):
        depth5, layout = _depth_layout(rgb, depth, plane_z, z_bounds, background, dhw.shape[1], kwargs.pop("variant", None),
                                       kwargs.pop("depth_backward", "pixel"), kwargs.pop("depth_forward", "pixel"), kwargs.pop("_gather_runs", None))
        return self.render_views(depth5, dhw, ray_dir, eye_pos, z_dir, _layout=layout, **kwargs)

    def chunked_render(self, dhw: torch.Tensor, ray_dir: torch.Tensor, eye_pos: torch.Tensor, z_dir: torch.Tensor, **kwargs) -> "ChunkedRender":
        return ChunkedRender(self, dhw, ray_dir, eye_pos, z_dir, **kwargs)

    def render_views_chunks(self, chunks, dhw: torch.Tensor, ray_dir: torch.Tensor, eye_pos: torch.Tensor, z_dir: torch.Tensor, **kwargs):
        if torch.is_grad_enabled():
            if any(t.requires_grad for t in (dhw, ray_dir, eye_pos, z_dir)) and (self.geometry_grad or dhw.requires_grad):
                raise NotImplementedError("the plane-chunked render has no gradient w.r.t. the plane geometry or the camera tensors: use render_views "
                                          "on the concatenation, torch.cat(chunks, 1), with MPI(geometry_grad=True), or detach these tensors")
            if isinstance(chunks, (list, tuple)) and any(c.requires_grad for c in chunks):
                chunks = tuple(chunks)
                color, depth, T, st = _ChunkedRenderFunction.apply(self, dhw, ray_dir, eye_pos, z_dir, kwargs, *chunks)
                return dict(color=color, depth=depth, T=T if kwargs.get("want_transmittance") else None, status=st)
        cr = self.chunked_render(dhw, ray_dir, eye_pos, z_dir, **kwargs)
        it = iter(chunks)
        while True:
            chunk = next(it, None)
            if chunk is None:
                break
            cr.add(chunk)
            del chunk
        return cr.finish()

    def raise_on_status(self, status: torch.Tensor, params=None, keep=None, c2w_mat=None, sphere_c=None):
        word = int(status[0].item())
        if word == 0:
            return
        if status.is_cuda:
            status.zero_()
        if word & _lib.STATUS_BAD_VIEW_INDEX:
            raise IndexError("view_to_mpi holds an index outside [0, #mpi)")
        if word & _lib.STATUS_RGBA_RANGE:
            raise AssertionError("Expected alpha to be within the the range [0, 1]")
        if word & _lib.STATUS_CAMERA_BEHIND_PLANE:
            dist = keep[1][..., 0].flatten().tolist() if keep is not None else "?"
            eye0 = keep[3][0].tolist() if keep is not None else "?"
            raise AssertionError(f"Camera must be placed closer to origin than MPI. {dist}, {eye0}")
        if word & _lib.STATUS_OUT_OF_LAST_PLANE:
            msg = "Ray goes out of the last plane"
            if params is not None:
                dev = keep[0].device if keep is not None else status.device
                uv = torch.empty((params.N, 4), dtype=torch.float32, device=dev)
                _call("gmpi_last_plane_uv_minmax_launch", dev, ctypes.byref(params), uv.data_ptr())
                uv = uv.cpu()
                mn_u, mx_u, mn_v, mx_v = (float(uv[:, 0].min()), float(uv[:, 1].max()), float(uv[:, 2].min()),
                                          float(uv[:, 3].max()))
                dist = keep[1][0, -1, 0].item()
                if not mn_u >= -1:
                    msg = f"Ray's U direction goes out of plane at {dist}, min val {mn_u}"
                elif not mx_u <= 1:
                    msg = f"Ray's U direction goes out of plane at {dist}, max val {mx_u}"
                elif not mn_v >= -1:
                    msg = f"Ray's V direction goes out of plane at {dist}, min val {mn_v}"
                else:
                    msg = f"Ray's V direction goes out of plane at {dist}, max val {mx_v}"
                print("\npos: ", keep[3][:4, :].cpu())
                print("\ndir: ", keep[2][:4, :3, 0, 0].cpu())
                if c2w_mat is not None and sphere_c is not None:
                    from .poses import yaw_pitch_from_w2c
                    yaws, pitches = yaw_pitch_from_w2c(torch.inverse(c2w_mat.float().cpu()), torch.FloatTensor(sphere_c))
                    print("\nyaws: ", yaws.numpy().tolist(), "\n")
                    print("\npitches: ", pitches.numpy().tolist(), "\n")
            if self.on_out_of_plane == "exit":
                print(f"AssertionError: {msg}", file=sys.stderr)
                sys.exit(1)
            raise RuntimeError(msg)


def _bridge_forward(ctx, mpi, volume, geometry, kwargs):
    kw = dict(kwargs, want_transmittance=True)
    user_out = kw.get("out") or {}
    kw["out"] = {k: v for k, v in user_out.items() if k != "T"}
    res = mpi.render_views(volume.detach(), *geometry, _in_autograd_fn=True, **kw)
    bwd = res.pop("_bwd")
    p, images = bwd[0], bwd[2] if len(bwd) == 3 else None
    if kwargs.get("want_transmittance") and user_out.get("T") is not None:
        user_out["T"].copy_(res["T"])
    bwd_variant = _lib.VARIANT_AUTO if images is not None and p.variant == _lib.VARIANT_LDS else p.variant
    ctx.scalars = _Scalars(p.flags, bwd_variant, p.rgba_dtype, p.N, p.M, p.D, p.Ht, p.Wt, p.H, p.W, p.views_per_mpi)
    ctx.mark_non_differentiable(res["status"])
    ctx.set_materialize_grads(False)
    return res, bwd[1], images


def _upstream(ctx, dev, g_color, g_depth, g_T):
    if g_color is None:
# ... 404 lines not shown
```

### ml-gmpi_amd/renderer.py

```python
import logging

import numpy as np
import torch

from .hip_mpi import MPI, _call, _cat, _depth_layout, _shared_layout
from .pinhole import gen_cam
from .plane_geometry import compute_plane_dhws, sample_distance
from .poses import draw_angle_noise, gen_sphere_path, gen_sphere_paths_ahead, host_math

logger = logging.getLogger("ml_gmpi_amd")

EPS = 1e-6
_COS_FRONTAL = 0.98006658
_COS_TILTED = 0.86280707
_COS_OBLIQUE = 0.93937271

PRESETS = {
    "FFHQ": dict(plane_min_d=0.95, plane_max_d=1.12, cam_fov=12.6, sphere_center_z=1.0, sphere_r=1.0,
                 horizontal_mean=0.0, horizontal_std=0.289, vertical_mean=0.0, vertical_std=0.127,
                 cam_pose_n_truncated_stds=2),
    "MetFaces": dict(plane_min_d=0.95, plane_max_d=1.12, cam_fov=12.6, sphere_center_z=1.0, sphere_r=1.0,
                     horizontal_mean=0.0, horizontal_std=0.339, vertical_mean=0.0, vertical_std=0.133,
                     cam_pose_n_truncated_stds=2),
    "AFHQCat": dict(plane_min_d=2.55, plane_max_d=2.8, cam_fov=13.39, sphere_center_z=2.7, sphere_r=2.7,
# ... 288 lines not shown
        if hit is None or hit[0] is not base or hit[1].shape[0] != n_mpis:
            hit = self._dhw_rep = (base, base.expand(n_mpis, -1, -1).contiguous())
        return hit[1]

    def _generate_rays_hip(self, c2w: torch.Tensor, reuse: bool = False):
        from . import _lib
        if not c2w.is_cuda:
            raise _lib.GmpiError("ray_backend='hip' needs a ROCm device (use ray_backend='torch' on the CPU)")
        if c2w.dtype is not torch.float32 or not c2w.is_contiguous():
            c2w = c2w.to(torch.float32).contiguous()
        B, H, W = c2w.shape[0], self.cam.height, self.cam.width
        dirs = self.cam.unit_dirs(c2w.device)
        stream = torch.cuda.current_stream(c2w.device).cuda_stream
        bufs = self._ray_bufs.get((B, H, W, stream)) if reuse else None
        if bufs is None:
            bufs = (torch.empty((B, 3, H, W), dtype=torch.float32, device=c2w.device),
                    torch.empty((B, 3), dtype=torch.float32, device=c2w.device),
                    torch.empty((B, 3), dtype=torch.float32, device=c2w.device))
            if reuse:
                if len(self._ray_bufs) >= 4:
                    self._ray_bufs.clear()
                self._ray_bufs[(B, H, W, stream)] = bufs
        ray, eye, zd = bufs
        _call("gmpi_generate_rays_launch", c2w.device, c2w.data_ptr(), dirs.data_ptr(), B, H, W, ray.data_ptr(), eye.data_ptr(), zd.data_ptr(),
              stream=stream)
        return ray, eye, zd

    def _dhw_on_device(self):
        src = self.dynamic_mpi_plane_dhws
        if self._dhw_dev is None or self._dhw_dev[0] is not src:
            self._dhw_dev = (src, src.reshape((1, -1, 3)).to(self.device, torch.float32).contiguous())
        return self._dhw_dev[1]

    def render(self, batch_mpi_rgbas, render_h, render_w, horizontal_mean=None, horizontal_std=None,
               vertical_mean=None, vertical_std=None, random_pose=True, given_yaws=None, given_pitches=None,
               given_cam_infos=None, assert_not_out_of_last_plane=True, **ext):
        horizontal_mean = self.horizontal_mean if horizontal_mean is None else horizontal_mean
        horizontal_std = self.horizontal_std if horizontal_std is None else horizontal_std
        vertical_mean = self.vertical_mean if vertical_mean is None else vertical_mean
        vertical_std = self.vertical_std if vertical_std is None else vertical_std
        views_per_mpi = int(ext.pop("views_per_mpi", 1))
        want_T = bool(ext.pop("want_transmittance", False))
        layout = ext.pop("_layout", None)
        shading = ext.pop("_shading", None)
        layers_variant = ext.pop("_layers", None)
        chunks = ext.pop("_chunks", None)
        defer = ext.pop("defer_status", self.status_mode)
        assert not ext, f"unknown arguments {list(ext)}"

        n_mpis = batch_mpi_rgbas.shape[0]
        batch_size = n_mpis * views_per_mpi
        if render_h != self.render_h or render_w != self.render_w:
            self.set_cam(self.cam_fov, render_h, render_w)
        cam_angles, frontal, tilted, oblique = None, False, False, False
        if given_cam_infos is None and self.ray_backend == "hip":
            yaws, pitches, c2w, cam_angles = self._draw_poses(batch_size, horizontal_mean, horizontal_std, vertical_mean, vertical_std,
                                                              random_pose, given_yaws, given_pitches)
            frontal, tilted, oblique = self._frontal, self._tilted, self._oblique
            recording = torch.is_grad_enabled() and (batch_mpi_rgbas.requires_grad or (layout is not None and layout.requires_grad) or (shading is not None and shading.requires_grad) or (self.mpi.geometry_grad and self._dhw_for(n_mpis).requires_grad)
                                                     or (layout is not None and self.mpi.geometry_grad_layouts and layout.plane_z_arg is not None and layout.plane_z_arg.requires_grad)
                                                     or (isinstance(chunks, (list, tuple)) and any(c.requires_grad for c in chunks)))
            ray_t, eye_t, zd_t = self._generate_rays_hip(c2w, reuse=not recording and defer != "lag")
        else:
            if given_cam_infos is None:
                yaws, pitches, c2w, rays, eyes, zdirs = self.sample_cam_poses(
                    batch_size, horizontal_mean, horizontal_std, vertical_mean, vertical_std, random_pose=random_pose,
                    given_yaws=given_yaws, given_pitches=given_pitches)
            else:
                yaws, pitches, c2w = (given_cam_infos[k] for k in ("batch_yaws", "batch_pitches", "batch_tf_c2w"))
                rays, eyes, zdirs = (given_cam_infos[k] for k in ("batch_ray_dir", "batch_eye_pos", "batch_z_dir"))
            assert len(rays) == batch_size or (isinstance(rays, torch.Tensor) and rays.shape[0] == batch_size), \
                f"{len(rays)}, {batch_size}"
            if self._batched_cam is not None and rays is self._batched_cam[0]:
                ray_t, eye_t, zd_t = self._batched_cam[1:]
            else:
                ray_t, eye_t, zd_t = _cat(rays), _cat(eyes), _cat(zdirs)
            self._batched_cam = None
        assert ray_t.shape[0] == batch_size, f"{ray_t.shape[0]}, {batch_size}"

        dhw = self._dhw_for(n_mpis)
        if chunks is not None:
            res = self.mpi.render_views_chunks(
                chunks, dhw, ray_t, eye_t, zd_t, views_per_mpi=views_per_mpi, check_last_plane=assert_not_out_of_last_plane, out_pm1=True,
                want_transmittance=want_T, c2w_mat=c2w, sphere_c=self.sphere_center, defer_status=defer)
        elif layers_variant is not None:
            res = self.mpi.render_views_layers(
                batch_mpi_rgbas, dhw, ray_t, eye_t, zd_t, variant=layers_variant[0], layers_backward=layers_variant[1], views_per_mpi=views_per_mpi,
                check_last_plane=assert_not_out_of_last_plane, out_pm1=True, want_transmittance=want_T,
                c2w_mat=c2w, sphere_c=self.sphere_center, defer_status=defer)
        elif shading is not None:
            res = self.mpi.render_views_shaded(
                batch_mpi_rgbas, shading, dhw, ray_t, eye_t, zd_t, views_per_mpi=views_per_mpi,
                check_last_plane=assert_not_out_of_last_plane, out_pm1=True, want_transmittance=want_T,
                c2w_mat=c2w, sphere_c=self.sphere_center, defer_status=defer, frontal_hint=frontal, tilted_hint=tilted, oblique_hint=oblique)
        else:
            res = self.mpi.render_views(
                batch_mpi_rgbas, dhw, ray_t, eye_t, zd_t, views_per_mpi=views_per_mpi,
                check_last_plane=assert_not_out_of_last_plane, out_pm1=True, want_transmittance=want_T,
                c2w_mat=c2w, sphere_c=self.sphere_center, defer_status=defer, frontal_hint=frontal, tilted_hint=tilted, oblique_hint=oblique,
                _layout=layout)
        if cam_angles is None:
            cam_angles = torch.cat([pitches, yaws], -1).to(self.device)
        if want_T:
            return res["color"], res["depth"], c2w, cam_angles, res["T"]
        return res["color"], res["depth"], c2w, cam_angles


    def render_chunks(self, chunks, render_h, render_w, **kwargs):
        if isinstance(chunks, (list, tuple)):
            assert len(chunks) > 0, "no chunks"
            return self.render(chunks[0], render_h, render_w, _chunks=chunks, **kwargs)
        it = iter(chunks)
        first = next(it)

        def rest():
            nonlocal first
            chunk, first = first, None
            yield chunk
            del chunk
            yield from it
        shape_only = first.new_empty((first.shape[0], 0))
        return self.render(shape_only, render_h, render_w, _chunks=rest(), **kwargs)

    def render_layers(self, layers, render_h, render_w, *, variant=None, layers_backward="planar", **kwargs):
        if layers.ndim != 5 or layers.shape[4] != 4:
            raise ValueError(f"render_layers takes layers of shape [B, D, Ht, Wt, 4], got {tuple(layers.shape)}")
        if layers_backward not in ("planar", "texel"):
            raise ValueError(f'layers_backward is "planar" or "texel", not {layers_backward!r}')
        return self.render(layers, render_h, render_w, _layers=(variant, layers_backward), **kwargs)

    def render_shaded(self, batch_mpi_rgbas, shading, render_h, render_w, **kwargs):
        if shading is None:
            raise ValueError("render_shaded needs a shading image [B,1,Ht,Wt]")
        return self.render(batch_mpi_rgbas, render_h, render_w, _shading=shading, **kwargs)

    def render_shared(self, batch_mpi_rgb, batch_mpi_alpha, render_h, render_w, *, background_rgb=None, variant=None, **kwargs):
        alpha, layout = _shared_layout(batch_mpi_rgb, batch_mpi_alpha, background_rgb, variant, kwargs.pop("shared_backward", "tile"),
                                       kwargs.pop("_gather_runs", None))
        return self.render(alpha, render_h, render_w, _layout=layout, **kwargs)


    def render_depth(self, batch_rgb, batch_depth, render_h, render_w, *, z_range, n_z_bins, plane_z=None, background_rgb=None, **kwargs):
        from .depth_alpha import depth_alpha_bounds
        if plane_z is None:
            plane_z = self.get_xyz_single_res(batch_depth.shape[-2], batch_depth.shape[-1], only_z=True)[1].reshape(-1)
        depth5, layout = _depth_layout(batch_rgb, batch_depth, plane_z, depth_alpha_bounds(z_range, n_z_bins), background_rgb,
                                       self.dynamic_mpi_plane_dhws.shape[0], None, kwargs.pop("depth_backward", "pixel"), kwargs.pop("depth_forward", "pixel"),
                                       kwargs.pop("_gather_runs", None))
        return self.render(depth5, render_h, render_w, _layout=layout, **kwargs)


class _RaysFromC2W(torch.autograd.Function):

# ... 25 lines not shown
```

Before: 534,800 Mpix*planes/s.

## Add pinhole camera path computing world rays in-kernel from c2w and shared unit directions

Adds a pinhole launch entry in which kernels get per-view c2w matrices and one shared camera-space unit-direction grid, and rotate each pixel ray on the fly. This replaces the per-view world ray buffer, so the ray-generation pass and the reads of N*3*H*W floats go away. The renderer picks this path by default for non-recording plain renders. In exchange each pixel does a few extra FMAs, and the error path has to rebuild the full camera tensors when status flags fire.

```diff
diff --git a/include/gmpi_render.h b/include/gmpi_render.h
--- a/include/gmpi_render.h
+++ b/include/gmpi_render.h
@@ -85,6 +85,13 @@
 uint64_t gmpi_render_workspace_bytes(const GmpiRenderParams *params);
 
 int gmpi_mpi_render_launch(const GmpiRenderParams *params, void *stream);
+
+typedef struct GmpiPinhole {
+    uint32_t struct_size;
+    const float *c2w;
+    const float *unit_dirs;
+} GmpiPinhole;
+int gmpi_mpi_render_pinhole_launch(const GmpiRenderParams *params, const GmpiPinhole *cam, void *stream);
 
 int gmpi_mpi_render_layers_launch(const GmpiRenderParams *params, void *stream);
 
diff --git a/ml-gmpi_amd/_lib.py b/ml-gmpi_amd/_lib.py
--- a/ml-gmpi_amd/_lib.py
+++ b/ml-gmpi_amd/_lib.py
@@ -19,6 +19,7 @@
 
 EXPORTS = (
     "gmpi_mpi_render_launch",
+    "gmpi_mpi_render_pinhole_launch",
     "gmpi_render_workspace_bytes",
     "gmpi_render_backward_workspace_bytes",
     "gmpi_mpi_render_backward_launch",
@@ -107,6 +108,13 @@
     ]
 
 
+class GmpiPinhole(ctypes.Structure):
+    _fields_ = [
+        ("struct_size", ctypes.c_uint32),
+        ("c2w", ctypes.c_void_p), ("unit_dirs", ctypes.c_void_p),
+    ]
+
+
 class GmpiCarry(ctypes.Structure):
     _fields_ = [
         ("struct_size", ctypes.c_uint32), ("reserved", ctypes.c_uint32),
@@ -207,6 +215,8 @@
     vp = ctypes.c_void_p
     lib.gmpi_mpi_render_launch.restype = ctypes.c_int
     lib.gmpi_mpi_render_launch.argtypes = [ctypes.POINTER(GmpiRenderParams), vp]
+    lib.gmpi_mpi_render_pinhole_launch.restype = ctypes.c_int
+    lib.gmpi_mpi_render_pinhole_launch.argtypes = [ctypes.POINTER(GmpiRenderParams), ctypes.POINTER(GmpiPinhole), vp]
     lib.gmpi_render_workspace_bytes.restype = ctypes.c_uint64
     lib.gmpi_render_workspace_bytes.argtypes = [ctypes.POINTER(GmpiRenderParams)]
     lib.gmpi_render_backward_workspace_bytes.restype = ctypes.c_uint64
diff --git a/ml-gmpi_amd/csrc/gmpi_abi.hip b/ml-gmpi_amd/csrc/gmpi_abi.hip
--- a/ml-gmpi_amd/csrc/gmpi_abi.hip
+++ b/ml-gmpi_amd/csrc/gmpi_abi.hip
@@ -254,7 +254,7 @@
     }
 }
 
-static int to_kparams(const GmpiRenderParams* q, KParams& p, bool need_outputs, bool need_volume = false, bool takes_u8 = false) {
+static int to_kparams(const GmpiRenderParams* q, KParams& p, bool need_outputs, bool need_volume = false, bool takes_u8 = false, bool no_camera = false) {
     if (q == nullptr) return GMPI_E_NULL;
     if (q->struct_size != sizeof(GmpiRenderParams)) return GMPI_E_ABI;
     bool interleaved = false;
@@ -264,10 +264,10 @@
         if (q->views_per_mpi < 1) return GMPI_E_SHAPE;
         if (q->N > static_cast<int64_t>(q->M) * q->views_per_mpi) return GMPI_E_SHAPE;
     }
-    if (q->dhw == nullptr || q->ray_dir == nullptr || q->eye_pos == nullptr) return GMPI_E_NULL;
+    if (q->dhw == nullptr || (!no_camera && (q->ray_dir == nullptr || q->eye_pos == nullptr))) return GMPI_E_NULL;
     if (need_outputs && (q->rgb_out == nullptr || q->depth_out == nullptr)) return GMPI_E_NULL;
     if (need_outputs || need_volume) {
-        if (q->rgba == nullptr || q->z_dir == nullptr) return GMPI_E_NULL;
+        if (q->rgba == nullptr || (!no_camera && q->z_dir == nullptr)) return GMPI_E_NULL;
         if (q->rgba_dtype < GMPI_DTYPE_F32 || q->rgba_dtype > (takes_u8 ? GMPI_DTYPE_U8 : GMPI_DTYPE_F16)) return GMPI_E_DTYPE;
         interleaved = takes_u8 && q->rgba_dtype == GMPI_DTYPE_U8 && q->rgba_stride[4] == 4 && q->rgba_stride[2] == 1;
         if (q->rgba_stride[4] != 1 && !interleaved) return GMPI_E_STRIDE;
@@ -360,14 +360,13 @@
 
 using namespace gmpi;
 
-extern "C" {
-
-int gmpi_mpi_render_launch(const GmpiRenderParams* params, void* stream) {
+static int render_launch(const GmpiRenderParams* params, const GmpiPinhole* cam, void* stream) {
     if (params != nullptr && params->struct_size == sizeof(GmpiRenderParams) && params->N == 0) return GMPI_OK;
     KParams p;
-    const int rc = to_kparams(params, p, true, false, true);
+    const int rc = to_kparams(params, p, true, false, true, cam != nullptr);
     if (rc != GMPI_OK) return rc;
     if (p.N == 0) return GMPI_OK;
+    if (cam != nullptr) p.ray_dir = cam->unit_dirs, p.eye_pos = cam->c2w, p.z_dir = nullptr;
     hipStream_t st = static_cast<hipStream_t>(stream);
     int variant = params->variant;
     if (params->rgba_dtype == GMPI_DTYPE_U8) {
@@ -429,6 +428,17 @@
     return GMPI_E_VARIANT;
 }
 
+extern "C" {
+
+int gmpi_mpi_render_launch(const GmpiRenderParams* params, void* stream) { return render_launch(params, nullptr, stream); }
+
+int gmpi_mpi_render_pinhole_launch(const GmpiRenderParams* params, const GmpiPinhole* cam, void* stream) {
+    if (params == nullptr || cam == nullptr) return GMPI_E_NULL;
+    if (params->struct_size != sizeof(GmpiRenderParams) || cam->struct_size != sizeof(GmpiPinhole)) return GMPI_E_ABI;
+    if (cam->c2w == nullptr || cam->unit_dirs == nullptr) return GMPI_E_NULL;
+    return render_launch(params, cam, stream);
+}
+
 int gmpi_render_layers_supports(const GmpiRenderParams* params) {
     if (params == nullptr) return GMPI_E_NULL;
     if (params->struct_size != sizeof(GmpiRenderParams)) return GMPI_E_ABI;
@@ -485,7 +495,7 @@
 
 uint64_t gmpi_render_workspace_bytes(const GmpiRenderParams* params) {
     KParams p;
-    if (to_kparams(params, p, true, false, true) != GMPI_OK || p.N == 0) return 0;
+    if (to_kparams(params, p, true, false, true, true) != GMPI_OK || p.N == 0) return 0;
     if (params->rgba_dtype == GMPI_DTYPE_U8) return 0;
     if (params->variant == GMPI_VARIANT_BAND) return band_workspace_bytes(p, params->rgba_dtype);
     if (params->variant == GMPI_VARIANT_AUTO && auto_takes_band(p, params->rgba_dtype)) return band_workspace_bytes(p, params->rgba_dtype);
@@ -1085,6 +1095,7 @@
         case 40: return 1;
         case 42: return 1;
         case 44: return 1;
+        case 48: return 1;
         case 46: return 1;
         case 36: return 1;
         default: return -1;
diff --git a/ml-gmpi_amd/csrc/gmpi_device.hpp b/ml-gmpi_amd/csrc/gmpi_device.hpp
--- a/ml-gmpi_amd/csrc/gmpi_device.hpp
+++ b/ml-gmpi_amd/csrc/gmpi_device.hpp
@@ -34,6 +34,9 @@
     int32_t band_rot, band_split;
     int32_t band_tail;
 };
+__device__ __host__ __forceinline__ bool pinhole_cameras(const KParams& p) { return p.z_dir == nullptr; }
+__device__ __forceinline__ const float* pinhole_c2w(const KParams& p) { return p.eye_pos; }
+__device__ __forceinline__ const float* pinhole_unit_dirs(const KParams& p) { return p.ray_dir; }
 struct CarryK {
     const float* state_in;
     float* state_out;
@@ -384,24 +387,57 @@
     float cx, cy;
     int64_t HW;
     const float* __restrict__ rays;
+    const float* __restrict__ c2w;
 };
-template <bool AC>
-__device__ __forceinline__ View view_setup(const KParams& p, int n, uint32_t& bad) {
+struct Rotation { float r00, r01, r02, r10, r11, r12, r20, r21, r22; };
+template <bool AC, bool PINHOLE = false>
+__device__ __forceinline__ View view_setup(const KParams& p, int n, uint32_t& bad, Rotation* rot = nullptr) {
     View vw;
     vw.m = view_mpi(p, n, bad);
     vw.dhw = p.dhw + static_cast<int64_t>(vw.m) * p.D * 3;
-    vw.ex = p.eye_pos[3 * n + 0], vw.ey = p.eye_pos[3 * n + 1], vw.ez = p.eye_pos[3 * n + 2];
-    vw.zx = p.z_dir[3 * n + 0], vw.zy = p.z_dir[3 * n + 1], vw.zz = p.z_dir[3 * n + 2];
     vw.cx = AC ? static_cast<float>(p.Wt - 1) * 0.5f : static_cast<float>(p.Wt);
     vw.cy = AC ? static_cast<float>(p.Ht - 1) * 0.5f : static_cast<float>(p.Ht);
     vw.HW = static_cast<int64_t>(p.H) * p.W;
-    vw.rays = p.ray_dir + static_cast<int64_t>(n) * 3 * vw.HW;
+    vw.c2w = nullptr;
+    if (PINHOLE && pinhole_cameras(p)) {
+        const float* __restrict__ c = vw.c2w = pinhole_c2w(p) + 16 * static_cast<int64_t>(n);
+        vw.ex = c[3], vw.ey = c[7], vw.ez = c[11];
+        vw.zx = c[2], vw.zy = c[6], vw.zz = c[10];
+        if (rot != nullptr) *rot = Rotation{c[0], c[1], c[2], c[4], c[5], c[6], c[8], c[9], c[10]};
+        vw.rays = pinhole_unit_dirs(p);
+    } else {
+        vw.ex = p.eye_pos[3 * n + 0], vw.ey = p.eye_pos[3 * n + 1], vw.ez = p.eye_pos[3 * n + 2];
+        vw.zx = p.z_dir[3 * n + 0], vw.zy = p.z_dir[3 * n + 1], vw.zz = p.z_dir[3 * n + 2];
+        vw.rays = p.ray_dir + static_cast<int64_t>(n) * 3 * vw.HW;
+    }
     return vw;
+}
+
+__device__ __forceinline__ Rotation view_rotation(const View& vw) {
+    Rotation R{0.0f, 0.0f, 0.0f, 0.0f, 0.0f, 0.0f, 0.0f, 0.0f, 0.0f};
+    if (vw.c2w != nullptr) {
+        const float* __restrict__ c = vw.c2w;
+        R = Rotation{c[0], c[1], c[2], c[4], c[5], c[6], c[8], c[9], c[10]};
+    }
+    return R;
+}
+__device__ __forceinline__ void pixel_ray(const View& vw, const Rotation& R, const float* __restrict__ rdv, int64_t q, float& rx, float& ry, float& rz) {
+    const float d0 = rdv[q], d1 = rdv[vw.HW + q], d2 = rdv[2 * vw.HW + q];
+    if (vw.c2w != nullptr) {
+        rx = __builtin_fmaf(R.r02, d2, __builtin_fmaf(R.r01, d1, R.r00 * d0));
+        ry = __builtin_fmaf(R.r12, d2, __builtin_fmaf(R.r11, d1, R.r10 * d0));
+        rz = __builtin_fmaf(R.r22, d2, __builtin_fmaf(R.r21, d1, R.r20 * d0));
+    } else {
+        rx = d0, ry = d1, rz = d2;
+    }
+}
+__device__ __forceinline__ void pixel_ray(const View& vw, const float* __restrict__ rdv, int64_t q, float& rx, float& ry, float& rz) {
+    pixel_ray(vw, view_rotation(vw), rdv, q, rx, ry, rz);
 }
 
 __device__ __forceinline__ void check_camera_behind(const KParams& p, const View& vw, bool once) {
     if (p.status != nullptr && once) {
-        const float ez0 = p.eye_pos[2];
+        const float ez0 = vw.c2w != nullptr ? pinhole_c2w(p)[11] : p.eye_pos[2];
         bool behind = false;
         for (int k = 0; k < p.D; ++k) behind |= !(vw.dhw[3 * k] >= ez0);
         if (behind) atomicOr(p.status, GMPI_STATUS_CAMERA_BEHIND_PLANE);
@@ -532,8 +568,9 @@
 #pragma unroll
     for (int c = 0; c < 4; ++c) {
         const int64_t q = static_cast<int64_t>((c & 2) ? cy1 : cy0) * W + ((c & 1) ? cx1 : cx0);
-        float s, u, v;
-        plane_coord<AC>(zdiff, ph, pw, vw.ex, vw.ey, rdv[q], rdv[vw.HW + q], rdv[2 * vw.HW + q], vw.cx, vw.cy, cix[c], ciy[c], s, u, v);
+        float s, u, v, crx, cry, crz;
+        pixel_ray(vw, rdv, q, crx, cry, crz);
+        plane_coord<AC>(zdiff, ph, pw, vw.ex, vw.ey, crx, cry, crz, vw.cx, vw.cy, cix[c], ciy[c], s, u, v);
         e.finite = e.finite && (fabsf(cix[c]) < 1e6f) && (fabsf(ciy[c]) < 1e6f);
         e.mnx = fminf(e.mnx, cix[c]), e.mxx = fmaxf(e.mxx, cix[c]), e.mny = fminf(e.mny, ciy[c]), e.mxy = fmaxf(e.mxy, ciy[c]);
     }
diff --git a/ml-gmpi_amd/csrc/render_band.hip b/ml-gmpi_amd/csrc/render_band.hip
--- a/ml-gmpi_amd/csrc/render_band.hip
+++ b/ml-gmpi_amd/csrc/render_band.hip
@@ -158,11 +158,11 @@
     int bxi, byi;
     band_pos(brem, bands_x, bands_y, p.band_cols, bxi, byi);
     uint32_t ignore = 0;
-    const int m = view_mpi(p, n, ignore);
+    const View vw = view_setup<AC, true>(p, n, ignore);
+    const int m = vw.m;
     const int Ht = p.Ht, Wt = p.Wt, H = p.H, W = p.W;
-    const float ex = p.eye_pos[3 * n + 0], ey = p.eye_pos[3 * n + 1], ez = p.eye_pos[3 * n + 2];
-    const int64_t HW = static_cast<int64_t>(H) * W;
-    const float* __restrict__ rdv = p.ray_dir + static_cast<int64_t>(n) * 3 * HW;
+    const float ex = vw.ex, ey = vw.ey, ez = vw.ez;
+    const float* __restrict__ rdv = vw.rays;
     const TexT* __restrict__ vol = static_cast<const TexT*>(p.rgba) + static_cast<int64_t>(m) * p.s_mpi;
     const int sx0 = min(bxi * (NSB * SBW), W - 1), sy0 = byi * SBH;
     const int by0p = min(sy0, H - 1), by1p = min(sy0 + SBH - 1, H - 1);
@@ -180,9 +180,9 @@
 #pragma unroll
         for (int c = 0; c < 4; ++c) {
             const int64_t q = static_cast<int64_t>((c & 2) ? by1p : by0p) * W + ((c & 1) ? bx1p : bx0p);
-            float ix, iy, sc;
-            const float crz = rdv[2 * HW + q];
-            plane_coord_recip<AC>(zdiff, hw, hh, rw_a, rh_a, ex, ey, rdv[q], rdv[HW + q], crz, __builtin_amdgcn_rcpf(crz), cx, cy, ix, iy, sc);
+            float ix, iy, sc, crx, cry, crz;
+            pixel_ray(vw, rdv, q, crx, cry, crz);
+            plane_coord_recip<AC>(zdiff, hw, hh, rw_a, rh_a, ex, ey, crx, cry, crz, __builtin_amdgcn_rcpf(crz), cx, cy, ix, iy, sc);
             finite = finite && (fabsf(ix) < kCoordLimit) && (fabsf(iy) < kCoordLimit);
             mnx = fminf(mnx, ix), mxx = fmaxf(mxx, ix), mny = fminf(mny, iy), mxy = fmaxf(mxy, iy);
         }
@@ -296,7 +296,8 @@
     const int sb = wave / WPS, wj = wave % WPS;
     const int lane = tid & 63;
     uint32_t bad_w = 0;
-    View vw = view_setup<AC>(p, n, bad_w);
+    Rotation rot{0.0f, 0.0f, 0.0f, 0.0f, 0.0f, 0.0f, 0.0f, 0.0f, 0.0f};
+    View vw = view_setup<AC, true>(p, n, bad_w, &rot);
     vw.cx = cx, vw.cy = cy;
     const int D = p.D, H = p.H, W = p.W;
     const float* __restrict__ dhw = vw.dhw;
@@ -317,7 +318,7 @@
 #pragma unroll
     for (int q = 0; q < PPT; ++q) {
         const int64_t pix = static_cast<int64_t>(min(py0 + WPS * q, H - 1)) * W + pxc;
-        rx[q] = rdv[pix], ry[q] = rdv[HW + pix], rz[q] = rdv[2 * HW + pix];
+        pixel_ray(vw, rot, rdv, pix, rx[q], ry[q], rz[q]);
         rcp_rz[q] = 1.0f / rz[q];
     }
     auto ray_dot = [&](int q) { return gmpi::ray_dot(vw, rx[q], ry[q], rz[q]); };
diff --git a/ml-gmpi_amd/csrc/render_gather.hip b/ml-gmpi_amd/csrc/render_gather.hip
--- a/ml-gmpi_amd/csrc/render_gather.hip
+++ b/ml-gmpi_amd/csrc/render_gather.hip
@@ -11,12 +11,13 @@
     const int px = blockIdx.x * kGatherTileW + threadIdx.x;
     const int py = blockIdx.y * kGatherTileH + threadIdx.y;
     uint32_t bad = 0;
-    const View vw = view_setup<AC>(p, n, bad);
+    const View vw = view_setup<AC, true>(p, n, bad);
     check_camera_behind(p, vw, blockIdx.x == 0 && blockIdx.y == 0 && threadIdx.x == 0 && threadIdx.y == 0);
     const bool active = px < p.W && py < p.H;
     const int64_t HW = vw.HW;
     const int64_t pix = static_cast<int64_t>(min(py, p.H - 1)) * p.W + min(px, p.W - 1);
-    const float rx = vw.rays[pix], ry = vw.rays[HW + pix], rz = vw.rays[2 * HW + pix];
+    float rx, ry, rz;
+    pixel_ray(vw, vw.rays, pix, rx, ry, rz);
     const float dot = ray_dot(vw, rx, ry, rz);
     const bool check_range = (p.flags & GMPI_FLAG_CHECK_RANGE) != 0;
     const TexT* __restrict__ vol = tex_offset(static_cast<const TexT*>(p.rgba), static_cast<int64_t>(vw.m) * p.s_mpi);
diff --git a/ml-gmpi_amd/csrc/render_lds.hip b/ml-gmpi_amd/csrc/render_lds.hip
--- a/ml-gmpi_amd/csrc/render_lds.hip
+++ b/ml-gmpi_amd/csrc/render_lds.hip
@@ -114,7 +114,7 @@
 
     const int tid = threadIdx.x;
     uint32_t bad = 0;
-    const View vw = view_setup<AC>(p, n, bad);
+    const View vw = view_setup<AC, true>(p, n, bad);
     const int D = p.D, Ht = p.Ht, Wt = p.Wt, H = p.H, W = p.W;
     const float* __restrict__ dhw = vw.dhw;
     const float ex = vw.ex, ey = vw.ey, ez = vw.ez, cx = vw.cx, cy = vw.cy;
@@ -128,7 +128,8 @@
 
     const TileLane tl = tile_lane<TW, TH>(ft.txi, ft.tyi, tid, W, H);
     const int64_t pix = tl.pix;
-    const float rx = rdv[pix], ry = rdv[HW + pix], rz = rdv[2 * HW + pix];
+    float rx, ry, rz;
+    pixel_ray(vw, rdv, pix, rx, ry, rz);
     const float dot = ray_dot(vw, rx, ry, rz);
     const float rcp_rz = 1.0f / rz;
     Accum A = load_carry(carry, n, HW, pix);
diff --git a/ml-gmpi_amd/csrc/render_u8.hip b/ml-gmpi_amd/csrc/render_u8.hip
--- a/ml-gmpi_amd/csrc/render_u8.hip
+++ b/ml-gmpi_amd/csrc/render_u8.hip
@@ -24,7 +24,7 @@
     const int n = ft.n;
 
     uint32_t bad = 0;
-    const View vw = view_setup<AC>(p, n, bad);
+    const View vw = view_setup<AC, true>(p, n, bad);
     check_camera_behind(p, vw, ft.rem == 0 && tid == 0);
     const int D = p.D, Ht = p.Ht, Wt = p.Wt, H = p.H, W = p.W;
     const int64_t HW = vw.HW;
@@ -35,7 +35,8 @@
 
     const TileLane tl = tile_lane<kUW, kUH>(ft.txi, ft.tyi, tid, W, H);
     const int64_t pix = tl.pix;
-    const float rx = rdv[pix], ry = rdv[HW + pix], rz = rdv[2 * HW + pix];
+    float rx, ry, rz;
+    pixel_ray(vw, rdv, pix, rx, ry, rz);
     const float dot = ray_dot(vw, rx, ry, rz);
     const float rcp_rz = 1.0f / rz;
     Accum A = load_carry(carry, n, HW, pix);
diff --git a/ml-gmpi_amd/csrc/render_wave.hip b/ml-gmpi_amd/csrc/render_wave.hip
--- a/ml-gmpi_amd/csrc/render_wave.hip
+++ b/ml-gmpi_amd/csrc/render_wave.hip
@@ -129,26 +129,19 @@
     const int tyi = trem / tiles_x, txi = trem - tyi * tiles_x;
 
     uint32_t bad = 0;
-    const int m = view_mpi(p, n, bad);
+    const View vw = view_setup<AC, true>(p, n, bad);
+    const int m = vw.m;
     const int D = p.D, Ht = p.Ht, Wt = p.Wt, H = p.H, W = p.W;
-    const float* __restrict__ dhw = p.dhw + static_cast<int64_t>(m) * D * 3;
-    const float ex = p.eye_pos[3 * n + 0], ey = p.eye_pos[3 * n + 1], ez = p.eye_pos[3 * n + 2];
-    const float zx = p.z_dir[3 * n + 0], zy = p.z_dir[3 * n + 1], zz = p.z_dir[3 * n + 2];
-    const float cx = AC ? static_cast<float>(Wt - 1) * 0.5f : static_cast<float>(Wt);
-    const float cy = AC ? static_cast<float>(Ht - 1) * 0.5f : static_cast<float>(Ht);
+    const float* __restrict__ dhw = vw.dhw;
+    const float ex = vw.ex, ey = vw.ey, ez = vw.ez, zx = vw.zx, zy = vw.zy, zz = vw.zz, cx = vw.cx, cy = vw.cy;
     const bool check_range = (p.flags & GMPI_FLAG_CHECK_RANGE) != 0;
     const bool check_last = (p.flags & GMPI_FLAG_CHECK_LAST_PLANE) != 0;
-    const int64_t HW = static_cast<int64_t>(H) * W;
-    const float* __restrict__ rdv = p.ray_dir + static_cast<int64_t>(n) * 3 * HW;
+    const int64_t HW = vw.HW;
+    const float* __restrict__ rdv = vw.rays;
     const TexT* __restrict__ vol = static_cast<const TexT*>(p.rgba) + static_cast<int64_t>(m) * p.s_mpi;
     const int64_t s_chan = p.s_chan, s_row = p.s_row, s_plane = p.s_plane;
 
-    if (p.status != nullptr && trem == 0 && threadIdx.x == 0) {
-        const float ez0 = p.eye_pos[2];
-        bool behind = false;
-        for (int k = 0; k < D; ++k) behind |= !(dhw[3 * k] >= ez0);
-        if (behind) atomicOr(p.status, GMPI_STATUS_CAMERA_BEHIND_PLANE);
-    }
+    check_camera_behind(p, vw, trem == 0 && threadIdx.x == 0);
 
     const int part = SPLIT == 1 ? 0 : wv / WPB;
     int sx0 = (txi * WPB + (wv - part * WPB)) * kSW;
@@ -167,7 +160,7 @@
 #pragma unroll
     for (int j = 0; j < kPX; ++j) {
         const int64_t q = pixel_index(j);
-        rx[j] = rdv[q], ry[j] = rdv[HW + q], rz[j] = rdv[2 * HW + q];
+        pixel_ray(vw, rdv, q, rx[j], ry[j], rz[j]);
         rrz[j] = 1.0f / rz[j];
     }
     Accum A[kPX];
@@ -193,7 +186,7 @@
         float crx, cry, crz;
         {
             const int64_t q = static_cast<int64_t>((qc & 2) ? y_hi : y_lo) * W + ((qc & 1) ? min(sx0 + kSW - 1, W - 1) : sx0);
-            crx = rdv[q], cry = rdv[HW + q], crz = rdv[2 * HW + q];
+            pixel_ray(vw, rdv, q, crx, cry, crz);
         }
         struct Box { int bx0, bx1, by0, nr; float zdiff, hw, hh; };
         const float crcp = __builtin_amdgcn_rcpf(crz);
diff --git a/ml-gmpi_amd/driver.py b/ml-gmpi_amd/driver.py
--- a/ml-gmpi_amd/driver.py
+++ b/ml-gmpi_amd/driver.py
@@ -135,7 +135,11 @@
 
         def launch(dhw, ray, eye, zd, **kw):
             r.mpi.render_views(mpi_rgbas, dhw, ray, eye, zd, **kw)
-        return self._render_path(launch, mpi_rgbas.device, render_size, yaws, pitches, indices, to_uint8, depth_range, want_transmittance, to_host)
+
+        def launch_pinhole(dhw, pinhole, **kw):
+            r.mpi.render_views(mpi_rgbas, dhw, pinhole=pinhole, **kw)
+        return self._render_path(launch, mpi_rgbas.device, render_size, yaws, pitches, indices, to_uint8, depth_range, want_transmittance, to_host,
+                                 launch_pinhole if r.ray_backend == "hip" and mpi_rgbas.is_cuda and mpi_rgbas.dtype is not torch.uint8 else None)
 
     @torch.no_grad()
     def render_path_layers(self, layers: torch.Tensor, render_size: int, yaws: Sequence[float], pitches: Sequence[float],
@@ -177,7 +181,7 @@
             r.mpi.render_views_depth(rgb, depth, plane_z, z_bounds, dhw, ray, eye, zd, background=background, depth_forward=depth_forward, **kw)
         return self._render_path(launch, depth.device, render_size, yaws, pitches, indices, to_uint8, depth_range, want_transmittance, to_host)
 
-    def _render_path(self, launch, dev, render_size, yaws, pitches, indices, to_uint8, depth_range, want_transmittance, to_host):
+    def _render_path(self, launch, dev, render_size, yaws, pitches, indices, to_uint8, depth_range, want_transmittance, to_host, launch_pinhole=None):
         r = self.renderer
         idx = list(range(len(yaws))) if indices is None else list(indices)
         n = len(idx)
@@ -199,26 +203,32 @@
             main = torch.cuda.current_stream(dev)
             self._copy_stream.wait_stream(main)
         group = max(self.batch, (int(256e6 // (12 * render_size * render_size)) // self.batch) * self.batch)
-        ray_g = eye_g = zd_g = None
+        ray_g = eye_g = zd_g = c2w_g = None
         for s in range(0, n, self.batch):
             chunk = idx[s:s + self.batch]
             if s % group == 0:
                 members = idx[s:s + group]
                 gy = torch.tensor([[float(yaws[i])] for i in members], dtype=torch.float32)
                 gp = torch.tensor([[float(pitches[i])] for i in members], dtype=torch.float32)
-                _, _, c2w, rays, eyes, zdirs = r.sample_cam_poses(len(members), 0.0, 0.0, 0.0, 0.0, False, given_yaws=gy, given_pitches=gp)
-                if r._batched_cam is not None and rays is r._batched_cam[0]:
-                    ray_g, eye_g, zd_g = r._batched_cam[1:]
+                if launch_pinhole is not None:
+                    _, _, c2w_g, _ = r._draw_poses(len(members), 0.0, 0.0, 0.0, 0.0, False, gy, gp)
                 else:
-                    ray_g, eye_g, zd_g = torch.cat(rays), torch.cat(eyes), torch.cat(zdirs)
-                r._batched_cam = None
+                    _, _, c2w, rays, eyes, zdirs = r.sample_cam_poses(len(members), 0.0, 0.0, 0.0, 0.0, False, given_yaws=gy, given_pitches=gp)
+                    if r._batched_cam is not None and rays is r._batched_cam[0]:
+                        ray_g, eye_g, zd_g = r._batched_cam[1:]
+                    else:
+                        ray_g, eye_g, zd_g = torch.cat(rays), torch.cat(eyes), torch.cat(zdirs)
+                    r._batched_cam = None
             g0 = s % group
-            ray_t, eye_t, zd_t = ray_g[g0:g0 + len(chunk)], eye_g[g0:g0 + len(chunk)], zd_g[g0:g0 + len(chunk)]
             out = dict(color=rgb[s:s + len(chunk)], depth=dep[s:s + len(chunk)])
             if T is not None:
                 out["T"] = T[s:s + len(chunk)]
-            launch(dhw, ray_t, eye_t, zd_t, views_per_mpi=len(chunk), check_last_plane=True, out_pm1=True,
-                   want_transmittance=want_transmittance, status=status, defer_status=True, out=out)
+            kw = dict(views_per_mpi=len(chunk), check_last_plane=True, out_pm1=True, want_transmittance=want_transmittance, status=status,
+                      defer_status=True, out=out)
+            if launch_pinhole is not None:
+                launch_pinhole(dhw, (c2w_g[g0:g0 + len(chunk)], r.cam.unit_dirs(dev).view(3, render_size, render_size)), **kw)
+            else:
+                launch(dhw, ray_g[g0:g0 + len(chunk)], eye_g[g0:g0 + len(chunk)], zd_g[g0:g0 + len(chunk)], **kw)
             if pipe:
                 e = s + len(chunk)
                 frames_to_uint8(rgb[s:e], dep[s:e], near, far, out=(img8[s:e], dep8[s:e]))
diff --git a/ml-gmpi_amd/hip_mpi.py b/ml-gmpi_amd/hip_mpi.py
--- a/ml-gmpi_amd/hip_mpi.py
+++ b/ml-gmpi_amd/hip_mpi.py
@@ -254,7 +254,7 @@
     return None if t is None else t.data_ptr()
 
 
-_Keep = collections.namedtuple("_Keep", "rgba dhw ray_dir eye_pos z_dir view_to_mpi")
+_Keep = collections.namedtuple("_Keep", "rgba dhw ray_dir eye_pos z_dir view_to_mpi pinhole", defaults=(None,))
 _Scalars = collections.namedtuple("_Scalars", "flags variant rgba_dtype N M D Ht Wt H W views_per_mpi")
 
 
@@ -262,10 +262,12 @@
     p = _lib.GmpiRenderParams()
     p.struct_size = ctypes.sizeof(_lib.GmpiRenderParams)
     p.flags, p.variant, p.rgba_dtype, p.N, p.M, p.D, p.Ht, p.Wt, p.H, p.W, p.views_per_mpi = scalars
-    rgba, dhw, ray_dir, eye_pos, z_dir, view_to_mpi = keep
+    rgba, dhw, ray_dir, eye_pos, z_dir, view_to_mpi, pinhole = keep
     p.rgba = rgba.data_ptr()
     p.rgba_stride[:] = rgba.stride()
-    p.dhw, p.ray_dir, p.eye_pos, p.z_dir = dhw.data_ptr(), ray_dir.data_ptr(), eye_pos.data_ptr(), z_dir.data_ptr()
+    p.dhw = dhw.data_ptr()
+    if pinhole is None:
+        p.ray_dir, p.eye_pos, p.z_dir = ray_dir.data_ptr(), eye_pos.data_ptr(), z_dir.data_ptr()
     if view_to_mpi is not None:
         p.view_to_mpi = view_to_mpi.data_ptr()
     if color is not None:
@@ -273,6 +275,21 @@
     if T is not None:
         p.transmittance_out = T.data_ptr()
     return p
+
+
+def _pinhole_struct(pinhole) -> _lib.GmpiPinhole:
+    cam = _lib.GmpiPinhole()
+    cam.struct_size = ctypes.sizeof(_lib.GmpiPinhole)
+    cam.c2w, cam.unit_dirs = pinhole[0].data_ptr(), pinhole[1].data_ptr()
+    return cam
+
+
+def _pinhole_tensors(pinhole):
+    c2w, dirs = (_f32_on(t.detach(), pinhole[0].device) for t in pinhole)
+    N, (_, H, W), dev = c2w.shape[0], dirs.shape, c2w.device
+    ray, eye, zd = (torch.empty(shape, dtype=torch.float32, device=dev) for shape in ((N, 3, H, W), (N, 3), (N, 3)))
+    _call("gmpi_generate_rays_launch", dev, c2w.data_ptr(), dirs.data_ptr(), N, H, W, ray.data_ptr(), eye.data_ptr(), zd.data_ptr())
+    return ray, eye, zd
 
 
 def _shared_color(rgb: torch.Tensor, background: Optional[torch.Tensor]) -> _lib.GmpiSharedColor:
@@ -655,18 +672,27 @@
                                 c2w_mat=c2w_mat, sphere_c=sphere_c)
         return out["color"], out["depth"]
 
-    def render_views(self, rgba: torch.Tensor, dhw: torch.Tensor, ray_dir: torch.Tensor, eye_pos: torch.Tensor,
-                     z_dir: torch.Tensor, views_per_mpi: Union[int, Sequence[int]] = 1,
+    def render_views(self, rgba: torch.Tensor, dhw: torch.Tensor, ray_dir: Optional[torch.Tensor] = None, eye_pos: Optional[torch.Tensor] = None,
+                     z_dir: Optional[torch.Tensor] = None, views_per_mpi: Union[int, Sequence[int]] = 1,
                      view_to_mpi: Optional[torch.Tensor] = None, check_last_plane: bool = False,
                      out_pm1: bool = False, want_transmittance: bool = False, c2w_mat=None, sphere_c=None,
                      status: Optional[torch.Tensor] = None, defer_status: bool = False, out: Optional[dict] = None,
                      _in_autograd_fn: bool = False, frontal_hint: bool = False, tilted_hint: bool = False, oblique_hint: bool = False,
                      _layout: Optional[_Layout] = None, _shading: Optional[torch.Tensor] = None, _layers: Optional[str] = None,
-                     _layers_backward: str = "planar"):
+                     _layers_backward: str = "planar", pinhole=None):
         if torch.is_grad_enabled() and dhw.requires_grad and not self.geometry_grad:
             raise NotImplementedError("no gradient flows to the plane geometry (the reference computes the grid under "
                                       "torch.no_grad(), mpi.py:65); MPI(geometry_grad=True) provides one")
-        if torch.is_grad_enabled() and not _in_autograd_fn:
+        if pinhole is not None:
+            if ray_dir is not None or eye_pos is not None or z_dir is not None:
+                raise ValueError("render_views takes pinhole=(c2w, unit_dirs) in place of ray_dir, eye_pos and z_dir, not next to them")
+            if _layout is not None or _shading is not None or _layers is not None:
+                raise ValueError("pinhole=(c2w, unit_dirs) is taken by the plain volume render only: the layouts read the camera tensors")
+            if torch.is_grad_enabled() and not _in_autograd_fn and (rgba.requires_grad or (self.geometry_grad and dhw.requires_grad)):
+                (ray_dir, eye_pos, z_dir), pinhole = _pinhole_tensors(pinhole), None
+        elif ray_dir is None or eye_pos is None or z_dir is None:
+            raise TypeError("render_views needs ray_dir, eye_pos and z_dir, or pinhole=(c2w, unit_dirs)")
+        if torch.is_grad_enabled() and not _in_autograd_fn and pinhole is None:
             if rgba.dtype is torch.uint8 and self.geometry_grad and any(t.requires_grad for t in (dhw, ray_dir, eye_pos, z_dir)):
                 raise NotImplementedError("no gradient flows through a uint8 volume, w.r.t. the plane geometry and the camera tensors included "
                                           "(geometry_grad=True): render dequantize_volume(q) (ml_gmpi_amd.quantized) for that, or detach the "
@@ -702,12 +728,18 @@
             variant, images = _lib.VARIANT_GATHER if self.variant == "gather" else _lib.VARIANT_AUTO, (_shading_operand(_shading, dev),)
         if _layout is not None:
             D, variant, images = _layout.operands(self, rgba, dhw)
-        ray_dir, eye_pos, z_dir, dhw = (_f32_on(t, dev) for t in (ray_dir, eye_pos, z_dir, dhw))
-        N, _, H, W = ray_dir.shape
-        assert eye_pos.shape == (N, 3) and z_dir.shape == (N, 3), (eye_pos.shape, z_dir.shape, N)
+        dhw = _f32_on(dhw, dev)
+        if pinhole is None:
+            ray_dir, eye_pos, z_dir = (_f32_on(t, dev) for t in (ray_dir, eye_pos, z_dir))
+            N, _, H, W = ray_dir.shape
+            assert eye_pos.shape == (N, 3) and z_dir.shape == (N, 3), (eye_pos.shape, z_dir.shape, N)
+        else:
+            pinhole = tuple(_f32_on(t.detach(), dev) for t in pinhole)
+            N, (_, H, W) = pinhole[0].shape[0], pinhole[1].shape
+            assert pinhole[0].shape == (N, 4, 4) and pinhole[1].shape == (3, H, W), (pinhole[0].shape, pinhole[1].shape)
         assert dhw.shape == (M, D, 3), (dhw.shape, rgba.shape)
         uniform, view_to_mpi = _view_index(views_per_mpi, view_to_mpi, M, N, dev)
-        keep = _Keep(rgba, dhw, ray_dir, eye_pos, z_dir, view_to_mpi)
+        keep = _Keep(rgba, dhw, ray_dir, eye_pos, z_dir, view_to_mpi, pinhole)
         out = out or {}
         color, depth, T = out.get("color"), out.get("depth"), out.get("T") if want_transmittance else None
         if color is None:
@@ -758,7 +790,10 @@
                 if self.range_check == "full" and rgba.dtype is not torch.uint8 and self._full_check_needed(rgba_in):
                     _range_pass((rgba,), p, dev, stream)
                     fully_checked = rgba_in
-                _call("gmpi_mpi_render_launch", dev, ctypes.byref(p), stream=stream)
+                if pinhole is None:
+                    _call("gmpi_mpi_render_launch", dev, ctypes.byref(p), stream=stream)
+                else:
+                    _call("gmpi_mpi_render_pinhole_launch", dev, ctypes.byref(p), ctypes.byref(_pinhole_struct(pinhole)), stream=stream)
             else:
                 _layout.launch(self, p, rgba, images, dev, stream)
             res = dict(color=color, depth=depth, T=T, status=status)
@@ -892,6 +927,10 @@
             raise IndexError("view_to_mpi holds an index outside [0, #mpi)")
         if word & _lib.STATUS_RGBA_RANGE:
             raise AssertionError("Expected alpha to be within the the range [0, 1]")
+        if keep is not None and keep.pinhole is not None and word & (_lib.STATUS_CAMERA_BEHIND_PLANE | _lib.STATUS_OUT_OF_LAST_PLANE):
+            keep = keep._replace(pinhole=None, **dict(zip(("ray_dir", "eye_pos", "z_dir"), _pinhole_tensors(keep.pinhole))))
+            if params is not None:
+                params = _render_params(_Scalars(*(getattr(params, k) for k in _Scalars._fields)), keep)
         if word & _lib.STATUS_CAMERA_BEHIND_PLANE:
             dist = keep[1][..., 0].flatten().tolist() if keep is not None else "?"
             eye0 = keep[3][0].tolist() if keep is not None else "?"
diff --git a/ml-gmpi_amd/renderer.py b/ml-gmpi_amd/renderer.py
--- a/ml-gmpi_amd/renderer.py
+++ b/ml-gmpi_amd/renderer.py
@@ -364,7 +364,7 @@
         batch_size = n_mpis * views_per_mpi
         if render_h != self.render_h or render_w != self.render_w:
             self.set_cam(self.cam_fov, render_h, render_w)
-        cam_angles, frontal, tilted, oblique = None, False, False, False
+        cam_angles, frontal, tilted, oblique, pinhole = None, False, False, False, None
         if given_cam_infos is None and self.ray_backend == "hip":
             yaws, pitches, c2w, cam_angles = self._draw_poses(batch_size, horizontal_mean, horizontal_std, vertical_mean, vertical_std,
                                                               random_pose, given_yaws, given_pitches)
@@ -372,7 +372,12 @@
             recording = torch.is_grad_enabled() and (batch_mpi_rgbas.requires_grad or (layout is not None and layout.requires_grad) or (shading is not None and shading.requires_grad) or (self.mpi.geometry_grad and self._dhw_for(n_mpis).requires_grad)
                                                      or (layout is not None and self.mpi.geometry_grad_layouts and layout.plane_z_arg is not None and layout.plane_z_arg.requires_grad)
                                                      or (isinstance(chunks, (list, tuple)) and any(c.requires_grad for c in chunks)))
-            ray_t, eye_t, zd_t = self._generate_rays_hip(c2w, reuse=not recording and defer != "lag")
+            if (not recording and layout is None and shading is None and layers_variant is None and chunks is None
+                    and batch_mpi_rgbas.dtype is not torch.uint8):
+                pinhole = (c2w, self.cam.unit_dirs(c2w.device).view(3, self.cam.height, self.cam.width))
+                ray_t = eye_t = zd_t = None
+            else:
+                ray_t, eye_t, zd_t = self._generate_rays_hip(c2w, reuse=not recording and defer != "lag")
         else:
             if given_cam_infos is None:
                 yaws, pitches, c2w, rays, eyes, zdirs = self.sample_cam_poses(
@@ -388,7 +393,8 @@
             else:
                 ray_t, eye_t, zd_t = _cat(rays), _cat(eyes), _cat(zdirs)
             self._batched_cam = None
-        assert ray_t.shape[0] == batch_size, f"{ray_t.shape[0]}, {batch_size}"
+        n_views = c2w.shape[0] if pinhole is not None else ray_t.shape[0]
+        assert n_views == batch_size, f"{n_views}, {batch_size}"
 
         dhw = self._dhw_for(n_mpis)
         if chunks is not None:
@@ -410,7 +416,7 @@
                 batch_mpi_rgbas, dhw, ray_t, eye_t, zd_t, views_per_mpi=views_per_mpi,
                 check_last_plane=assert_not_out_of_last_plane, out_pm1=True, want_transmittance=want_T,
                 c2w_mat=c2w, sphere_c=self.sphere_center, defer_status=defer, frontal_hint=frontal, tilted_hint=tilted, oblique_hint=oblique,
-                _layout=layout)
+                _layout=layout, pinhole=pinhole)
         if cam_angles is None:
             cam_angles = torch.cat([pitches, yaws], -1).to(self.device)
         if want_T:
```

Result: no change. 534,400 Mpix*planes/s (-0.1%).
